# ishine/minimax-speech

Hardware: AMD Instinct MI355X
Metric: 24 kHz audio-seconds generated per wall-second per node (CosyVoice2-0.5B-shaped LM + flow + DAC-VAE, end to end) (higher is better)
Workload: dtype bf16

## Files before the change

### include/mmx_hip.h

```cpp
#ifndef MMX_HIP_H
#define MMX_HIP_H
#include <stdint.h>
#ifdef __cplusplus
extern "C" {
#endif

#ifndef __HIP__
typedef struct ihipStream_t* hipStream_t;
#endif

#define MMX_F32 0
#define MMX_BF16 1
#define MMX_X2 2
#define MMX_X3 3
#define MMX_X2W 0x12
#define MMX_X3W 0x13
#define MMX_H2 4
#define MMX_H2W 0x14

#define MMX_ACT_NONE 0
#define MMX_ACT_LRELU 1
#define MMX_ACT_GELU 2
#define MMX_ACT_SILU 3
#define MMX_ACT_MISH 4
#define MMX_ACT_TANH 5

int mmx_abi_version(void);

typedef struct MmxGemmParams {
    const void* A;
    const void* W;
    const float* bias;
    const float* residual;
    const float* rowmask;
    const float* alpha;
    float* out_f32;
    void* out_act;
    int64_t lda, ldw, ldr, ldo_f, ldo_a;
    int64_t a_bstride, w_bstride, r_bstride, rm_bstride, of_bstride, oa_bstride;
    int64_t row_off, row_lo, row_hi;
    int64_t out_off, out_len;
    int32_t M, N, batch;
    int32_t ntaps, cin, dil;
    int32_t bias_mod, alpha_mod, bias_per_row;
    int32_t act, act2;
    float slope;
    int32_t row_stride;
} MmxGemmParams;
int mmx_gemm_win(const MmxGemmParams* p, int dtype, hipStream_t stream);
#define MMX_TILE_128x128 1
#define MMX_TILE_128x64 2
#define MMX_TILE_64x64 3
#define MMX_TILE_32x64 4
int mmx_gemm_win_tile(const MmxGemmParams* p, int dtype, int tile, hipStream_t stream);

int mmx_rownorm(const float* x, int64_t ldx, int64_t x_bstride, int rows, int C, int batch,
                const float* gamma, const float* beta, float eps, int rms, int act,
                const float* rowmask, int64_t rm_bstride, const float* addvec, int64_t av_bstride,
                float* out_f32, int64_t ldo_f, int64_t of_bstride,
                void* out_act, int64_t ldo_a, int64_t oa_bstride, int dtype, hipStream_t stream);

int mmx_groupnorm(const float* x, int B, int T, int C, int groups, const float* gamma, const float* beta, float eps,
                  int act, const float* rowmask, void* out, int dtype, hipStream_t stream);

int mmx_act_rows(const float* x, int64_t rows, int C, int act, const float* rowmask, float* out_f32, void* out_act, int dtype,
                 hipStream_t stream);

int mmx_gather_rows(const int64_t* ids, int n, const float* table, int C, float scale, const float* rowmask,
                    float* out_f32, int64_t ldo_f, void* out_act, int64_t ldo_a, int dtype, hipStream_t stream);

int mmx_copy2d(const void* in, int in_dtype, int64_t ibs, int64_t irs, int64_t ics, int rep,
               void* out, int out_dtype, int64_t obs, int64_t ors, int64_t ocs,
               int rows, int cols, int batch, hipStream_t stream);

int mmx_est_pack(const float* x, int64_t x_bs, int x_mod, const float* mu, const float* spks, const float* cond, int B, int T, int C,
                 void* h, int64_t ldh, int dtype, hipStream_t stream);
int mmx_sinusoidal_emb(const float* t, int B, int dim, float scale, void* out, int dtype, hipStream_t stream);

int mmx_cfg_euler(float* x, const float* d_cond, const float* d_uncond, float cfg, float dt, int64_t n,
                  hipStream_t stream);

int mmx_attn_dense(const void* q, int64_t ldq, int64_t q_bs, const void* k, int64_t ldk, int64_t k_bs,
                   const void* v, int64_t ldv, int64_t v_bs, void* out, int64_t ldo, int64_t o_bs,
                   int B, int H, int D, int Tq, int Tk, float scale, const float* keymask, int64_t km_bs, int chunk,
                   const void* pos, int64_t ldp, const float* pos_u, const float* pos_v,
                   int head_stride, int q_begin, int dtype, hipStream_t stream);
int mmx_attn_flash_bf16(const void* q, int64_t ldq, int64_t q_bs, const void* k, int64_t ldk, int64_t k_bs,
                        const void* vt, int64_t ldvt, int64_t vt_bs, void* out, int64_t ldo, int64_t o_bs,
                        int B, int H, int T, float scale, const float* keymask, int64_t km_bs, int chunk, int q_begin,
                        const int32_t* klen, hipStream_t stream);
int mmx_attn_relpos_x(const float* q, int64_t ldq, int64_t q_bs, const float* k, int64_t ldk, int64_t k_bs, const float* v,
                      int64_t ldv, int64_t v_bs, const float* pos, int64_t ldp, const float* pos_u, const float* pos_v,
                      float* out, int64_t ldo, int64_t o_bs, int B, int H, int T, float scale, int chunk, const int32_t* klen,
                      hipStream_t stream);
int mmx_attn_flash_x(const float* q, int64_t ldq, int64_t q_bs, const float* k, int64_t ldk, int64_t k_bs,
                     const float* v, int64_t ldv, int64_t v_bs, float* out, int64_t ldo, int64_t o_bs,
                     int B, int H, int T, float scale, const float* keymask, int64_t km_bs, int chunk,
                     int q_begin, const int32_t* klen, hipStream_t stream);
int mmx_attn_flash_xs(const void* qk, int64_t ldqk, int64_t qk_bs, const void* vt, int64_t ldvt, int64_t vt_bs,
                      float* out, int64_t ldo, int64_t o_bs, int B, int H, int T, float scale, const float* keymask,
                      int64_t km_bs, int chunk, int q_begin, const int32_t* klen, int form, hipStream_t stream);
int mmx_attn_relpos_bf16(const void* q, int64_t ldq, int64_t q_bs, const void* k, int64_t ldk, int64_t k_bs,
                         const void* vt, int64_t ldvt, int64_t vt_bs, const void* pos, int64_t ldp,
                         const float* pos_u, const float* pos_v, void* out, int64_t ldo, int64_t o_bs,
                         int B, int H, int T, float scale, int chunk, const int32_t* klen, hipStream_t stream);

int mmx_attn_flash_fp8(const void* q, int64_t ldq, int64_t q_bs, const void* k, int64_t ldk, int64_t k_bs,
                       const void* vt, int64_t ldvt, int64_t vt_bs, void* out, int64_t ldo, int64_t o_bs,
                       int B, int H, int T, float scale, const float* keymask, int64_t km_bs, int chunk, int q_begin,
                       const int32_t* klen, hipStream_t stream);

int mmx_conv_cin1(const float* x, int64_t x_bs, int T, int C, int k, const float* w, const float* bias, float slope,
                  const float* alpha, float* out_f32, void* out_act, int batch, int dtype, hipStream_t stream);
int mmx_vae_sample(const float* ml, const float* noise, int64_t rows, int D, float* z, float* m, float* logs,
                   hipStream_t stream);
int mmx_mask_rows(void* x, int64_t rows, int C, const float* rowmask, int dtype, hipStream_t stream);
int mmx_pool_rows(const float* x, int64_t x_bs, int rows, int C, int batch, const float* mask, int64_t m_bs, void* out,
                  int64_t ldo, int dtype, hipStream_t stream);
int mmx_prefetch4(const void* p0, int64_t n0, const void* p1, int64_t n1, const void* p2, int64_t n2, const void* p3, int64_t n3,
                  void* sink, int workgroups, hipStream_t stream);
int mmx_resample_linear(const float* x, int64_t rows, int T, int T2, float* out, hipStream_t stream);

int mmx_conv_cout1_tanh(const void* act, int64_t a_bs, int T, int C, int k, const float* w, const float* bias,
                        float slope, int use_tanh, float* out, int64_t o_bs, int batch, int dtype, hipStream_t stream);

#define MMX_X_PACKED 1
#define MMX_OUT_PACKED 2
int mmx_pack_skinny(const void* w, int64_t ldw, int N, int K, const float* kscale, int interleave_half,
                    void* wp, int dtype, hipStream_t stream);
int mmx_skinny_gemm(const void* x, int x_dtype, int64_t ldx, int B, int K, int N, const void* wp,
                    const float* bias, int rs, float eps, int epi, float* out_f32, int64_t ldo_f,
                    void* out_act, int64_t ldo_a, int dtype, int flags, const float* kgamma, hipStream_t stream);

int mmx_decode_prep(const float* x, int64_t ldx, int B, int K, const float* gamma, float* h, int64_t ldh, void* xs,
                    float* ssq, int dtype, hipStream_t stream);
int mmx_skinny2(const void* xs, int B, int K, int N, const void* wp, const float* bias, const float* ssq_in, float eps,
                int epi, float* out, int64_t ldo, void* xs_out, const float* gamma_next, float* ssq_out,
                int tiles_per_wg, int ksplit, float* part, int64_t part_floats, int32_t* tickets, int dtype,
                hipStream_t stream);

int mmx_rope_kv_store(const float* qkv, int64_t ldqkv, int64_t qkv_bs, int B, int rows, int Hq, int Hkv, int D,
                      const float* inv_freq, const int32_t* pos, void* q_out, int64_t ldq, int64_t q_bs,
                      void* kc, void* vc, const int32_t* block_table, int max_pages, int page,
                      int dtype, hipStream_t stream);
int mmx_paged_attn(const void* q, int64_t ldq, int64_t q_bs, int B, int rows, int Hq, int Hkv, int D, float scale,
                   const int32_t* pos, const void* kc, const void* vc, const int32_t* block_table, int max_pages,
                   int page, void* out, int64_t ldo, int64_t o_bs, int dtype, hipStream_t stream);
#define MMX_DA_PACKED 1
#define MMX_DA_PER_HEAD 2
#define MMX_DA_SPLIT 4
#define MMX_DA_H2 8
#define MMX_DA_ONE_HEAD 16
int mmx_decode_attn(const float* qkv, int64_t ldqkv, int B, int Hq, int Hkv, int D, const float* inv_freq,
                    const float* rope_tab, const int32_t* pos, void* kc, void* vc, const int32_t* block_table, int max_pages, int page,
                    float scale, void* out, int64_t ldo, int dtype, int out_packed, hipStream_t stream);
int mmx_decode_attn_fin(const float* qkv, int64_t ldqkv, int B, int Hq, int Hkv, int D, const float* inv_freq,
                        const float* rope_tab, const int32_t* pos, const int32_t* finished, void* kc, void* vc,
                        const int32_t* block_table, int max_pages, int page, float scale, void* out, int64_t ldo, int dtype,
                        int out_packed, hipStream_t stream);
int mmx_swiglu(const float* gu, int64_t ldgu, int rows, int I, void* out, int64_t ldo, int dtype, hipStream_t stream);

int mmx_sample_step(const float* logits, int64_t ldl, int V, int B, int eos_id, int top_k, float top_p,
                    int win_size, float tau_r, uint64_t seed, int32_t* state, int32_t* out_tokens, int max_out,
                    int32_t* sampled, const int32_t* forced, const float* speech_emb, int E, float* next_x,
                    int64_t ldx, float* logp_out, hipStream_t stream);
int mmx_sample_step_tab(const float* logits, int64_t ldl, int V, int B, int eos_id, const int32_t* samp, int32_t* state,
                        int32_t* out_tokens, int max_out, int32_t* sampled, const int32_t* forced, const float* speech_emb,
                        int E, float* next_x, int64_t ldx, float* logp_out, hipStream_t stream);

typedef struct MmxEstNext {
    const void* wqkv;
    const float* n1g;
    const float* n1b;
    void* q_out;
    void* vt_out;
    int64_t q_bs, vt_bs;
    int32_t ldq, ldvt;
} MmxEstNext;
typedef struct MmxEstTailParams {
    const void* ao;
    float* x;
    const void* wo;
    const void* w1;
    const void* w2;
    const float* bo;
    const float* b1;
    const float* b2;
    const float* n3g;
    const float* n3b;
    const float* rowmask;
    void* act_out;
    int64_t ao_bs, x_bs, rm_bs, act_bs;
    int32_t ldao, act_ld, B, T;
    int32_t t_begin;
    float eps;
    MmxEstNext next;
} MmxEstTailParams;
typedef struct MmxEstResnetParams {
    const void* a_in;
    float* x;
    const void* w1;
    const void* w2;
    const void* wr;
    const float* b1;
    const float* g1;
    const float* be1;
    const float* b2;
    const float* g2;
    const float* be2;
    const float* br;
    const float* tv;
    const float* rowmask;
    int64_t a_bs, x_bs, tv_bs, rm_bs;
    int32_t lda, cin, B, T;
    int32_t t_begin;
    float eps;
    MmxEstNext next;
} MmxEstResnetParams;
int mmx_est_tail(const MmxEstTailParams* p, int dtype, int bm, int cfg, hipStream_t stream);
int mmx_est_resnet(const MmxEstResnetParams* p, int dtype, int bm, int cfg, hipStream_t stream);
typedef struct {
    const float* x;
    float* x_out;
    void* act_out;
    const void* w7;
    const void* w1;
    const float* b7;
    const float* b1;
    const float* a0;
    const float* a2;
    const float* alpha_next;
    const int32_t* lens;
    int64_t x_bs;
    int32_t B, T, C, dil;
    float slope;
} MmxDacRuParams;
int mmx_dac_ru(const MmxDacRuParams* p, int dtype, int bm, hipStream_t stream);

int mmx_logmel(const float* wave, int64_t w_bs, int L, int B, const float* gain, const int32_t* lens, const int32_t* h_lens,
               const void* basis, const void* filt, int n_fft, int hop, int bin0, int n_bins, int n_mels, float* out_cm,
               int64_t ldo, void* out_tm, int T, int dtype, hipStream_t stream);

int mmx_logmel_w(const float* wave, int64_t w_bs, int L, int B, const int32_t* lens, const int32_t* h_lens, const void* basis,
                 const void* filt, int n_fft, int hop, int bin0, int n_bins, int n_mels, float* out_cm, int64_t ldo,
                 void* out_tm, int T, int dtype, hipStream_t stream);

int mmx_s3_rope_fsmn(float* qkv, int64_t ldqkv, int64_t qkv_bs, int B, int T, int C, const float* x, int64_t x_bs, float* r,
                     int64_t r_bs, const float* wt, const float* rope_cos, const float* rope_sin, int rope_rows,
                     const int32_t* lens, hipStream_t stream);

int mmx_fsq_encode(const float* x, int64_t ldx, int64_t x_bs, int B, int T, int C, const float* W, const float* bias,
                   const int32_t* lens, int32_t* ids, int64_t ld_ids, float* pre, hipStream_t stream);

#define MMX_RESAMPLE_NOUT 1024
int mmx_resample_sinc(const float* wave, int64_t w_bs, int L, int B, const int32_t* lens, const int32_t* h_lens, int orig, int neu,
                      int width, const float* taps, const int32_t* first, const int32_t* count, int cmax, float* out,
                      int64_t o_bs, int out_cols, hipStream_t stream);

#define MMX_LOUD_PAD 0
#define MMX_LOUD_DROP 1
#define MMX_LOUD_MAX_CH 5
int mmx_kweight_blocks(const float* wave, int64_t w_bs, int L, int B, const int32_t* lens, int rate, int partial, const double* tab,
                       int seg, double* work, int cap, double* energy, int64_t e_bs, float* peak, hipStream_t stream);
int mmx_loudness_gate(const double* energy, int64_t e_bs, int cap, const float* peak, const int32_t* lens, int L, int nclips, int nch,
                      const double* G, int rate, int partial, float* lufs, int want_gain, float target_db, float max_peak, float* gain,
                      uint8_t* mask, int64_t mask_bs, hipStream_t stream);
int mmx_scale_rows(const float* x, int64_t x_bs, int L, int B, const int32_t* lens, const float* gain, int nch, float* out,
                   int64_t o_bs, hipStream_t stream);

int mmx_spec_dist(const float* x, int64_t x_bs, const float* y, int64_t y_bs, int L, int B, const int32_t* lens, const int32_t* h_lens,
                  const void* basis, const void* filt, int n_fft, int n_mels, double eps, double pow, double* work, int cap,
                  double* out, hipStream_t stream);
int mmx_wave_sums(const float* x, int64_t x_bs, const float* y, int64_t y_bs, int L, int B, const int32_t* lens, float clip, double* work,
                  int cap, double* out, hipStream_t stream);

#ifdef __cplusplus
}
#endif
#endif
```

### minimax-speech_amd/csrc/fused.hip

```cpp
#include "common.h"
#include "../../include/mmx_hip.h"
#include <type_traits>

namespace {

typedef __attribute__((ext_vector_type(4))) unsigned int u32x4_t;

__device__ unsigned long long* g_tail_stamps = nullptr;
#define TSTAMP(i) do { if constexpr (LAB) { if (st && lane == 0) st[(i)] = __builtin_amdgcn_s_memtime(); } } while (0)

template <typename T> struct FT;
template <> struct FT<bf16_t> { static constexpr int E = 8, KB = 32; typedef short8_t frag_t; };
template <> struct FT<float> { static constexpr int E = 4, KB = 16; typedef float4_t frag_t; };

template <typename T>
__device__ __forceinline__ float4_t mma(typename FT<T>::frag_t a, typename FT<T>::frag_t b, float4_t c) {
    if constexpr (sizeof(T) == 2) {
        return __builtin_amdgcn_mfma_f32_16x16x32_bf16(a, b, c, 0, 0, 0);
    } else {
#pragma unroll
        for (int s = 0; s < 4; ++s) c = __builtin_amdgcn_mfma_f32_16x16x4f32(a[s], b[s], c, 0, 0, 0);
        return c;
    }
}

__host__ __device__ constexpr int tile_pitch(int K, int esz) { return ((K * esz + 255) & ~255) + 32; }

template <typename T, int NF, int PF_>
struct WRing {
    static constexpr int E = FT<T>::E, PF = PF_;
    u32x4_t w[PF][NF];
    __device__ __forceinline__ void prime(const T* wb, long ns, int nk, int nf) {
#pragma unroll
        for (int p = 0; p < PF; ++p)
#pragma unroll
            for (int j = 0; j < NF; ++j)
                w[p][j] = *reinterpret_cast<const u32x4_t*>(wb + (j < nf ? j : 0) * ns + (long)(p < nk ? p : nk - 1) * 64 * E);
    }
};

template <typename T, int MF, int NF, int PF, int NS = 1, int RW = 4>
__device__ __forceinline__ void stage_run(WRing<T, RW, PF>& ring, const char* a_lane, int pitch, int cin_steps,
                                          const T* wb, long ns, int nk, const T* wbn, long nsn, int nkn, int nfn,
                                          float4_t (&acc)[MF][NF], int plane = 0, int tap_pitch = 0) {
    constexpr int E = FT<T>::E, KB = FT<T>::KB;
    typedef typename FT<T>::frag_t frag_t;
    if (tap_pitch == 0) tap_pitch = pitch;
    constexpr int AD = (PF % 2) ? PF : ((MF == 1 && PF >= 4) ? 4 : 2);
    static_assert(PF % AD == 0, "ring depths");
    if constexpr (NS == 2 && MF == 4) {
        frag_t a2[2][MF];
        int rt = 0, rc = 0, rs = 0, rp = 0;
        auto read_u = [&](frag_t (&dst)[MF]) {
            const char* ap = a_lane + rt * tap_pitch + rc * (KB * (int)sizeof(T)) + rp * plane;
#pragma unroll
            for (int i = 0; i < MF; ++i) dst[i] = *reinterpret_cast<const frag_t*>(ap + i * 16 * pitch);
            if (rp == 0) rp = 1;
            else {
                rp = 0;
                if (rs + 1 < nk) {
                    ++rs;
                    if (++rc == cin_steps) { rc = 0; ++rt; }
                }
            }
        };
        auto group2 = [&](int ks, auto last_c) {
            constexpr bool LAST = decltype(last_c)::value;
#pragma unroll
            for (int p = 0; p < PF; ++p) {
                frag_t b[NF];
#pragma unroll
                for (int jj = 0; jj < NF; ++jj) b[jj] = __builtin_bit_cast(frag_t, ring.w[p][jj]);
                if constexpr (LAST) {
                    if (wbn) {
                        const T* src = wbn + (long)(p < nkn ? p : nkn - 1) * 64 * E;
#pragma unroll
                        for (int jj = 0; jj < RW; ++jj) ring.w[p][jj] = *reinterpret_cast<const u32x4_t*>(src + (jj < nfn ? jj : 0) * nsn);
                    }
                } else {
                    const T* src = wb + (long)(ks + p + PF) * 64 * E;
#pragma unroll
                    for (int jj = 0; jj < NF; ++jj) ring.w[p][jj] = *reinterpret_cast<const u32x4_t*>(src + jj * ns);
                }
#pragma unroll
                for (int s2 = 0; s2 < 2; ++s2) {
                    read_u(a2[(s2 + 1) & 1]);
                    __builtin_amdgcn_sched_barrier(0);
#pragma unroll
                    for (int i = 0; i < MF; ++i)
#pragma unroll
                        for (int jj = 0; jj < NF; ++jj) acc[i][jj] = mma<T>(a2[s2][i], b[jj], acc[i][jj]);
                    __builtin_amdgcn_sched_barrier(0);
                }
            }
        };
        read_u(a2[0]);
        for (int ks = 0; ks + PF < nk; ks += PF) group2(ks, std::false_type{});
        group2(nk - PF, std::true_type{});
        return;
    }
    frag_t a[AD][NS][MF];
    int rt = 0, rc = 0, rs = 0;
    auto read_a = [&](frag_t (&dst)[NS][MF]) {
        const char* ap = a_lane + rt * tap_pitch + rc * (KB * (int)sizeof(T));
#pragma unroll
        for (int s2 = 0; s2 < NS; ++s2)
#pragma unroll
            for (int i = 0; i < MF; ++i) dst[s2][i] = *reinterpret_cast<const frag_t*>(ap + s2 * plane + i * 16 * pitch);
        if (rs + 1 < nk) {
            ++rs;
            if (++rc == cin_steps) { rc = 0; ++rt; }
        }
    };
    auto group = [&](int ks, auto last_c) {
        constexpr bool LAST = decltype(last_c)::value;
#pragma unroll
        for (int p = 0; p < PF; ++p) {
            read_a(a[(p + AD - 1) % AD]);
            frag_t b[NF];
#pragma unroll
            for (int jj = 0; jj < NF; ++jj) b[jj] = __builtin_bit_cast(frag_t, ring.w[p][jj]);
            if constexpr (LAST) {
                if (wbn) {
                    const T* src = wbn + (long)(p < nkn ? p : nkn - 1) * 64 * E;
#pragma unroll
                    for (int jj = 0; jj < RW; ++jj) ring.w[p][jj] = *reinterpret_cast<const u32x4_t*>(src + (jj < nfn ? jj : 0) * nsn);
                }
            } else {
                const T* src = wb + (long)(ks + p + PF) * 64 * E;
#pragma unroll
                for (int jj = 0; jj < NF; ++jj) ring.w[p][jj] = *reinterpret_cast<const u32x4_t*>(src + jj * ns);
            }
            __builtin_amdgcn_sched_barrier(0);
#pragma unroll
            for (int s2 = 0; s2 < NS; ++s2)
#pragma unroll
                for (int i = 0; i < MF; ++i)
#pragma unroll
                    for (int jj = 0; jj < NF; ++jj) acc[i][jj] = mma<T>(a[p % AD][s2][i], b[jj], acc[i][jj]);
            __builtin_amdgcn_sched_barrier(0);
        }
    };
#pragma unroll
    for (int s_ = 0; s_ < AD - 1; ++s_) read_a(a[s_]);
    for (int ks = 0; ks + PF < nk; ks += PF) group(ks, std::false_type{});
    group(nk - PF, std::true_type{});
}

template <typename T, int MF, int NF, int PF, int NS, int RW, bool WP>
__device__ __forceinline__ void stage_run_w(WRing<T, RW, PF>& ring, const char* a_lane, int pitch, int cin_steps,
                                            const T* wb, long ns, int nk, long wlo, const T* wbn, long nsn, int nkn, int nfn,
                                            float4_t (&acc)[MF][NF], int plane = 0, int tap_pitch = 0) {
    if constexpr (!WP) {
        stage_run<T, MF, NF, PF, NS, RW>(ring, a_lane, pitch, cin_steps, wb, ns, nk, wbn, nsn, nkn, nfn, acc, plane, tap_pitch);
    } else {
        stage_run<T, MF, NF, PF, NS, RW>(ring, a_lane, pitch, cin_steps, wb, ns, nk, wb + wlo, ns, nk, NF, acc, plane, tap_pitch);
        stage_run<T, MF, NF, PF, 1, RW>(ring, a_lane, pitch, cin_steps, wb + wlo, ns, nk, wbn, nsn, nkn, nfn, acc, 0, tap_pitch);
    }
}

template <int MF, int NF>
__device__ __forceinline__ void zero_acc(float4_t (&acc)[MF][NF]) {
#pragma unroll
    for (int i = 0; i < MF; ++i)
#pragma unroll
        for (int j = 0; j < NF; ++j) acc[i][j] = float4_t{0.f, 0.f, 0.f, 0.f};
}

constexpr int PATCH_FLOATS = 16 * 68;
constexpr int TAIL_PRM_FLOATS = 6 * 256 + 1024;
template <int NF>
__device__ __forceinline__ void to_rows(const float4_t (&acc)[NF], float* patch, int lane, float (&v)[NF * 4]) {
    constexpr int LDC = NF * 16 + 4;
    const int g = lane >> 4, l16 = lane & 15;
#pragma unroll
    for (int j = 0; j < NF; ++j)
#pragma unroll
        for (int r = 0; r < 4; ++r) patch[(4 * g + r) * LDC + j * 16 + l16] = acc[j][r];
    __builtin_amdgcn_fence(__ATOMIC_RELEASE, "wavefront");
    __builtin_amdgcn_wave_barrier();
    const float* src = patch + (lane >> 2) * LDC + (lane & 3) * (NF * 4);
#pragma unroll
    for (int c = 0; c < NF * 4; c += 4) {
        const float4_t t = *reinterpret_cast<const float4_t*>(src + c);
        v[c] = t[0]; v[c + 1] = t[1]; v[c + 2] = t[2]; v[c + 3] = t[3];
    }
    __builtin_amdgcn_wave_barrier();
}

constexpr int SPATCH_FLOATS = 16 * 20;
__device__ __forceinline__ void to_rows_sp(const float4_t (&acc)[2], float* patch, int lane, float (&v)[8]) {
    constexpr int LDC = 20;
    const int g = lane >> 4, l16 = lane & 15;
    const float* src = patch + (lane >> 2) * LDC + (lane & 1) * 8;
#pragma unroll
    for (int j = 0; j < 2; ++j) {
#pragma unroll
        for (int r = 0; r < 4; ++r) patch[(4 * g + r) * LDC + l16] = acc[j][r];
        __builtin_amdgcn_fence(__ATOMIC_RELEASE, "wavefront");
        __builtin_amdgcn_wave_barrier();
        if (((lane >> 1) & 1) == j) {
            const float4_t t0 = *reinterpret_cast<const float4_t*>(src), t1 = *reinterpret_cast<const float4_t*>(src + 4);
            v[0] = t0[0]; v[1] = t0[1]; v[2] = t0[2]; v[3] = t0[3];
            v[4] = t1[0]; v[5] = t1[1]; v[6] = t1[2]; v[7] = t1[3];
        }
        __builtin_amdgcn_wave_barrier();
    }
}
template <int NF, bool SP>
__device__ __forceinline__ void rows_of(const float4_t (&acc)[NF], float* patch, int lane, float (&v)[NF * 4]) {
    if constexpr (SP) { static_assert(NF == 2, "one-fragment patch: 32-column slices"); to_rows_sp(acc, patch, lane, v); }
    else to_rows<NF>(acc, patch, lane, v);
}

template <int N>
__device__ __forceinline__ void loadn(const float* p, float (&v)[N]) {
#pragma unroll
    for (int c = 0; c < N; c += 4) {
        const float4_t t = *reinterpret_cast<const float4_t*>(p + c);
        v[c] = t[0]; v[c + 1] = t[1]; v[c + 2] = t[2]; v[c + 3] = t[3];
    }
}
template <int N>
__device__ __forceinline__ void storen(float* p, const float (&v)[N]) {
#pragma unroll
    for (int c = 0; c < N; c += 4) *reinterpret_cast<float4_t*>(p + c) = float4_t{v[c], v[c + 1], v[c + 2], v[c + 3]};
}
template <typename T, int N>
__device__ __forceinline__ void storen_T(T* p, const float (&v)[N]) {
    if constexpr (sizeof(T) == 2) {
#pragma unroll
        for (int c = 0; c < N; c += 8) {
            uint4 pk;
            pk.x = pack_bf16x2(v[c], v[c + 1]);
            pk.y = pack_bf16x2(v[c + 2], v[c + 3]);
            pk.z = pack_bf16x2(v[c + 4], v[c + 5]);
            pk.w = pack_bf16x2(v[c + 6], v[c + 7]);
            *reinterpret_cast<uint4*>(p + c) = pk;
        }
    } else {
        storen<N>(p, v);
    }
}

template <typename T, int NS, int N>
__device__ __forceinline__ void store_tile(char* p, int plane, const float (&v)[N]) {
    if constexpr (NS == 1) {
        storen_T<T, N>(reinterpret_cast<T*>(p), v);
    } else {
        float lo[N];
#pragma unroll
        for (int c = 0; c < N; c += 8) {
            uint4 pk;
            pk.x = pack_bf16x2(v[c], v[c + 1]);
            pk.y = pack_bf16x2(v[c + 2], v[c + 3]);
            pk.z = pack_bf16x2(v[c + 4], v[c + 5]);
            pk.w = pack_bf16x2(v[c + 6], v[c + 7]);
            *reinterpret_cast<uint4*>(p + c * 2) = pk;
            const unsigned w[4] = {pk.x, pk.y, pk.z, pk.w};
#pragma unroll
            for (int e = 0; e < 4; ++e) {
                lo[c + 2 * e] = v[c + 2 * e] - __uint_as_float(w[e] << 16);
                lo[c + 2 * e + 1] = v[c + 2 * e + 1] - __uint_as_float(w[e] & 0xffff0000u);
            }
        }
        storen_T<bf16_t, N>(reinterpret_cast<bf16_t*>(p + plane), lo);
    }
}

template <int MFR, int CW, int NW>
__device__ __forceinline__ void layernorm_rows(float (&v)[MFR][CW], float* stats, const float (&g)[CW], const float (&be)[CW],
                                               float eps, int wave, int lane) {
    const int rl = lane >> 2;
    float mean[MFR];
    auto total = [&](int row) {
        float t = 0.f;
#pragma unroll
        for (int w = 0; w < NW; w += 4) {
            const float4_t q = *reinterpret_cast<const float4_t*>(stats + row * NW + w);
            t += (q[0] + q[1]) + (q[2] + q[3]);
        }
        return t;
    };
#pragma unroll
    for (int i = 0; i < MFR; ++i) {
        float s = 0.f;
#pragma unroll
        for (int c = 0; c < CW; ++c) s += v[i][c];
        s += dpp_f32<0xB1>(s);
        s += dpp_f32<0x4E>(s);
        if ((lane & 3) == 0) stats[(i * 16 + rl) * NW + wave] = s;
    }
    __syncthreads();
#pragma unroll
    for (int i = 0; i < MFR; ++i) mean[i] = total(i * 16 + rl) * (1.0f / 256.0f);
    __syncthreads();
#pragma unroll
    for (int i = 0; i < MFR; ++i) {
        float q = 0.f;
#pragma unroll
        for (int c = 0; c < CW; ++c) { const float d = v[i][c] - mean[i]; q += d * d; }
        q += dpp_f32<0xB1>(q);
        q += dpp_f32<0x4E>(q);
        if ((lane & 3) == 0) stats[(i * 16 + rl) * NW + wave] = q;
    }
    __syncthreads();
#pragma unroll
    for (int i = 0; i < MFR; ++i) {
        const float rstd = rsqrtf(total(i * 16 + rl) * (1.0f / 256.0f) + eps);
#pragma unroll
        for (int c = 0; c < CW; ++c) v[i][c] = (v[i][c] - mean[i]) * rstd * g[c] + be[c];
    }
}

template <typename T>
__device__ __forceinline__ void load_tile(const T* __restrict__ src, long ld, int r0, int nvalid, int rows, int K,
                                          char* tile, int pitch, int tid, int nthreads) {
    constexpr int E = FT<T>::E, U = 8;
    const int cpr = K / E;
    const int total = rows * cpr;
    for (int base = tid; base < total; base += U * nthreads) {
        uint4 v[U];
        int off[U];
#pragma unroll
        for (int u = 0; u < U; ++u) {
            const int id = base + u * nthreads;
            const int idc = id < total ? id : total - 1;
            const int r = idc / cpr, ch = idc - r * cpr;
            const int gr = r0 + r;
            const bool ok = gr >= 0 && gr < nvalid;
            const int grc = gr < 0 ? 0 : (gr < nvalid ? gr : nvalid - 1);
            v[u] = *reinterpret_cast<const uint4*>(src + (long)grc * ld + ch * E);
            if (!ok) v[u] = make_uint4(0, 0, 0, 0);
            off[u] = id < total ? r * pitch + ch * 16 : -1;
        }
#pragma unroll
        for (int u = 0; u < U; ++u)
            if (off[u] >= 0) *reinterpret_cast<uint4*>(tile + off[u]) = v[u];
    }
}
__device__ __forceinline__ void load_tile_split(const float* __restrict__ src, long ld, int r0, int nvalid, int rows, int K,
                                                char* tile, int pitch, int plane, int tid, int nthreads) {
    constexpr int U = 8;
    const int cpr = K / 4;
    const int total = rows * cpr;
    for (int base = tid; base < total; base += U * nthreads) {
        float4 v[U];
        int off[U];
#pragma unroll
        for (int u = 0; u < U; ++u) {
            const int id = base + u * nthreads;
            const int idc = id < total ? id : total - 1;
            const int r = idc / cpr, ch = idc - r * cpr;
            const int gr = r0 + r;
            const bool ok = gr >= 0 && gr < nvalid;
            const int grc = gr < 0 ? 0 : (gr < nvalid ? gr : nvalid - 1);
            v[u] = *reinterpret_cast<const float4*>(src + (long)grc * ld + ch * 4);
            if (!ok) v[u] = make_float4(0.f, 0.f, 0.f, 0.f);
            off[u] = id < total ? r * pitch + ch * 8 : -1;
        }
#pragma unroll
        for (int u = 0; u < U; ++u) {
            if (off[u] < 0) continue;
            uint2 hi, lo;
            hi.x = pack_bf16x2(v[u].x, v[u].y);
            hi.y = pack_bf16x2(v[u].z, v[u].w);
            lo.x = pack_bf16x2(v[u].x - __uint_as_float(hi.x << 16), v[u].y - __uint_as_float(hi.x & 0xffff0000u));
            lo.y = pack_bf16x2(v[u].z - __uint_as_float(hi.y << 16), v[u].w - __uint_as_float(hi.y & 0xffff0000u));
            *reinterpret_cast<uint2*>(tile + off[u]) = hi;
            *reinterpret_cast<uint2*>(tile + plane + off[u]) = lo;
        }
    }
}

__device__ __forceinline__ void load_tile_split_halves(const float* __restrict__ src, long ld, int r0, int nvalid, int rows,
                                                       char* tile0, char* tile1, int pitch, int plane, int tid, int nthreads) {
    constexpr int U = 16;
    constexpr int cpr = 512 / 4;
    const int total = rows * cpr;
    for (int base = tid; base < total; base += U * nthreads) {
        float4 v[U];
        int off[U];
#pragma unroll
        for (int u = 0; u < U; ++u) {
            const int id = base + u * nthreads;
            const int idc = id < total ? id : total - 1;
            const int r = idc / cpr, ch = idc - r * cpr;
            const int gr = r0 + r;
            const bool ok = gr >= 0 && gr < nvalid;
            const int grc = gr < 0 ? 0 : (gr < nvalid ? gr : nvalid - 1);
            v[u] = *reinterpret_cast<const float4*>(src + (long)grc * ld + ch * 4);
            if (!ok) v[u] = make_float4(0.f, 0.f, 0.f, 0.f);
            off[u] = id < total ? r * pitch + (ch & 63) * 8 + ((ch >> 6) ? (int)(tile1 - tile0) : 0) : -1;
        }
#pragma unroll
        for (int u = 0; u < U; ++u) {
            if (off[u] < 0) continue;
            uint2 hi, lo;
            hi.x = pack_bf16x2(v[u].x, v[u].y);
            hi.y = pack_bf16x2(v[u].z, v[u].w);
            lo.x = pack_bf16x2(v[u].x - __uint_as_float(hi.x << 16), v[u].y - __uint_as_float(hi.x & 0xffff0000u));
            lo.y = pack_bf16x2(v[u].z - __uint_as_float(hi.y << 16), v[u].w - __uint_as_float(hi.y & 0xffff0000u));
            *reinterpret_cast<uint2*>(tile0 + off[u]) = hi;
            *reinterpret_cast<uint2*>(tile0 + plane + off[u]) = lo;
        }
    }
}

template <typename T, int NW, int PW = 4>
__device__ __forceinline__ const T* qkv_pass(const void* wqkv, int wave, int lane, int p) {
    constexpr int E = FT<T>::E, KB = FT<T>::KB, PC = 16 * PW, PPK = 512 / (PC * NW);
    return reinterpret_cast<const T*>(wqkv) + (long)lane * E +
           (long)(((p / PPK) * 512 + (wave * PPK + p % PPK) * PC) / 16) * ((long)(256 / KB) * 64 * E);
}

template <typename T, int MF, int PF, int NW, int NS = 1, int PW = 4, bool WP = false>
__device__ __forceinline__ void ln_qkv(float (&xv)[MF][64 / NW], const float (&n1g)[64 / NW], const float (&n1b)[64 / NW],
                                       const MmxEstNext& nx, float eps, char* a1, float* patch, float* stats,
                                       WRing<T, PW, PF>& ring, int b, int t0, int Tn, int wave, int lane, int plane = 0,
                                       unsigned long long* st = nullptr) {
    typedef std::conditional_t<NS == 1, T, float> TI;
    constexpr int E = FT<T>::E, KB = FT<T>::KB, C = 256, CW = 64 / NW, PC = 16 * PW, PPK = 512 / (PC * NW), NP = 3 * PPK;
    constexpr int P1 = tile_pitch(C, sizeof(T));
    constexpr int NK = C / KB;
    const int g = lane >> 4, l16 = lane & 15, rl = lane >> 2;
    const int col0 = wave * (256 / NW) + (lane & 3) * CW;
    const long ns = (long)NK * 64 * E;
    layernorm_rows<MF, CW, NW>(xv, stats, n1g, n1b, eps, wave, lane);
#pragma unroll
    for (int i = 0; i < MF; ++i) store_tile<T, NS, CW>(a1 + (i * 16 + rl) * P1 + col0 * (int)sizeof(T), plane, xv[i]);
    __syncthreads();
    TSTAMP(32);
    const char* a_lane = a1 + l16 * P1 + g * 16;
    constexpr bool VTC = sizeof(T) == 2;
    const bool planes = NS > 1 && nx.vt_out != nullptr;
    const bool vt_path = VTC && (NS == 1 || planes);
    constexpr int PV = 16 * 2 + 16;
    for (int p = 0; p < NP; ++p) {
        float4_t acc[MF][PW];
        zero_acc(acc);
        const T* wn = p + 1 < NP ? qkv_pass<T, NW, PW>(nx.wqkv, wave, lane, p + 1) : nullptr;
        stage_run_w<T, MF, PW, PF, NS, PW, WP>(ring, a_lane, P1, NK, qkv_pass<T, NW, PW>(nx.wqkv, wave, lane, p), ns, NK, 1536L * C, wn, ns, NK, PW, acc, plane);
        TSTAMP(33 + 2 * p);
        const int kind = p / PPK, cw = (wave * PPK + p % PPK) * PC;
        if (vt_path && kind == 2) {
            char* vw = reinterpret_cast<char*>(patch);
#pragma unroll
            for (int s2 = 0; s2 < NS; ++s2) {
                bf16_t* dst = reinterpret_cast<bf16_t*>(nx.vt_out) + (long)b * nx.vt_bs + (long)s2 * 512 * nx.ldvt + (long)cw * nx.ldvt + t0;
#pragma unroll
                for (int i = 0; i < MF; ++i) {
#pragma unroll
                    for (int j = 0; j < PW; ++j) {
                        uint2 pk;
                        pk.x = pack_bf16x2(acc[i][j][0], acc[i][j][1]);
                        pk.y = pack_bf16x2(acc[i][j][2], acc[i][j][3]);
                        *reinterpret_cast<uint2*>(vw + (j * 16 + l16) * PV + (4 * g) * 2) = pk;
                        if (s2 + 1 < NS) {
                            acc[i][j][0] -= __uint_as_float(pk.x << 16); acc[i][j][1] -= __uint_as_float(pk.x & 0xffff0000u);
                            acc[i][j][2] -= __uint_as_float(pk.y << 16); acc[i][j][3] -= __uint_as_float(pk.y & 0xffff0000u);
                        }
                    }
                    __builtin_amdgcn_fence(__ATOMIC_RELEASE, "wavefront");
                    __builtin_amdgcn_wave_barrier();
#pragma unroll
                    for (int k2 = 0; k2 < PW / 2; ++k2) {
                        const int chunk = lane + 64 * k2, colv = chunk >> 1, c8 = chunk & 1;
                        uint4 v = *reinterpret_cast<const uint4*>(vw + colv * PV + c8 * 16);
                        const int t = t0 + i * 16 + c8 * 8;
                        if (t >= Tn) continue;
                        if (t + 8 > Tn) {
                            unsigned short* h = reinterpret_cast<unsigned short*>(&v);
#pragma unroll
                            for (int e = 0; e < 8; ++e)
                                if (t + e >= Tn) h[e] = 0;
                        }
                        *reinterpret_cast<uint4*>(dst + (long)colv * nx.ldvt + i * 16 + c8 * 8) = v;
                    }
                    __builtin_amdgcn_wave_barrier();
                }
            }
        } else if (planes) {
            bf16_t* out = reinterpret_cast<bf16_t*>(nx.q_out) + (long)b * nx.q_bs;
            const int col = kind * 512 + cw + (lane & 3) * (4 * PW);
#pragma unroll
            for (int i = 0; i < MF; ++i) {
                float v[4 * PW], lo[4 * PW];
                to_rows<PW>(acc[i], patch, lane, v);
                const int t = t0 + i * 16 + rl;
                if (t < Tn) {
#pragma unroll
                    for (int c = 0; c < 4 * PW; ++c) lo[c] = v[c] - bf2f(f2bf(v[c]));
                    storen_T<bf16_t, 4 * PW>(out + (long)t * nx.ldq + col, v);
                    storen_T<bf16_t, 4 * PW>(out + (long)t * nx.ldq + 1024 + col, lo);
                }
            }
        } else {
            TI* out = reinterpret_cast<TI*>(nx.q_out) + (long)b * nx.q_bs;
            const int col = kind * 512 + cw + (lane & 3) * (4 * PW);
#pragma unroll
            for (int i = 0; i < MF; ++i) {
                float v[4 * PW];
                to_rows<PW>(acc[i], patch, lane, v);
                const int t = t0 + i * 16 + rl;
                if (t < Tn) storen_T<TI, 4 * PW>(out + (long)t * nx.ldq + col, v);
            }
        }
        TSTAMP(34 + 2 * p);
    }
}

template <typename T, int BM, int PF, int NW, int NS, int PW, bool WP = false>
__device__ __forceinline__ void est_tail_tile(const MmxEstTailParams& p, const int tile) {
    constexpr bool HK = NS == 2 && BM == 64 && sizeof(T) == 2;
    static_assert(!HK || (NW == 8 && PW == 2), "64-row split tile: 8 waves, 32-column passes");
    constexpr int MF = BM / 16, E = FT<T>::E, KB = FT<T>::KB, C = 256, CI = 512, CF = 1024, CH = HK ? 256 : 512, NCH = CF / CH;
    constexpr int WC = C / NW, CW = WC / 4, NFN = WC / 16, PC = 16 * PW, PPC = CH / (PC * NW);
    static_assert(NFN <= PW, "the ring is PW fragments wide");
    constexpr int P0 = tile_pitch(HK ? C : CI, sizeof(T)), P1 = tile_pitch(C, sizeof(T));
    constexpr int PL0 = BM * P0, PL1 = BM * P1;
    constexpr bool PRECISE = sizeof(T) == 4;
    typedef std::conditional_t<NS == 1, T, float> TI;
    extern __shared__ __attribute__((aligned(16))) char smem[];
    char* buf0 = smem;
    char* a1 = buf0 + NS * PL0;
    float* patch_all = reinterpret_cast<float*>(a1 + NS * PL1);
    constexpr int PATCHF = HK ? SPATCH_FLOATS : PATCH_FLOATS;
    float* stats = patch_all + NW * PATCHF;
    float* prm = stats + BM * NW;
    constexpr int PRM_BO = 0, PRM_N3G = 256, PRM_N3B = 512, PRM_B2 = 768, PRM_N1G = 1024, PRM_N1B = 1280, PRM_B1 = 1536;
    const int tid = threadIdx.x, lane = tid & 63, wave = tid >> 6;
    const int g = lane >> 4, l16 = lane & 15, rl = lane >> 2;
    float* patch = patch_all + wave * PATCHF;
    const int b = blockIdx.y, t0 = p.t_begin + tile * BM, Tn = p.T;
    const int col0 = wave * WC + (lane & 3) * CW;
    unsigned long long* st = nullptr;
    if constexpr (LAB) {
        st = g_tail_stamps;
        if (st) st += ((long)(blockIdx.y * gridDim.x + blockIdx.x) * NW + wave) * 64;
    }
    TSTAMP(0);

    const T* wo = reinterpret_cast<const T*>(p.wo) + (long)lane * E;
    const T* w1 = reinterpret_cast<const T*>(p.w1) + (long)lane * E;
    const T* w2 = reinterpret_cast<const T*>(p.w2) + (long)lane * E;
    constexpr int NK0 = CI / KB, NK1 = C / KB, NK2 = CH / KB, NK2T = CF / KB, NKH = NK0 / 2;
    const long ns0 = (long)NK0 * 64 * E, ns1 = (long)NK1 * 64 * E, ns2 = (long)NK2T * 64 * E;
    WRing<T, PW, PF> ring;
    const T* wo_w = wo + (long)(wave * NFN) * ns0;

    auto w1_pass = [&](int q) { return w1 + (long)(((q / PPC) * CH + (wave * PPC + q % PPC) * PC) / 16) * ns1; };
    float x1[MF][CW];
    float rm[MF];
    {
        const float* rmk = p.rowmask ? p.rowmask + (long)b * p.rm_bs : nullptr;
#pragma unroll
        for (int i = 0; i < MF; ++i) {
            const int t = t0 + i * 16 + rl;
            rm[i] = (rmk && t < Tn) ? rmk[t] : 1.f;
        }
    }
    {
        constexpr int PRM_PER = (TAIL_PRM_FLOATS / 4 + 64 * NW - 1) / (64 * NW);
        float4_t pr[PRM_PER];
#pragma unroll
        for (int k = 0; k < PRM_PER; ++k) {
            const int id0 = tid + k * 64 * NW, id = id0 < TAIL_PRM_FLOATS / 4 ? id0 : TAIL_PRM_FLOATS / 4 - 1;
            const int seg = id >> 6, o4 = (id & 63) * 4;
            const float* src = seg == 0 ? p.bo : seg == 1 ? p.n3g : seg == 2 ? p.n3b : seg == 3 ? p.b2
                             : seg == 4 ? (p.next.wqkv ? p.next.n1g : p.b2) : seg == 5 ? (p.next.wqkv ? p.next.n1b : p.b2) : p.b1 + (seg - 6) * 256;
            pr[k] = *reinterpret_cast<const float4_t*>(src + o4);
        }
        const float* xr = p.x + (long)b * p.x_bs;
#pragma unroll
        for (int i = 0; i < MF; ++i) {
            const int t = t0 + i * 16 + rl;
            loadn<CW>(xr + (long)(t < Tn ? t : Tn - 1) * C + col0, x1[i]);
            if (t >= Tn) {
#pragma unroll
                for (int c = 0; c < CW; ++c) x1[i][c] = 0.f;
            }
        }
        ring.prime(wo_w, ns0, NK0, NFN);
        if constexpr (HK) {
            static_assert(P0 == P1 && PL0 == PL1, "both halves of the attention tile have the shape of a1");
            load_tile_split_halves(reinterpret_cast<const float*>(p.ao) + (long)b * p.ao_bs, p.ldao, t0, Tn, BM, buf0, a1, P0, PL0, tid, 64 * NW);
        } else if constexpr (NS == 1) load_tile<T>(reinterpret_cast<const T*>(p.ao) + (long)b * p.ao_bs, p.ldao, t0, Tn, BM, CI, buf0, P0, tid, 64 * NW);
        else load_tile_split(reinterpret_cast<const float*>(p.ao) + (long)b * p.ao_bs, p.ldao, t0, Tn, BM, CI, buf0, P0, PL0, tid, 64 * NW);
#pragma unroll
        for (int k = 0; k < PRM_PER; ++k) {
            const int id = tid + k * 64 * NW;
            if (id < TAIL_PRM_FLOATS / 4) *reinterpret_cast<float4_t*>(prm + id * 4) = pr[k];
        }
        TSTAMP(1);
        __syncthreads();
        TSTAMP(2);
        float4_t acc[MF][NFN];
        zero_acc(acc);
        if constexpr (HK) {
            const T* wo_h = wo_w + (long)NKH * 64 * E;
            if constexpr (WP) {
                const long wlo = (long)C * CI;
                stage_run<T, MF, NFN, PF, NS, PW>(ring, buf0 + l16 * P0 + g * 16, P0, NKH, wo_w, ns0, NKH, wo_h, ns0, NKH, NFN, acc, PL0);
                stage_run<T, MF, NFN, PF, NS, PW>(ring, a1 + l16 * P1 + g * 16, P1, NKH, wo_h, ns0, NKH, wo_w + wlo, ns0, NKH, NFN, acc, PL1);
                stage_run<T, MF, NFN, PF, 1, PW>(ring, buf0 + l16 * P0 + g * 16, P0, NKH, wo_w + wlo, ns0, NKH, wo_h + wlo, ns0, NKH, NFN, acc, 0);
                stage_run<T, MF, NFN, PF, 1, PW>(ring, a1 + l16 * P1 + g * 16, P1, NKH, wo_h + wlo, ns0, NKH, w1_pass(0), ns1, NK1, PW, acc, 0);
            } else {
                stage_run<T, MF, NFN, PF, NS, PW>(ring, buf0 + l16 * P0 + g * 16, P0, NKH, wo_w, ns0, NKH, wo_h, ns0, NKH, NFN, acc, PL0);
                stage_run<T, MF, NFN, PF, NS, PW>(ring, a1 + l16 * P1 + g * 16, P1, NKH, wo_h, ns0, NKH, w1_pass(0), ns1, NK1, PW, acc, PL1);
            }
        } else
        stage_run_w<T, MF, NFN, PF, NS, PW, WP>(ring, buf0 + l16 * P0 + g * 16, P0, NK0, wo_w, ns0, NK0, (long)C * CI, w1_pass(0), ns1, NK1, PW, acc, PL0);
        TSTAMP(3);
        float bo[CW];
        loadn<CW>(prm + PRM_BO + col0, bo);
#pragma unroll
        for (int i = 0; i < MF; ++i) {
            float v[CW];
            rows_of<NFN, HK>(acc[i], patch, lane, v);
#pragma unroll
            for (int c = 0; c < CW; ++c) x1[i][c] += v[c] + bo[c];
        }
        TSTAMP(4);
    }
    float n3g[CW], n3b[CW];
    loadn<CW>(prm + PRM_N3G + col0, n3g);
    loadn<CW>(prm + PRM_N3B + col0, n3b);
    {
        float hn[MF][CW];
#pragma unroll
        for (int i = 0; i < MF; ++i)
#pragma unroll
            for (int c = 0; c < CW; ++c) hn[i][c] = x1[i][c];
        layernorm_rows<MF, CW, NW>(hn, stats, n3g, n3b, p.eps, wave, lane);
#pragma unroll
        for (int i = 0; i < MF; ++i) store_tile<T, NS, CW>(a1 + (i * 16 + rl) * P1 + col0 * (int)sizeof(T), PL1, hn[i]);
    }
    __syncthreads();
    TSTAMP(5);
    float4_t acc2[MF][NFN];
    zero_acc(acc2);
    const T* w2_w = w2 + (long)(wave * NFN) * ns2;
    for (int ch = 0; ch < NCH; ++ch) {
        const int sb = HK ? 6 + ch * 5 : 0;
        for (int h = 0; h < PPC; ++h) {
            const int q = ch * PPC + h;
            const int hc = (wave * PPC + h) * PC + (lane & 3) * (4 * PW);
            float4_t acc[MF][PW];
            zero_acc(acc);
            const bool more = h + 1 < PPC;
            const T* wn = more ? w1_pass(q + 1) : w2_w + (long)(ch * NK2) * 64 * E;
            stage_run_w<T, MF, PW, PF, NS, PW, WP>(ring, a1 + l16 * P1 + g * 16, P1, NK1, w1_pass(q), ns1, NK1, (long)CF * C, wn, more ? ns1 : ns2,
                                                   more ? NK1 : NK2, more ? PW : NFN, acc, PL1);
            TSTAMP(HK ? sb : 6 + ch * 12 + h * 2);
            if constexpr (HK) {
                const bool odd = lane & 1;
                const int cb = (wave * PPC + h) * PC;
                float bj[PW];
#pragma unroll
                for (int j = 0; j < PW; ++j) bj[j] = prm[PRM_B1 + ch * CH + cb + j * 16 + l16];
                char* dst = buf0 + (4 * g + (odd ? 2 : 0)) * P0 + (cb + (l16 & ~1)) * (int)sizeof(T);
#pragma unroll
                for (int r = 0; r < MF; ++r)
#pragma unroll
                    for (int j = 0; j < PW; ++j) {
                        float v[4];
#pragma unroll
                        for (int e = 0; e < 4; e += 2) {
                            const f32x2_t gl = gelu_fast2(f32x2_t{acc[r][j][e] + bj[j], acc[r][j][e + 1] + bj[j]});
                            v[e] = gl.x; v[e + 1] = gl.y;
                        }
                        const float y0 = dpp_f32<0xB1>(odd ? v[0] : v[2]), y1 = dpp_f32<0xB1>(odd ? v[1] : v[3]);
                        const float a0 = odd ? y0 : v[0], c0 = odd ? v[2] : y0, a1v = odd ? y1 : v[1], c1 = odd ? v[3] : y1;
                        const unsigned h0 = pack_bf16x2(a0, c0), h1 = pack_bf16x2(a1v, c1);
                        const unsigned l0 = pack_bf16x2(a0 - __uint_as_float(h0 << 16), c0 - __uint_as_float(h0 & 0xffff0000u));
                        const unsigned l1 = pack_bf16x2(a1v - __uint_as_float(h1 << 16), c1 - __uint_as_float(h1 & 0xffff0000u));
                        char* q2 = dst + r * 16 * P0 + j * 16 * (int)sizeof(T);
                        *reinterpret_cast<unsigned*>(q2) = h0;
                        *reinterpret_cast<unsigned*>(q2 + P0) = h1;
                        *reinterpret_cast<unsigned*>(q2 + PL0) = l0;
                        *reinterpret_cast<unsigned*>(q2 + PL0 + P0) = l1;
                    }
                TSTAMP(sb + 1);
                continue;
            }
            float b1[4 * PW];
            loadn<4 * PW>(prm + PRM_B1 + ch * CH + hc, b1);
#pragma unroll
            for (int i = 0; i < MF; ++i) {
                float v[4 * PW];
                rows_of<PW, HK>(acc[i], patch, lane, v);
                if constexpr (NS > 1 && !PRECISE) {
#pragma unroll
                    for (int c = 0; c < 4 * PW; c += 2) {
                        const f32x2_t gl = gelu_fast2(f32x2_t{v[c] + b1[c], v[c + 1] + b1[c + 1]});
                        v[c] = gl.x; v[c + 1] = gl.y;
                    }
                } else {
#pragma unroll
                    for (int c = 0; c < 4 * PW; ++c) v[c] = act_c<((PRECISE || NS > 1) ? ACT_GELU : ACT_GELU_POLY), PRECISE>(v[c] + b1[c], 0.f);
                }
                store_tile<T, NS, 4 * PW>(buf0 + (i * 16 + rl) * P0 + hc * (int)sizeof(T), PL0, v);
            }
            TSTAMP(HK ? sb + 1 : 7 + ch * 12 + h * 2);
        }
        __syncthreads();
        TSTAMP(HK ? sb + 2 : 14 + ch * 12);
        const T* wn = ch + 1 < NCH ? w1_pass((ch + 1) * PPC) : (p.next.wqkv ? qkv_pass<T, NW, PW>(p.next.wqkv, wave, lane, 0) : nullptr);
        if constexpr (WP && !HK) {
            constexpr int NKQ = NK2 / 2;
            const T* wh = w2_w + (long)(ch * NK2) * 64 * E;
            stage_run_w<T, MF, NFN, PF, NS, PW, WP>(ring, buf0 + l16 * P0 + g * 16, P0, NKQ, wh, ns2, NKQ, (long)C * CF, wh + (long)NKQ * 64 * E, ns2, NKQ, NFN, acc2, PL0);
            stage_run_w<T, MF, NFN, PF, NS, PW, WP>(ring, buf0 + NKQ * KB * (int)sizeof(T) + l16 * P0 + g * 16, P0, NKQ, wh + (long)NKQ * 64 * E, ns2, NKQ, (long)C * CF, wn, ns1, NK1, PW, acc2, PL0);
        } else
        stage_run_w<T, MF, NFN, PF, NS, PW, WP>(ring, buf0 + l16 * P0 + g * 16, P0, NK2, w2_w + (long)(ch * NK2) * 64 * E, ns2, NK2, (long)C * CF, wn, ns1, NK1, PW, acc2, PL0);
        TSTAMP(HK ? sb + 3 : 15 + ch * 12);
        __syncthreads();
        TSTAMP(HK ? sb + 4 : 16 + ch * 12);
    }
    float* wpatch = HK ? reinterpret_cast<float*>(buf0) + wave * PATCH_FLOATS : patch;
    {
        float* xw = p.x + (long)b * p.x_bs;
        float b2[CW];
        loadn<CW>(prm + PRM_B2 + col0, b2);
#pragma unroll
        for (int i = 0; i < MF; ++i) {
            float v[CW];
            to_rows<NFN>(acc2[i], wpatch, lane, v);
            const int t = t0 + i * 16 + rl;
#pragma unroll
            for (int c = 0; c < CW; ++c) x1[i][c] = (x1[i][c] + v[c] + b2[c]) * rm[i];
            if (t < Tn) {
                storen<CW>(xw + (long)t * C + col0, x1[i]);
                if (p.act_out)
                    storen_T<TI, CW>(reinterpret_cast<TI*>(p.act_out) + (long)b * p.act_bs + (long)t * p.act_ld + col0, x1[i]);
            }
        }
    }
    TSTAMP(31);
    if (p.next.wqkv) {
        float n1g[CW], n1b[CW];
        loadn<CW>(prm + PRM_N1G + col0, n1g);
        loadn<CW>(prm + PRM_N1B + col0, n1b);
        ln_qkv<T, MF, PF, NW, NS, PW, WP>(x1, n1g, n1b, p.next, p.eps, a1, wpatch, stats, ring, b, t0, Tn, wave, lane, PL1, st);
    }
    TSTAMP(63);
}

template <typename T, int BM, int PF, int NW, int NS = 1, int OCC = 1, int PW = 4, bool WP = false>
__global__ __launch_bounds__(64 * NW, OCC) void est_tail_kernel(MmxEstTailParams p) {
    est_tail_tile<T, BM, PF, NW, NS, PW, WP>(p, blockIdx.x);
}

template <typename T, int BM, int PF, int NW, int NS = 1, bool WP = false>
__global__ __launch_bounds__(64 * NW) void est_resnet_kernel(MmxEstResnetParams p) {
    constexpr int MF = BM / 16, MH = MF + 1, E = FT<T>::E, KB = FT<T>::KB, C = 256;
    constexpr int WC = C / NW, CW = WC / 4, NFN = WC / 16;
    constexpr int P1 = tile_pitch(C, sizeof(T));
    constexpr int PLH = (BM + 16) * P1;
    constexpr bool PRECISE = sizeof(T) == 4;
    extern __shared__ __attribute__((aligned(16))) char smem[];
    const int cin = p.cin;
    const int PA = tile_pitch(cin, sizeof(T));
    const int PLA = (BM + 18) * PA;
    char* ain = smem;
    char* h1 = ain + NS * PLA;
    float* patch_all = reinterpret_cast<float*>(h1 + NS * PLH);
    float* stats = patch_all + NW * PATCH_FLOATS;
    const int tid = threadIdx.x, lane = tid & 63, wave = tid >> 6;
    const int g = lane >> 4, l16 = lane & 15, rl = lane >> 2;
    float* patch = patch_all + wave * PATCH_FLOATS;
    const int b = blockIdx.y, t0 = p.t_begin + blockIdx.x * BM, Tn = p.T;
    const int col0 = wave * WC + (lane & 3) * CW;
    const int cs = cin / KB;
    const T* w1 = reinterpret_cast<const T*>(p.w1) + (long)lane * E;
    const T* w2 = reinterpret_cast<const T*>(p.w2) + (long)lane * E;
    const T* wr = reinterpret_cast<const T*>(p.wr) + (long)lane * E;
    const int nk1 = 3 * cs, nk2 = 3 * (C / KB), nkr = cs;
    const long ns1 = (long)nk1 * 64 * E, ns2 = (long)nk2 * 64 * E, nsr = (long)nkr * 64 * E;
    const T* w1_w = w1 + (long)(wave * NFN) * ns1;
    const T* w2_w = w2 + (long)(wave * NFN) * ns2;
    const T* wr_w = wr + (long)(wave * NFN) * nsr;
    WRing<T, 4, PF> ring;
    ring.prime(w1_w, ns1, nk1, NFN);
    const float* rmk = p.rowmask ? p.rowmask + (long)b * p.rm_bs : nullptr;
    float bb[CW], tv[CW], gg[CW], be[CW], rm1[MH];
    loadn<CW>(p.b1 + col0, bb);
    loadn<CW>(p.tv + (long)b * p.tv_bs + col0, tv);
    loadn<CW>(p.g1 + col0, gg);
    loadn<CW>(p.be1 + col0, be);
#pragma unroll
    for (int i = 0; i < MH; ++i) {
        const int t = t0 - 16 + i * 16 + rl;
        rm1[i] = (t >= 0 && t < Tn) ? (rmk ? rmk[t] : 1.f) : 0.f;
    }
    if constexpr (NS == 1) load_tile<T>(reinterpret_cast<const T*>(p.a_in) + (long)b * p.a_bs, p.lda, t0 - 18, Tn, BM + 18, cin, ain, PA, tid, 64 * NW);
    else load_tile_split(reinterpret_cast<const float*>(p.a_in) + (long)b * p.a_bs, p.lda, t0 - 18, Tn, BM + 18, cin, ain, PA, PLA, tid, 64 * NW);
    __syncthreads();

    {
        float4_t acc[MH][NFN];
        zero_acc(acc);
        stage_run_w<T, MH, NFN, PF, NS, 4, WP>(ring, ain + l16 * PA + g * 16, PA, cs, w1_w, ns1, nk1, (long)C * 3 * cin, w2_w, ns2, nk2, NFN, acc, PLA);
        float hv[MH][CW];
#pragma unroll
        for (int i = 0; i < MH; ++i) {
            to_rows<NFN>(acc[i], patch, lane, hv[i]);
#pragma unroll
            for (int c = 0; c < CW; ++c) hv[i][c] += bb[c];
        }
        layernorm_rows<MH, CW, NW>(hv, stats, gg, be, p.eps, wave, lane);
#pragma unroll
        for (int i = 0; i < MH; ++i) {
            const int t = t0 - 16 + i * 16 + rl;
            float o[CW];
#pragma unroll
            for (int c = 0; c < CW; ++c) {
                const float y = act_c<ACT_MISH, PRECISE>(hv[i][c], 0.f) * rm1[i];
                o[c] = t >= 0 ? (y + tv[c]) * rm1[i] : 0.f;
            }
            store_tile<T, NS, CW>(h1 + (i * 16 + rl) * P1 + col0 * (int)sizeof(T), PLH, o);
        }
    }
    float br[CW];
    loadn<CW>(p.b2 + col0, bb);
    loadn<CW>(p.g2 + col0, gg);
    loadn<CW>(p.be2 + col0, be);
    loadn<CW>(p.br + col0, br);
    __syncthreads();
    float h2[MF][CW];
    {
        float4_t acc[MF][NFN];
        zero_acc(acc);
        stage_run_w<T, MF, NFN, PF, NS, 4, WP>(ring, h1 + (14 + l16) * P1 + g * 16, P1, C / KB, w2_w, ns2, nk2, (long)C * 3 * C, wr_w, nsr, nkr, NFN, acc, PLH);
#pragma unroll
        for (int i = 0; i < MF; ++i) {
            to_rows<NFN>(acc[i], patch, lane, h2[i]);
#pragma unroll
            for (int c = 0; c < CW; ++c) h2[i][c] += bb[c];
        }
        layernorm_rows<MF, CW, NW>(h2, stats, gg, be, p.eps, wave, lane);
#pragma unroll
        for (int i = 0; i < MF; ++i)
#pragma unroll
            for (int c = 0; c < CW; ++c) h2[i][c] = act_c<ACT_MISH, PRECISE>(h2[i][c], 0.f) * rm1[i + 1];
    }
    {
        if (p.next.wqkv) { loadn<CW>(p.next.n1g + col0, gg); loadn<CW>(p.next.n1b + col0, be); }
        float4_t acc[MF][NFN];
        zero_acc(acc);
        const T* wq0 = p.next.wqkv ? qkv_pass<T, NW>(p.next.wqkv, wave, lane, 0) : nullptr;
        stage_run_w<T, MF, NFN, PF, NS, 4, WP>(ring, ain + (18 + l16) * PA + g * 16, PA, cs, wr_w, nsr, nkr, (long)C * cin, wq0, (long)(C / KB) * 64 * E, C / KB, 4, acc, PLA);
        float* xw = p.x + (long)b * p.x_bs;
#pragma unroll
        for (int i = 0; i < MF; ++i) {
            float v[CW];
            to_rows<NFN>(acc[i], patch, lane, v);
            const int t = t0 + i * 16 + rl;
#pragma unroll
            for (int c = 0; c < CW; ++c) h2[i][c] += v[c] + br[c];
            if (t < Tn) storen<CW>(xw + (long)t * C + col0, h2[i]);
        }
    }
    __syncthreads();
    if (p.next.wqkv) ln_qkv<T, MF, PF, NW, NS, 4, WP>(h2, gg, be, p.next, p.eps, h1, patch, stats, ring, b, t0, Tn, wave, lane, PLH);
}


__host__ __device__ constexpr int dac_pitch(int cp) { return (((cp * 2 + 31) / 32) | 1) * 32; }
__host__ __device__ constexpr int dac_patch_floats(int C) { return 16 * ((C % 48 == 0 ? 48 : 64) + 4); }

template <int C, int BM, int WR, int WC, int NS, int PF, bool WP = false, int NF = C / (16 * WC)>
__global__ __launch_bounds__(256) void dac_ru_kernel(MmxDacRuParams p) {
    typedef bf16_t T;
    constexpr int E = 8, KB = 32, CP = (C + 31) / 32 * 32, PA = dac_pitch(CP);
    constexpr int NC = 4 * NF, WCOLS = 16 * NF, DAC_PATCH_FLOATS = dac_patch_floats(C);
    static_assert(NF >= 2 && NF <= 4 && 16 * (WCOLS + 4) <= DAC_PATCH_FLOATS, "n-fragments per wave / patch");
    constexpr int BMW = BM / WR, MF = BMW / 16;
    constexpr int NK7 = 7 * CP / KB, NK1 = CP / KB;
    constexpr bool PRECISE = NS > 1;
    static_assert(WR * WC == 4 && WC * NF * 16 == C && NK7 % PF == 0 && NK1 % PF == 0, "wave grid / ring depth");
    typedef std::conditional_t<NS == 1, bf16_t, float> TA;
    extern __shared__ __attribute__((aligned(16))) char smem[];
    const int d = p.dil, halo = 3 * d, rows_in = BM + 2 * halo;
    const int PLA = rows_in * PA, PLM = BM * PA;
    char* ain = smem;
    char* mid = ain + NS * PLA;
    float* patch_all = reinterpret_cast<float*>(mid + NS * PLM);
    float* prm = patch_all + 4 * DAC_PATCH_FLOATS;
    auto snk = [](float x, float alpha, float inv) {
        const float sn = PRECISE ? sin_cw(alpha * x) : __sinf(alpha * x);
        return x + inv * (sn * sn);
    };
    const int tid = threadIdx.x, lane = tid & 63, wave = tid >> 6;
    const int g = lane >> 4, l16 = lane & 15, rl = lane >> 2;
    const int wr = wave / WC, wc = wave % WC;
    float* patch = patch_all + wave * DAC_PATCH_FLOATS;
    const int b = blockIdx.y, t0 = blockIdx.x * BM;
    const int len = p.lens ? p.lens[b] : p.T;
    const int lc = len > 0 ? len : 1;
    const float* xb = p.x + (long)b * p.x_bs;

    const T* w7 = reinterpret_cast<const T*>(p.w7) + (long)lane * E;
    const T* w1 = reinterpret_cast<const T*>(p.w1) + (long)lane * E;
    const long ns7 = (long)NK7 * 64 * E, ns1 = (long)NK1 * 64 * E;
    const T* w7_w = w7 + (long)(wc * NF) * ns7;
    const T* w1_w = w1 + (long)(wc * NF) * ns1;
    WRing<T, NF, PF> ring;
    ring.prime(w7_w, ns7, NK7, NF);

    for (int id = tid; id < 8 * CP; id += 256) {
        const int v = id / CP, c = id - v * CP;
        const float* src = v == 0 ? p.a0 : v == 1 ? p.a2 : v == 2 ? p.b7 : v == 3 ? p.b1 : v == 4 ? p.alpha_next : v == 5 ? p.a0 : v == 6 ? p.a2 : p.alpha_next;
        const float val = (c < C && src) ? src[c] : 0.f;
        prm[id] = v < 5 ? val : 1.0f / (val + 1e-9f);
    }
    __syncthreads();
    {
        constexpr int CPR = CP / 4, U = 16;
        const int total = rows_in * CPR;
        for (int base = tid; base < total; base += U * 256) {
            float4 v[U];
            int off[U], cch[U];
#pragma unroll
            for (int u = 0; u < U; ++u) {
                const int id = base + u * 256;
                const int idc = id < total ? id : total - 1;
                const int r = idc / CPR, ch = idc - r * CPR;
                const int t = t0 - halo + r;
                const bool ok = t >= 0 && t < len && ch * 4 < C;
                const int tc = t < 0 ? 0 : (t < lc ? t : lc - 1);
                const int cc = ch * 4 < C ? ch * 4 : 0;
                v[u] = *reinterpret_cast<const float4*>(xb + (long)tc * C + cc);
                if (!ok) v[u] = make_float4(0.f, 0.f, 0.f, 0.f);
                off[u] = id < total ? r * PA + ch * 8 : -1;
                cch[u] = ch * 4;
            }
#pragma unroll
            for (int u = 0; u < U; ++u) {
                if (off[u] < 0) continue;
                const float4_t al = *reinterpret_cast<const float4_t*>(prm + cch[u]);
                const float4_t iv = *reinterpret_cast<const float4_t*>(prm + 5 * CP + cch[u]);
                float o[4] = {snk(v[u].x, al[0], iv[0]), snk(v[u].y, al[1], iv[1]), snk(v[u].z, al[2], iv[2]), snk(v[u].w, al[3], iv[3])};
                uint2 hi;
                hi.x = pack_bf16x2(o[0], o[1]);
                hi.y = pack_bf16x2(o[2], o[3]);
                *reinterpret_cast<uint2*>(ain + off[u]) = hi;
                if constexpr (NS > 1) {
                    uint2 lo;
                    lo.x = pack_bf16x2(o[0] - __uint_as_float(hi.x << 16), o[1] - __uint_as_float(hi.x & 0xffff0000u));
                    lo.y = pack_bf16x2(o[2] - __uint_as_float(hi.y << 16), o[3] - __uint_as_float(hi.y & 0xffff0000u));
                    *reinterpret_cast<uint2*>(ain + PLA + off[u]) = lo;
                }
            }
        }
        if constexpr (CP > C) {
            for (int id = tid; id < BM * (CP - C) / 4; id += 256) {
                const int r = id / ((CP - C) / 4), ch = id % ((CP - C) / 4);
#pragma unroll
                for (int s2 = 0; s2 < NS; ++s2) *reinterpret_cast<uint2*>(mid + s2 * PLM + r * PA + (C + ch * 4) * 2) = make_uint2(0, 0);
            }
        }
    }
    __syncthreads();
    {
        float4_t acc[MF][NF];
        zero_acc(acc);
        stage_run_w<T, MF, NF, PF, NS, NF, WP>(ring, ain + (wr * BMW + l16) * PA + g * 16, PA, CP / KB, w7_w, ns7, NK7, (long)C * 7 * CP, w1_w, ns1, NK1, NF, acc, PLA, d * PA);
        const int col = wc * WCOLS + (lane & 3) * NC;
        float b7[NC], a2[NC], i2[NC];
        loadn<NC>(prm + 2 * CP + col, b7);
        loadn<NC>(prm + 1 * CP + col, a2);
        loadn<NC>(prm + 6 * CP + col, i2);
#pragma unroll
        for (int i = 0; i < MF; ++i) {
            float v[NC];
            to_rows<NF>(acc[i], patch, lane, v);
#pragma unroll
            for (int c = 0; c < NC; ++c) {
                float y = v[c] + b7[c];
                y = y > 0.f ? y : y * p.slope;
                v[c] = snk(y, a2[c], i2[c]);
            }
            char* dst = mid + (wr * BMW + i * 16 + rl) * PA + col * 2;
            unsigned w[NC / 2];
#pragma unroll
            for (int e = 0; e < NC / 2; ++e) w[e] = pack_bf16x2(v[2 * e], v[2 * e + 1]);
#pragma unroll
            for (int e = 0; e < NC / 4; ++e) *reinterpret_cast<uint2*>(dst + 8 * e) = make_uint2(w[2 * e], w[2 * e + 1]);
            if constexpr (NS > 1) {
                unsigned l[NC / 2];
#pragma unroll
                for (int e = 0; e < NC / 2; ++e)
                    l[e] = pack_bf16x2(v[2 * e] - __uint_as_float(w[e] << 16), v[2 * e + 1] - __uint_as_float(w[e] & 0xffff0000u));
#pragma unroll
                for (int e = 0; e < NC / 4; ++e) *reinterpret_cast<uint2*>(dst + PLM + 8 * e) = make_uint2(l[2 * e], l[2 * e + 1]);
            }
        }
    }
    const int col = wc * WCOLS + (lane & 3) * NC;
    float xr[MF][NC];
#pragma unroll
    for (int i = 0; i < MF; ++i) {
        const int t = t0 + wr * BMW + i * 16 + rl;
        loadn<NC>(xb + (long)(t < lc ? t : lc - 1) * C + col, xr[i]);
    }
    __syncthreads();
    {
        float4_t acc[MF][NF];
        zero_acc(acc);
        stage_run_w<T, MF, NF, PF, NS, NF, WP>(ring, mid + (wr * BMW + l16) * PA + g * 16, PA, NK1, w1_w, ns1, NK1, (long)C * CP, (const T*)nullptr, 0, 0, NF, acc, PLM);
        float b1[NC], an[NC], in[NC];
        loadn<NC>(prm + 3 * CP + col, b1);
        loadn<NC>(prm + 4 * CP + col, an);
        loadn<NC>(prm + 7 * CP + col, in);
        float* xo = p.x_out ? p.x_out + (long)b * p.x_bs : nullptr;
#pragma unroll
        for (int i = 0; i < MF; ++i) {
            float v[NC];
            to_rows<NF>(acc[i], patch, lane, v);
            const int t = t0 + wr * BMW + i * 16 + rl;
            const bool live = t < len;
#pragma unroll
            for (int c = 0; c < NC; ++c) {
                float y = v[c] + b1[c];
                y = y > 0.f ? y : y * p.slope;
                v[c] = live ? y + xr[i][c] : 0.f;
            }
            if (t < p.T) {
                if (xo) storen<NC>(xo + (long)t * C + col, v);
                if (p.act_out) {
#pragma unroll
                    for (int c = 0; c < NC; ++c) v[c] = snk(v[c], an[c], in[c]);
                    TA* ao = reinterpret_cast<TA*>(p.act_out) + (long)b * p.x_bs + (long)t * C + col;
                    if constexpr (NS == 1) {
#pragma unroll
                        for (int e = 0; e < NC / 4; ++e)
                            *reinterpret_cast<uint2*>(ao + 4 * e) = make_uint2(pack_bf16x2(v[4 * e], v[4 * e + 1]), pack_bf16x2(v[4 * e + 2], v[4 * e + 3]));
                    } else {
                        storen<NC>(reinterpret_cast<float*>(ao), v);
                    }
                }
            }
        }
    }
}

constexpr size_t LDS_MAX = 160 * 1024;
constexpr size_t dac_ru_lds(int C, int bm, int ns, int dil) {
    const int CP = (C + 31) / 32 * 32, PA = dac_pitch(CP);
    return (size_t)ns * ((size_t)(bm + 6 * dil) * PA + (size_t)bm * PA) + 4 * dac_patch_floats(C) * 4 + 8 * CP * 4;
}
constexpr size_t tail_lds(int esz, int bm, int nw, int ns) {
    if (ns == 2 && bm == 64 && esz == 2)
        return (size_t)ns * 2 * bm * tile_pitch(256, esz) + (size_t)nw * SPATCH_FLOATS * 4 + (size_t)bm * nw * 4 + (size_t)TAIL_PRM_FLOATS * 4;
    return ns * ((size_t)bm * tile_pitch(512, esz) + (size_t)bm * tile_pitch(256, esz)) + (size_t)nw * PATCH_FLOATS * 4 + (size_t)bm * nw * 4 +
           (size_t)TAIL_PRM_FLOATS * 4;
}
constexpr size_t resnet_lds(int esz, int bm, int nw, int ns, int cin) {
    return ns * ((size_t)(bm + 18) * tile_pitch(cin, esz) + (size_t)(bm + 16) * tile_pitch(256, esz)) + (size_t)nw * PATCH_FLOATS * 4 +
           (size_t)(bm + 16) * nw * 4;
}

template <typename P>
struct Form {
    int dtype;
    bool wp;
    int bm, nw, pf;
    int pw, C;
    int (*launch)(const P&, hipStream_t);
};
template <typename T, int NS>
constexpr int form_dtype = sizeof(T) == 4 ? MMX_F32 : NS == 2 ? MMX_X2 : MMX_BF16;
template <typename P, size_t N>
constexpr const Form<P>* find_form(const Form<P> (&forms)[N], int dtype, bool wp, int bm, int nw, int pf, int pw, int C) {
    for (const Form<P>& f : forms)
        if (f.dtype == dtype && f.wp == wp && f.bm == bm && f.nw == nw && f.pf == pf && f.pw == pw && f.C == C) return &f;
    return nullptr;
}
constexpr bool cfg_fields_ok(int cfg, int known) {
    const int pf = cfg & 15, nw = (cfg >> 4) & 15;
    return cfg >= 0 && !(cfg & ~known) && (pf == 0 || pf == 2 || pf == 4 || pf == 8) && (nw == 0 || nw == 4 || nw == 8);
}

int check_next(const MmxEstNext& nx, int dtype, int T_) {
    if (!nx.wqkv) return MMX_OK;
    MMX_CHECK_ARG(nx.n1g && nx.n1b && nx.q_out);
    MMX_CHECK_ARG(((uintptr_t)nx.q_out % 16) == 0 && nx.q_bs % 8 == 0);
    if (dtype == MMX_X2) {
        if (nx.vt_out) {
            MMX_CHECK_ARG(nx.ldq % 8 == 0 && nx.ldq >= 2048 && nx.q_bs % 8 == 0 && nx.ldvt % 8 == 0 && nx.ldvt >= ((T_ + 7) / 8) * 8);
            MMX_CHECK_ARG(((uintptr_t)nx.vt_out % 16) == 0 && nx.vt_bs % 8 == 0 && nx.vt_bs >= 2 * 512 * (int64_t)nx.ldvt);
        } else {
            MMX_CHECK_ARG(nx.ldq % 4 == 0 && nx.ldq >= 1536 && nx.q_bs % 4 == 0);
        }
    } else if (dtype == MMX_BF16) {
        MMX_CHECK_ARG(nx.vt_out && nx.ldq % 8 == 0 && nx.ldq >= 1024 && nx.ldvt % 8 == 0 && nx.ldvt >= ((T_ + 7) / 8) * 8);
        MMX_CHECK_ARG(((uintptr_t)nx.vt_out % 16) == 0 && nx.vt_bs % 8 == 0);
    } else {
        MMX_CHECK_ARG(nx.ldq % 4 == 0 && nx.ldq >= 1536);
    }
    return MMX_OK;
}

template <typename T, int BM, int PF, int NW, int NS, int PW, bool WP>
int launch_tail(const MmxEstTailParams& p, hipStream_t stream) {
    constexpr size_t lds = tail_lds(sizeof(T), BM, NW, NS);
    MMX_CHECK_ARG(lds <= LDS_MAX);
    MMX_LDS_OPT_IN((est_tail_kernel<T, BM, PF, NW, NS, 1, PW, WP>), lds);
    hipLaunchKernelGGL((est_tail_kernel<T, BM, PF, NW, NS, 1, PW, WP>), dim3((p.T - p.t_begin + BM - 1) / BM, p.B), dim3(64 * NW), lds, stream, p);
    MMX_LAUNCH_CHECK();
    return MMX_OK;
}
using TailForm = Form<MmxEstTailParams>;
template <typename T, int BM, int PF, int NW, int NS = 1, int PW = 4, bool WP = false>
constexpr TailForm tail_form() { return {form_dtype<T, NS>, WP, BM, NW, PF, PW, 0, launch_tail<T, BM, PF, NW, NS, PW, WP>}; }
constexpr TailForm TAIL_FORMS[] = {
    tail_form<bf16_t, 64, 2, 8, 1, 2>(), tail_form<bf16_t, 32, 8, 8, 1, 2>(), tail_form<bf16_t, 32, 4, 8, 1, 2>(),
    tail_form<bf16_t, 64, 4, 4>(), tail_form<bf16_t, 64, 2, 4>(), tail_form<bf16_t, 32, 4, 8>(), tail_form<bf16_t, 32, 2, 8>(),
    tail_form<bf16_t, 32, 2, 4>(), tail_form<bf16_t, 32, 4, 4>(), tail_form<bf16_t, 16, 4, 8>(), tail_form<bf16_t, 16, 8, 4>(),
    tail_form<bf16_t, 64, 2, 8, 2, 2>(), tail_form<bf16_t, 64, 4, 8, 2, 2>(), tail_form<bf16_t, 32, 2, 8, 2, 2>(), tail_form<bf16_t, 32, 4, 8, 2, 2>(),
    tail_form<bf16_t, 32, 2, 8, 2>(), tail_form<bf16_t, 32, 4, 4, 2>(), tail_form<bf16_t, 16, 4, 8, 2>(), tail_form<bf16_t, 16, 8, 4, 2>(),
    tail_form<bf16_t, 64, 2, 8, 2, 2, true>(), tail_form<bf16_t, 32, 2, 8, 2, 4, true>(), tail_form<bf16_t, 16, 4, 8, 2, 4, true>(),
    tail_form<float, 32, 4, 4>(), tail_form<float, 16, 8, 4>(),
};
constexpr const TailForm* tail_select(int dtype, bool wp, int bm, int cfg) {
    if (!cfg_fields_ok(cfg, 0x7ff) || (bm != 16 && bm != 32 && bm != 64)) return nullptr;
    if (wp) cfg = 0;
    if (cfg & (256 | 1024)) return nullptr;
    int pf = cfg & 15, nw = (cfg >> 4) & 15;
    bool narrow = (cfg >> 9) & 1;
    if (cfg == 0 && dtype == MMX_BF16 && bm >= 32) { narrow = true; pf = bm == 64 ? 2 : 8; }
    if (dtype == MMX_X2 && bm == 64) narrow = true;
    if (narrow) nw = 8;
    else if (nw == 0) nw = dtype == MMX_X2 || (dtype == MMX_BF16 && bm == 32) ? 8 : 4;
    const int pw = narrow ? 2 : 4, pf_tile = narrow ? 128 / bm : 512 / (bm * nw);
    const TailForm* f = find_form(TAIL_FORMS, dtype, wp, bm, nw, pf, pw, 0);
    return f ? f : find_form(TAIL_FORMS, dtype, wp, bm, nw, pf_tile, pw, 0);
}
static_assert(tail_select(MMX_BF16, false, 64, 0)->launch == launch_tail<bf16_t, 64, 2, 8, 1, 2, false> && tail_select(MMX_BF16, false, 32, 0)->launch == launch_tail<bf16_t, 32, 8, 8, 1, 2, false>);
static_assert(tail_select(MMX_BF16, false, 16, 0)->launch == launch_tail<bf16_t, 16, 8, 4, 1, 4, false> && tail_select(MMX_X2, false, 64, 0)->launch == launch_tail<bf16_t, 64, 2, 8, 2, 2, false>);
static_assert(tail_select(MMX_X2, false, 32, 0)->launch == launch_tail<bf16_t, 32, 2, 8, 2, 4, false> && tail_select(MMX_X2, false, 16, 0)->launch == launch_tail<bf16_t, 16, 4, 8, 2, 4, false>);
static_assert(tail_select(MMX_X2, true, 64, 0)->launch == launch_tail<bf16_t, 64, 2, 8, 2, 2, true> && tail_select(MMX_X2, true, 32, 0)->launch == launch_tail<bf16_t, 32, 2, 8, 2, 4, true>);
static_assert(tail_select(MMX_X2, true, 16, 0)->launch == launch_tail<bf16_t, 16, 4, 8, 2, 4, true>);
static_assert(tail_select(MMX_F32, false, 32, 0)->launch == launch_tail<float, 32, 4, 4, 1, 4, false> && tail_select(MMX_F32, false, 16, 0)->launch == launch_tail<float, 16, 8, 4, 1, 4, false>);

template <typename T, int BM, int PF, int NW, int NS, bool WP>
int launch_resnet(const MmxEstResnetParams& p, hipStream_t stream) {
    const size_t lds = resnet_lds(sizeof(T), BM, NW, NS, p.cin);
    MMX_CHECK_ARG(lds <= LDS_MAX);
    MMX_LDS_OPT_IN((est_resnet_kernel<T, BM, PF, NW, NS, WP>), lds);
    hipLaunchKernelGGL((est_resnet_kernel<T, BM, PF, NW, NS, WP>), dim3((p.T - p.t_begin + BM - 1) / BM, p.B), dim3(64 * NW), lds, stream, p);
    MMX_LAUNCH_CHECK();
    return MMX_OK;
}
using ResnetForm = Form<MmxEstResnetParams>;
template <typename T, int BM, int PF, int NW, int NS = 1, bool WP = false>
constexpr ResnetForm resnet_form() { return {form_dtype<T, NS>, WP, BM, NW, PF, 0, 0, launch_resnet<T, BM, PF, NW, NS, WP>}; }
constexpr ResnetForm RESNET_FORMS[] = {
    resnet_form<bf16_t, 64, 2, 8>(), resnet_form<bf16_t, 32, 4, 8>(), resnet_form<bf16_t, 32, 2, 8>(), resnet_form<bf16_t, 16, 4, 8>(), resnet_form<bf16_t, 16, 2, 8>(),
    resnet_form<bf16_t, 64, 4, 4>(), resnet_form<bf16_t, 64, 2, 4>(), resnet_form<bf16_t, 32, 4, 4>(), resnet_form<bf16_t, 32, 2, 4>(),
    resnet_form<bf16_t, 16, 8, 4>(), resnet_form<bf16_t, 16, 4, 4>(), resnet_form<bf16_t, 16, 2, 4>(),
    resnet_form<float, 16, 8, 4>(), resnet_form<float, 16, 4, 4>(), resnet_form<float, 16, 2, 4>(),
    resnet_form<bf16_t, 32, 4, 8, 2>(), resnet_form<bf16_t, 32, 2, 8, 2>(), resnet_form<bf16_t, 32, 4, 4, 2>(), resnet_form<bf16_t, 32, 2, 4, 2>(),
    resnet_form<bf16_t, 16, 4, 8, 2>(), resnet_form<bf16_t, 16, 2, 8, 2>(), resnet_form<bf16_t, 16, 4, 4, 2>(), resnet_form<bf16_t, 16, 2, 4, 2>(),
    resnet_form<bf16_t, 32, 4, 8, 2, true>(), resnet_form<bf16_t, 32, 2, 8, 2, true>(), resnet_form<bf16_t, 32, 4, 4, 2, true>(), resnet_form<bf16_t, 32, 2, 4, 2, true>(),
    resnet_form<bf16_t, 16, 4, 8, 2, true>(), resnet_form<bf16_t, 16, 2, 8, 2, true>(), resnet_form<bf16_t, 16, 4, 4, 2, true>(), resnet_form<bf16_t, 16, 2, 4, 2, true>(),
};
constexpr int ring_depth(int want, int cin, int kb) {
    int pf = want;
    while (pf > 2 && ((3 * cin / kb) % pf || (cin / kb) % pf || (256 / kb) % pf)) pf /= 2;
    return (cin / kb) % 2 == 0 ? pf : 0;
}
constexpr const ResnetForm* resnet_select(int dtype, bool wp, int bm, int cfg, int cin) {
    if (!cfg_fields_ok(cfg, 0xff)) return nullptr;
    int nw = cfg >> 4;
    if (dtype == MMX_X2) nw = nw != 4 && resnet_lds(2, 32, 8, 2, cin) <= LDS_MAX ? 8 : 4;
    else if (nw == 0) nw = dtype == MMX_BF16 && resnet_lds(2, bm, 8, 1, cin) <= LDS_MAX ? 8 : 4;
    for (int pf = ring_depth(cfg & 15 ? cfg & 15 : 8, cin, dtype == MMX_F32 ? 16 : 32); pf >= 2; pf /= 2)
        if (const ResnetForm* f = find_form(RESNET_FORMS, dtype, wp, bm, nw, pf, 0, 0)) return f;
    return nullptr;
}
static_assert(resnet_select(MMX_BF16, false, 64, 0, 256)->launch == launch_resnet<bf16_t, 64, 2, 8, 1, false> && resnet_select(MMX_BF16, false, 32, 0, 256)->launch == launch_resnet<bf16_t, 32, 4, 8, 1, false>);
static_assert(resnet_select(MMX_X2, false, 32, 0, 320)->launch == launch_resnet<bf16_t, 32, 2, 4, 2, false> && resnet_select(MMX_X2, false, 32, 0, 256)->launch == launch_resnet<bf16_t, 32, 4, 8, 2, false>);
static_assert(resnet_select(MMX_X2, false, 32, 16 * 4, 256)->launch == launch_resnet<bf16_t, 32, 4, 4, 2, false> && resnet_select(MMX_X2, false, 16, 0, 512)->launch == launch_resnet<bf16_t, 16, 4, 4, 2, false>);
static_assert(resnet_select(MMX_X2, true, 32, 0, 320)->launch == launch_resnet<bf16_t, 32, 2, 4, 2, true> && resnet_select(MMX_X2, true, 32, 0, 256)->launch == launch_resnet<bf16_t, 32, 4, 8, 2, true>);
static_assert(resnet_select(MMX_X2, true, 32, 16 * 4, 256)->launch == launch_resnet<bf16_t, 32, 4, 4, 2, true> && resnet_select(MMX_F32, false, 16, 0, 256)->launch == launch_resnet<float, 16, 8, 4, 1, false>);

template <int C, int BM, int WR, int WC, int NS, int PF, bool WP>
int launch_dac_ru(const MmxDacRuParams& p, hipStream_t stream) {
    const size_t lds = dac_ru_lds(C, BM, NS, p.dil);
    MMX_CHECK_ARG(lds <= LDS_MAX);
    MMX_LDS_OPT_IN((dac_ru_kernel<C, BM, WR, WC, NS, PF, WP>), lds);
    hipLaunchKernelGGL((dac_ru_kernel<C, BM, WR, WC, NS, PF, WP>), dim3((p.T + BM - 1) / BM, p.B), dim3(256), lds, stream, p);
    MMX_LAUNCH_CHECK();
    return MMX_OK;
}
using DacRuForm = Form<MmxDacRuParams>;
template <int C, int BM, int WR, int WC, int NS, int PF, bool WP = false>
constexpr DacRuForm dac_ru_form() { return {NS == 2 ? MMX_X2 : MMX_BF16, WP, BM, 0, 0, 0, C, launch_dac_ru<C, BM, WR, WC, NS, PF, WP>}; }
constexpr DacRuForm DAC_RU_FORMS[] = {
    dac_ru_form<48, 256, 4, 1, 1, 2>(), dac_ru_form<48, 128, 4, 1, 1, 2>(), dac_ru_form<48, 64, 4, 1, 1, 2>(),
    dac_ru_form<96, 256, 2, 2, 1, 3>(), dac_ru_form<96, 128, 2, 2, 1, 3>(), dac_ru_form<96, 64, 2, 2, 1, 3>(),
    dac_ru_form<192, 128, 1, 4, 1, 2>(), dac_ru_form<192, 64, 1, 4, 1, 2>(), dac_ru_form<192, 32, 1, 4, 1, 2>(),
    dac_ru_form<48, 128, 4, 1, 2, 2>(), dac_ru_form<48, 64, 4, 1, 2, 2>(),
    dac_ru_form<96, 128, 2, 2, 2, 3>(), dac_ru_form<96, 64, 2, 2, 2, 3>(), dac_ru_form<96, 32, 2, 2, 2, 3>(),
    dac_ru_form<192, 32, 1, 4, 2, 2>(), dac_ru_form<192, 16, 1, 4, 2, 2>(),
    dac_ru_form<48, 64, 4, 1, 2, 2, true>(), dac_ru_form<96, 128, 2, 2, 2, 3, true>(), dac_ru_form<96, 64, 2, 2, 2, 3, true>(),
    dac_ru_form<192, 32, 1, 4, 2, 2, true>(),
    dac_ru_form<64, 256, 4, 1, 1, 2>(), dac_ru_form<64, 128, 4, 1, 1, 2>(), dac_ru_form<64, 64, 4, 1, 1, 2>(),
    dac_ru_form<128, 128, 2, 2, 1, 2>(), dac_ru_form<128, 64, 2, 2, 1, 2>(),
    dac_ru_form<64, 128, 4, 1, 2, 2>(), dac_ru_form<64, 64, 4, 1, 2, 2>(),
    dac_ru_form<128, 64, 2, 2, 2, 2>(), dac_ru_form<128, 32, 2, 2, 2, 2>(),
};
static_assert(dac_ru_lds(64, 256, 1, 9) <= LDS_MAX && dac_ru_lds(128, 128, 1, 9) <= LDS_MAX && dac_ru_lds(64, 128, 2, 9) <= LDS_MAX);
static_assert(dac_ru_lds(128, 64, 2, 9) <= LDS_MAX && dac_ru_lds(128, 128, 2, 9) > LDS_MAX);
constexpr const DacRuForm* dac_ru_select(int dtype, bool wp, int bm, int C, int dil) {
    const int dflt = dtype == MMX_BF16 ? (C == 48 || C == 64 || C == 128 ? 128 : C == 96 ? 256 : dil > 3 ? 32 : 64)
                   : dtype == MMX_X2   ? (C == 48 || C == 64 || C == 128 ? 64 : C == 96 ? (dil > 3 ? 128 : 64) : 32) : 0;
    if (wp && bm != 0 && bm != dflt) return nullptr;
    return find_form(DAC_RU_FORMS, dtype, wp, bm ? bm : dflt, 0, 0, 0, C);
}
static_assert(dac_ru_select(MMX_BF16, false, 0, 48, 9)->launch == launch_dac_ru<48, 128, 4, 1, 1, 2, false> && dac_ru_select(MMX_BF16, false, 0, 96, 9)->launch == launch_dac_ru<96, 256, 2, 2, 1, 3, false>);
static_assert(dac_ru_select(MMX_BF16, false, 0, 192, 3)->launch == launch_dac_ru<192, 64, 1, 4, 1, 2, false> && dac_ru_select(MMX_BF16, false, 0, 192, 9)->launch == launch_dac_ru<192, 32, 1, 4, 1, 2, false>);
static_assert(dac_ru_select(MMX_X2, false, 0, 48, 9)->launch == launch_dac_ru<48, 64, 4, 1, 2, 2, false> && dac_ru_select(MMX_X2, false, 0, 192, 9)->launch == launch_dac_ru<192, 32, 1, 4, 2, 2, false>);
static_assert(dac_ru_select(MMX_X2, false, 0, 96, 3)->launch == launch_dac_ru<96, 64, 2, 2, 2, 3, false> && dac_ru_select(MMX_X2, false, 0, 96, 9)->launch == launch_dac_ru<96, 128, 2, 2, 2, 3, false>);
static_assert(dac_ru_select(MMX_X2, true, 0, 48, 9)->launch == launch_dac_ru<48, 64, 4, 1, 2, 2, true> && dac_ru_select(MMX_X2, true, 0, 192, 9)->launch == launch_dac_ru<192, 32, 1, 4, 2, 2, true>);
static_assert(dac_ru_select(MMX_X2, true, 0, 96, 3)->launch == launch_dac_ru<96, 64, 2, 2, 2, 3, true> && dac_ru_select(MMX_X2, true, 0, 96, 9)->launch == launch_dac_ru<96, 128, 2, 2, 2, 3, true>);
static_assert(dac_ru_select(MMX_BF16, false, 0, 64, 1)->launch == launch_dac_ru<64, 128, 4, 1, 1, 2, false> && dac_ru_select(MMX_BF16, false, 0, 128, 9)->launch == launch_dac_ru<128, 128, 2, 2, 1, 2, false>);
static_assert(dac_ru_select(MMX_X2, false, 0, 64, 9)->launch == launch_dac_ru<64, 64, 4, 1, 2, 2, false> && dac_ru_select(MMX_X2, false, 0, 128, 9)->launch == launch_dac_ru<128, 64, 2, 2, 2, 2, false>);
static_assert(dac_ru_select(MMX_X2, true, 0, 64, 1) == nullptr && dac_ru_select(MMX_X2, true, 0, 128, 1) == nullptr);

}

#if MMX_LAB
extern "C" int mmx_lab_tail_stamps(void* buf) {
    unsigned long long* p = reinterpret_cast<unsigned long long*>(buf);
    const hipError_t e = hipMemcpyToSymbol(HIP_SYMBOL(g_tail_stamps), &p, sizeof(p));
    return e == hipSuccess ? MMX_OK : -(int)e - 1000;
}
#endif

extern "C" int mmx_est_tail(const MmxEstTailParams* pp, int dtype, int bm, int cfg, hipStream_t stream) {
    MMX_CHECK_ARG(pp != nullptr);
    const MmxEstTailParams& p = *pp;
    const bool wplanes = dtype == MMX_X2W;
    if (wplanes) dtype = MMX_X2;
    MMX_CHECK_ARG(p.ao && p.x && p.wo && p.w1 && p.w2 && p.bo && p.b1 && p.b2 && p.n3g && p.n3b && p.B > 0 && p.T > 0);
    MMX_CHECK_ARG(p.t_begin >= 0 && p.t_begin < p.T && p.t_begin % 16 == 0);
    MMX_CHECK_ARG(p.ldao >= 512 && p.ldao % (dtype == MMX_X2 ? 4 : 8) == 0 && p.ao_bs % (dtype == MMX_X2 ? 4 : 8) == 0 && p.x_bs % 4 == 0);
    MMX_CHECK_ARG(((uintptr_t)p.ao % 16) == 0 && ((uintptr_t)p.x % 16) == 0);
    MMX_CHECK_ARG(!p.act_out || (p.act_ld % (dtype == MMX_X2 ? 4 : 8) == 0 && p.act_bs % (dtype == MMX_X2 ? 4 : 8) == 0 && ((uintptr_t)p.act_out % 16) == 0));
    if (int rc = check_next(p.next, dtype, p.T)) return rc;
    const TailForm* form = tail_select(dtype, wplanes, bm, cfg);
    return form ? form->launch(p, stream) : MMX_EARG;
}

extern "C" int mmx_est_resnet(const MmxEstResnetParams* pp, int dtype, int bm, int cfg, hipStream_t stream) {
    MMX_CHECK_ARG(pp != nullptr);
    const MmxEstResnetParams& p = *pp;
    const bool wplanes = dtype == MMX_X2W;
    if (wplanes) dtype = MMX_X2;
    MMX_CHECK_ARG(p.a_in && p.x && p.w1 && p.w2 && p.wr && p.b1 && p.b2 && p.br && p.g1 && p.be1 && p.g2 && p.be2 && p.tv);
    MMX_CHECK_ARG(p.t_begin >= 0 && p.t_begin < p.T && p.t_begin % 16 == 0);
    MMX_CHECK_ARG(p.B > 0 && p.T > 0 && p.cin >= 64 && p.cin % 32 == 0 && p.cin <= 512 && p.lda >= p.cin);
    MMX_CHECK_ARG(p.lda % (dtype == MMX_X2 ? 4 : 8) == 0 && p.a_bs % (dtype == MMX_X2 ? 4 : 8) == 0);
    MMX_CHECK_ARG(((uintptr_t)p.a_in % 16) == 0 && ((uintptr_t)p.x % 16) == 0 && p.x_bs % 4 == 0 && p.tv_bs % 4 == 0 && ((uintptr_t)p.tv % 16) == 0);
    if (int rc = check_next(p.next, dtype, p.T)) return rc;
    const ResnetForm* form = resnet_select(dtype, wplanes, bm, cfg, p.cin);
    return form ? form->launch(p, stream) : MMX_EARG;
}

extern "C" int mmx_dac_ru(const MmxDacRuParams* pp, int dtype, int bm, hipStream_t stream) {
    MMX_CHECK_ARG(pp != nullptr);
    const MmxDacRuParams& p = *pp;
    MMX_CHECK_ARG(p.x && (p.x_out || p.act_out) && p.x != p.x_out && p.w7 && p.w1 && p.b7 && p.b1 && p.a0 && p.a2 && p.B > 0 && p.T > 0);
    MMX_CHECK_ARG(p.dil >= 1 && p.dil <= 9 && (p.C == 48 || p.C == 64 || p.C == 96 || p.C == 128 || p.C == 192) && p.x_bs % 4 == 0 && p.x_bs >= (int64_t)p.T * p.C);
    MMX_CHECK_ARG(((uintptr_t)p.x % 16) == 0 && ((uintptr_t)p.x_out % 16) == 0 && ((uintptr_t)p.act_out % 16) == 0 && ((uintptr_t)p.a0 % 16) == 0);
    MMX_CHECK_ARG(!p.act_out || p.alpha_next);
    const bool wplanes = dtype == MMX_X2W;
    const DacRuForm* form = dac_ru_select(wplanes ? MMX_X2 : dtype, wplanes, bm, p.C, p.dil);
    return form ? form->launch(p, stream) : MMX_EARG;
}
```

### minimax-speech_amd/mmx/_lib.py

```python
import ctypes as C
import os

import torch

F32, BF16 = 0, 1
X2, X3 = 2, 3
X2W, X3W = 0x12, 0x13
H2, H2W = 4, 0x14
DA_PACKED, DA_PER_HEAD, DA_SPLIT, DA_H2, DA_ONE_HEAD = 1, 2, 4, 8, 16
ACT = {"none": 0, "lrelu": 1, "gelu": 2, "silu": 3, "mish": 4, "tanh": 5}
TORCH_DT = {F32: torch.float32, BF16: torch.bfloat16, X2: torch.float32, X3: torch.float32, X2W: torch.float32, X3W: torch.float32}
WEIGHT_DT = {F32: torch.float32, BF16: torch.bfloat16, X2: torch.bfloat16, X3: torch.bfloat16, X2W: torch.bfloat16, X3W: torch.bfloat16}
ESIZE = {F32: 4, BF16: 2, X2: 4, X3: 4}
WPLANES = {X2W: 2, X3W: 3}
DTYPE_NAMES = {"f32": F32, "bf16": BF16, "x": X2, "x2": X2, "x3": X3}


def is_split(dtype):
    return dtype in (X2, X3, X2W, X3W)

_HERE = os.path.dirname(os.path.abspath(__file__))
LIB_PATH = os.environ.get("MMX_LIB") or os.path.join(os.path.dirname(_HERE), "lib", "libmmx_hip.so")

SYMBOLS = [
    "mmx_abi_version", "mmx_gemm_win", "mmx_gemm_win_tile", "mmx_rownorm", "mmx_groupnorm", "mmx_act_rows", "mmx_gather_rows", "mmx_copy2d", "mmx_est_pack",
    "mmx_sinusoidal_emb", "mmx_cfg_euler", "mmx_attn_dense", "mmx_attn_flash_bf16", "mmx_attn_flash_fp8", "mmx_attn_relpos_bf16", "mmx_attn_relpos_x", "mmx_attn_flash_x", "mmx_attn_flash_xs", "mmx_conv_cout1_tanh", "mmx_conv_cin1", "mmx_vae_sample", "mmx_resample_linear", "mmx_prefetch4", "mmx_mask_rows",
    "mmx_est_tail", "mmx_est_resnet", "mmx_dac_ru", "mmx_pack_skinny", "mmx_skinny_gemm", "mmx_skinny2", "mmx_decode_prep", "mmx_rope_kv_store", "mmx_paged_attn", "mmx_decode_attn", "mmx_decode_attn_fin", "mmx_swiglu", "mmx_sample_step",
    "mmx_sample_step_tab", "mmx_logmel", "mmx_pool_rows", "mmx_logmel_w", "mmx_s3_rope_fsmn", "mmx_fsq_encode", "mmx_resample_sinc", "mmx_kweight_blocks", "mmx_loudness_gate", "mmx_scale_rows",
    "mmx_spec_dist", "mmx_wave_sums",
]


class GemmParams(C.Structure):
    _fields_ = [
        ("A", C.c_void_p), ("W", C.c_void_p), ("bias", C.c_void_p), ("residual", C.c_void_p),
        ("rowmask", C.c_void_p), ("alpha", C.c_void_p), ("out_f32", C.c_void_p), ("out_act", C.c_void_p),
        ("lda", C.c_int64), ("ldw", C.c_int64), ("ldr", C.c_int64), ("ldo_f", C.c_int64), ("ldo_a", C.c_int64),
        ("a_bstride", C.c_int64), ("w_bstride", C.c_int64), ("r_bstride", C.c_int64), ("rm_bstride", C.c_int64),
        ("of_bstride", C.c_int64), ("oa_bstride", C.c_int64),
        ("row_off", C.c_int64), ("row_lo", C.c_int64), ("row_hi", C.c_int64),
        ("out_off", C.c_int64), ("out_len", C.c_int64),
        ("M", C.c_int32), ("N", C.c_int32), ("batch", C.c_int32),
        ("ntaps", C.c_int32), ("cin", C.c_int32), ("dil", C.c_int32),
        ("bias_mod", C.c_int32), ("alpha_mod", C.c_int32), ("bias_per_row", C.c_int32),
        ("act", C.c_int32), ("act2", C.c_int32), ("slope", C.c_float), ("row_stride", C.c_int32),
    ]


class EstNext(C.Structure):
    _fields_ = [("wqkv", C.c_void_p), ("n1g", C.c_void_p), ("n1b", C.c_void_p), ("q_out", C.c_void_p), ("vt_out", C.c_void_p),
                ("q_bs", C.c_int64), ("vt_bs", C.c_int64), ("ldq", C.c_int32), ("ldvt", C.c_int32)]


class EstTailParams(C.Structure):
    _fields_ = [(k, C.c_void_p) for k in ("ao", "x", "wo", "w1", "w2", "bo", "b1", "b2", "n3g", "n3b", "rowmask", "act_out")] + \
               [(k, C.c_int64) for k in ("ao_bs", "x_bs", "rm_bs", "act_bs")] + \
               [(k, C.c_int32) for k in ("ldao", "act_ld", "B", "T", "t_begin")] + [("eps", C.c_float), ("next", EstNext)]


class EstResnetParams(C.Structure):
    _fields_ = [(k, C.c_void_p) for k in ("a_in", "x", "w1", "w2", "wr", "b1", "g1", "be1", "b2", "g2", "be2", "br", "tv", "rowmask")] + \
               [(k, C.c_int64) for k in ("a_bs", "x_bs", "tv_bs", "rm_bs")] + \
               [(k, C.c_int32) for k in ("lda", "cin", "B", "T", "t_begin")] + [("eps", C.c_float), ("next", EstNext)]


class DacRuParams(C.Structure):
    _fields_ = [(k, C.c_void_p) for k in ("x", "x_out", "act_out", "w7", "w1", "b7", "b1", "a0", "a2", "alpha_next", "lens")] + \
               [("x_bs", C.c_int64)] + [(k, C.c_int32) for k in ("B", "T", "C", "dil")] + [("slope", C.c_float)]


def fill_struct(st, **kw):
    for k, v in kw.items():
        if v is not None and hasattr(v, "data_ptr"):
            assert v.is_cuda
            v = v.data_ptr()
        setattr(st, k, v)
    return st


ABI_VERSION = 10
_lib = None


class MmxError(RuntimeError):
    pass


def load():
    global _lib
    if _lib is None:
        if not os.path.exists(LIB_PATH):
            raise MmxError(f"{LIB_PATH} not found: build it with `make -C minimax-speech_amd/csrc` "
                           "(or __graft_entry__.build()); the hot path has no CPU fallback")
        lib = C.CDLL(LIB_PATH)
        for s in SYMBOLS:
            getattr(lib, s).restype = C.c_int
        if lib.mmx_abi_version() != ABI_VERSION:
            raise MmxError(f"{LIB_PATH} has ABI version {lib.mmx_abi_version()}, this package binds version {ABI_VERSION}: "
                           "rebuild it (`make -C minimax-speech_amd/csrc`)")
        _lib = lib
    return _lib


def _p(t):
    if t is None:
        return None
    if isinstance(t, int):
        return C.c_void_p(t)
    assert t.is_cuda, "libmmx_hip works on device memory only (no CPU fallback)"
    return C.c_void_p(t.data_ptr())


def stream():
    return C.c_void_p(torch.cuda.current_stream().cuda_stream)


def check(rc, what):
    if rc != 0:
        raise MmxError(f"{what} failed with code {rc}" + (" (argument/shape error)" if rc == -1 else ""))


def dt_of(t):
    return BF16 if t.dtype == torch.bfloat16 else F32


def i64(x):
    return C.c_int64(int(x))


def gemm_params(**kw):
    p = GemmParams()
    p.bias_mod = 1
    p.alpha_mod = 1
    p.ntaps = 1
    p.dil = 1
    p.batch = 1
    p.row_lo = 0
    p.out_len = 1 << 62
    p.slope = 0.1
    p.row_stride = 1
    for k, v in kw.items():
        if k in ("A", "W", "bias", "residual", "rowmask", "alpha", "out_f32", "out_act"):
            v = None if v is None else (v if isinstance(v, int) else v.data_ptr())
        setattr(p, k, v)
    return p


TILES = {"auto": 0, "128x128": 1, "128x64": 2, "64x64": 3, "32x64": 4}


def gemm_win(p, dtype, tile=0):
    if tile:
        check(load().mmx_gemm_win_tile(C.byref(p), C.c_int(dtype), C.c_int(tile), stream()), "mmx_gemm_win_tile")
    else:
        check(load().mmx_gemm_win(C.byref(p), C.c_int(dtype), stream()), "mmx_gemm_win")
```

### minimax-speech_amd/mmx/flow.py

```python
import gc
import itertools
import math
from collections import OrderedDict
from typing import Dict, Optional

import torch

from . import ops
from ._lib import BF16, F32, TORCH_DT, WEIGHT_DT, X2, X2W, is_split


def espnet_rel_pe(T: int, d: int) -> torch.Tensor:
    pos = torch.arange(T - 1, -T, -1, dtype=torch.float32)[:, None]
    div = torch.exp(torch.arange(0, d, 2, dtype=torch.float32) * -(math.log(10000.0) / d))
    pe = torch.zeros(2 * T - 1, d)
    pe[:, 0::2] = torch.sin(pos * div)
    pe[:, 1::2] = torch.cos(pos * div)
    return pe


import threading

CAPTURE_LOCK = threading.RLock()


_capture_primed = {}


def _prime_capture_state(dev):
    key = torch.device(dev).index if torch.device(dev).index is not None else torch.cuda.current_device()
    if key in _capture_primed:
        return
    with torch.inference_mode(False):
        t = torch.zeros(1, device=f"cuda:{key}")
        g = torch.cuda.CUDAGraph()
        gc_was_on = gc.isenabled()
        gc.collect()
        gc.disable()
        try:
            with torch.cuda.graph(g, capture_error_mode="thread_local"):
                t.add_(1.0)
        finally:
            if gc_was_on:
                gc.enable()
    _capture_primed[key] = (g, t)


class Graphed:

    cold_calls = 0

    def __init__(self, fn, enabled=True):
        self.fn, self.enabled, self.graph, self.calls = fn, enabled, None, 0

    def release(self):
        g, self.graph, self.fn = self.graph, None, None
        if g is not None:
            with CAPTURE_LOCK:
                g.reset()
            del g

    def __call__(self):
        if not self.enabled:
            return self.fn()
        if self.graph is None:
            self.calls += 1
            Graphed.cold_calls += 1
            if self.calls == 1:
                return self.fn()
            with CAPTURE_LOCK:
                torch.cuda.current_stream().synchronize()
                _prime_capture_state(torch.cuda.current_device())
                g = torch.cuda.CUDAGraph()
                gc_was_on = gc.isenabled()
                gc.collect()
                gc.disable()
                try:
                    with torch.cuda.graph(g, capture_error_mode="thread_local"):
                        self.fn()
                finally:
                    if gc_was_on:
                        gc.enable()
                self.graph = g
        self.graph.replay()


class FlowEngine:
    def __init__(self, sd: Dict[str, torch.Tensor], dtype=BF16, device="cuda", n_timesteps=10, cfg_rate=0.7,
                 enc_chunk=25, est_chunk=50, pre_lookahead_len=3, use_graphs=True, parts=("encoder", "estimator"),
                 fused=None, attn="bf16", wplanes=False):
        self.dtype, self.tdt, self.dev = dtype, TORCH_DT[dtype], torch.device(device)
        self.wplanes = dtype == X2 and ops.resolve_wplanes(wplanes, (v for k, v in sd.items() if v.dim() >= 2 and v.is_floating_point()
                                                                     and k != "input_embedding.weight" and not k.endswith("rand_noise")))
        self.pdt = X2W if self.wplanes else dtype
        self.n_timesteps, self.cfg, self.L = n_timesteps, cfg_rate, pre_lookahead_len
        self.enc_chunk, self.est_chunk = enc_chunk, est_chunk
        self.use_graphs = use_graphs
        self.fused = fused
        self.split = is_split(dtype)
        assert attn in ("bf16", "fp8")
        self.attn_fp8 = attn == "fp8" and dtype == BF16
        dt = self.pdt
        f = lambda k: sd[k].detach().to(self.dev, torch.float32).contiguous()
        lin = lambda k: ops.pack_linear(f(k), dt)
        cv = lambda k: ops.pack_conv1d(f(k), dt)
        self._pe, self._plans, self._vt = OrderedDict(), OrderedDict(), {}
        self.plan_budget_bytes = 16 << 30
        self.shape_log = None
        self.polite = False
        self.polite_flash_form = getattr(FlowEngine, "polite_flash_form_default", 1)
        self.plan_bytes = 0
        self.rand_noise = torch.randn([1, 80, 50 * 300], generator=torch.Generator().manual_seed(0))
        self.spk_enc = None
        if "speaker_encoder.init.weight" in sd:
            from .spk import SpeakerEncoderEngine
            self.spk_enc = SpeakerEncoderEngine(sd, dtype=dtype, device=device, pack_dtype=self.pdt)
        if "encoder" in parts:
            self._init_encoder(sd, f, lin, cv)
        if "estimator" in parts:
            self._init_estimator(sd, f, lin, cv)

    def clone_shared(self):
        import copy
        c = copy.copy(self)
        c._plans, c._pe, c._vt, c.plan_bytes = OrderedDict(), OrderedDict(), {}, 0
        c._stream_pool = OrderedDict()
        return c

    def set_noise(self, noise: torch.Tensor):
        if noise is not self.rand_noise and not torch.equal(noise.cpu(), self.rand_noise):
            self.rand_noise = noise.detach().cpu().float()
            self.close()

    def _init_encoder(self, sd, f, lin, cv):
        flow_level = "input_embedding.weight" in sd
        if flow_level:
            self.emb_table = f("input_embedding.weight")
            self.spk_w, self.spk_b = lin("spk_embed_affine_layer.weight"), f("spk_embed_affine_layer.bias")
            self.spk_dim = sd["spk_embed_affine_layer.weight"].shape[1]
            self.spk_gamma = torch.full((self.spk_dim,), 1.0 / math.sqrt(self.spk_dim), device=self.dev)
        e = "encoder"
        xs = math.sqrt(512.0)

        def embed(p):
            return dict(w=lin(p + ".out.0.weight"), b=f(p + ".out.0.bias"), g=f(p + ".out.1.weight") * xs,
                        beta=f(p + ".out.1.bias") * xs)

        def conf_layer(p):
            a = p + ".self_attn"
            return dict(
                n1g=f(p + ".norm_mha.weight"), n1b=f(p + ".norm_mha.bias"),
                wqkv=ops.pack_linear(torch.cat([f(a + ".linear_q.weight"), f(a + ".linear_k.weight"), f(a + ".linear_v.weight")], 0), self.pdt),
                bqkv=torch.cat([f(a + ".linear_q.bias"), f(a + ".linear_k.bias"), f(a + ".linear_v.bias")], 0).contiguous(),
                wpos=lin(a + ".linear_pos.weight"), pu=f(a + ".pos_bias_u"), pv=f(a + ".pos_bias_v"),
                wo=lin(a + ".linear_out.weight"), bo=f(a + ".linear_out.bias"),
                n2g=f(p + ".norm_ff.weight"), n2b=f(p + ".norm_ff.bias"),
                w1=lin(p + ".feed_forward.w_1.weight"), b1=f(p + ".feed_forward.w_1.bias"),
                w2=lin(p + ".feed_forward.w_2.weight"), b2=f(p + ".feed_forward.w_2.bias"))

        self.enc = dict(embed=embed(e + ".embed"), up_embed=embed(e + ".up_embed"),
                        pl_w1=cv(e + ".pre_lookahead_layer.conv1.weight"), pl_b1=f(e + ".pre_lookahead_layer.conv1.bias"),
                        pl_w2=cv(e + ".pre_lookahead_layer.conv2.weight"), pl_b2=f(e + ".pre_lookahead_layer.conv2.bias"),
                        layers=[conf_layer(f"{e}.encoders.{i}") for i in range(6)],
                        up_w=cv(e + ".up_layer.conv.weight"), up_b=f(e + ".up_layer.conv.bias"),
                        up_layers=[conf_layer(f"{e}.up_encoders.{i}") for i in range(4)],
                        ang=f(e + ".after_norm.weight"), anb=f(e + ".after_norm.bias"))
        if flow_level:
            self.enc.update(wproj=lin("encoder_proj.weight"), bproj=f("encoder_proj.bias"))

    def _init_estimator(self, sd, f, lin, cv):
        dt = self.dtype
        q = "decoder.estimator"
        self.tdim = sd[q + ".time_mlp.linear_1.weight"].shape[1]
        self.t_w1, self.t_b1 = lin(q + ".time_mlp.linear_1.weight"), f(q + ".time_mlp.linear_1.bias")
        self.t_w2, self.t_b2 = lin(q + ".time_mlp.linear_2.weight"), f(q + ".time_mlp.linear_2.bias")

        def tblock(p):
            a = p + ".attn1"
            d = dict(n1g=f(p + ".norm1.weight"), n1b=f(p + ".norm1.bias"),
                     wo=lin(a + ".to_out.0.weight"), bo=f(a + ".to_out.0.bias"),
                     n3g=f(p + ".norm3.weight"), n3b=f(p + ".norm3.bias"),
                     w1=lin(p + ".ff.net.0.proj.weight"), b1=f(p + ".ff.net.0.proj.bias"),
                     w2=lin(p + ".ff.net.2.weight"), b2=f(p + ".ff.net.2.bias"))
            wq, wk, wv = f(a + ".to_q.weight"), f(a + ".to_k.weight"), f(a + ".to_v.weight")
            if self.fused is not False:
                pk = (lambda w: ops.pack_skinny(w.float().contiguous(), dtype=X2W)) if self.wplanes else \
                     (lambda w: ops.pack_skinny(w.to(WEIGHT_DT[dt]).contiguous(), dtype=dt))
                d.update(wo_p=pk(f(a + ".to_out.0.weight")), w1_p=pk(f(p + ".ff.net.0.proj.weight")),
                         w2_p=pk(f(p + ".ff.net.2.weight")), wqkv_p=pk(torch.cat([wq, wk, wv], 0)))
            if dt == BF16:
                d["wqk"] = ops.pack_linear(torch.cat([wq, wk], 0), dt)
                d["wv"] = ops.pack_linear(wv, dt)
            else:
                d["wqkv"] = ops.pack_linear(torch.cat([wq, wk, wv], 0), self.pdt)
            return d

        self.resnets, mlp_w, mlp_b = [], [], []

        def resnet(p):
            idx = len(self.resnets)
            r = dict(idx=idx, cin=sd[p + ".block1.block.0.weight"].shape[1],
                     w1=cv(p + ".block1.block.0.weight"), b1=f(p + ".block1.block.0.bias"),
                     g1=f(p + ".block1.block.2.weight"), be1=f(p + ".block1.block.2.bias"),
                     w2=cv(p + ".block2.block.0.weight"), b2=f(p + ".block2.block.0.bias"),
                     g2=f(p + ".block2.block.2.weight"), be2=f(p + ".block2.block.2.bias"),
                     wr=cv(p + ".res_conv.weight"), br=f(p + ".res_conv.bias"))
            if self.fused is not False:
                pc = (lambda k: ops.pack_skinny(ops.conv1d_matrix(f(k)).contiguous(), dtype=X2W)) if self.wplanes else \
                     (lambda k: ops.pack_skinny(ops.pack_conv1d(f(k), dt), dtype=dt))
                r.update(w1_p=pc(p + ".block1.block.0.weight"), w2_p=pc(p + ".block2.block.0.weight"), wr_p=pc(p + ".res_conv.weight"))
            mlp_w.append(f(p + ".mlp.1.weight"))
            mlp_b.append(f(p + ".mlp.1.bias"))
            self.resnets.append(r)
            return r

        def stage(p):
            return dict(res=resnet(p + ".0"), blocks=[tblock(f"{p}.1.{j}") for j in range(4)])

        self.n_mid = len({k.split(".")[3] for k in sd if k.startswith(q + ".mid_blocks.")})
        self.down = stage(q + ".down_blocks.0")
        self.down_w, self.down_b = cv(q + ".down_blocks.0.2.weight"), f(q + ".down_blocks.0.2.bias")
        self.mid = [stage(f"{q}.mid_blocks.{i}") for i in range(self.n_mid)]
        self.up = stage(q + ".up_blocks.0")
        self.up_w, self.up_b = cv(q + ".up_blocks.0.2.weight"), f(q + ".up_blocks.0.2.bias")
        self.fin_w, self.fin_b = cv(q + ".final_block.block.0.weight"), f(q + ".final_block.block.0.bias")
        self.fin_g, self.fin_be = f(q + ".final_block.block.2.weight"), f(q + ".final_block.block.2.bias")
        self.proj_w, self.proj_b = cv(q + ".final_proj.weight"), f(q + ".final_proj.bias")
        self.mlp_w = ops.pack_linear(torch.cat(mlp_w, 0), self.pdt)
        self.mlp_b = torch.cat(mlp_b, 0).contiguous()
        self.C = sd[q + ".final_proj.weight"].shape[1]

    def _new(self, *shape, f32=False):
        return torch.empty(*shape, dtype=torch.float32 if f32 else self.tdt, device=self.dev)

    def _pos(self, T):
        if T in self._pe:
            self._pe.move_to_end(T)
        else:
            self._pe[T] = espnet_rel_pe(T, 512).to(self.dev, self.tdt)
            while len(self._pe) > 64:
                self._pe.popitem(last=False)
        return self._pe[T]

    def _conformer(self, lw, x, T, chunk, pe=None, B=1, klen=None, keymask=None, qkv=None, pos=None, t0=0):
        dt, R = self.dtype, B * (T - t0)
        hn = self._new(R, 512)
        ops.rownorm(x, lw["n1g"], lw["n1b"], 1e-12, rows=R, C_=512, out_act=hn, dtype=dt)
        dense = qkv is not None or not (dt == BF16 or self.split)
        if pos is None:
            pos = self._new(2 * T - 1, 512)
            ops.linear(pe, lw["wpos"], 512, dtype=dt, out_act=pos)
        ao = self._new(B * T, 512)
        if dt == BF16 and not dense:
            qk = self._new(R, 1024)
            ops.linear(hn, lw["wqkv"][:1024], 512, dtype=dt, bias=lw["bqkv"][:1024], out_act=qk)
            Tp = ops.round_up(T, 8)
            vt = self._new(B, 512, Tp)
            if Tp > T:
                vt[:, :, T:].zero_()
            ops.gemm(lw["wqkv"][1024:], hn, 512, T, dtype=dt, lda=lw["wqkv"].shape[1], cin=512, batch=B, a_bstride=0,
                     w_bstride=T * 512, bias=lw["bqkv"][1024:], bias_per_row=True, out_act=vt, ldo_a=Tp, oa_bstride=512 * Tp)
            ops.attn_relpos_bf16(qk, qk[:, 512:], vt, pos, lw["pu"], lw["pv"], ao, B=B, H=8, T=T, ldq=1024, ldk=1024, ldvt=Tp,
                                 ldp=512, ldo=512, q_bs=T * 1024, k_bs=T * 1024, vt_bs=512 * Tp, o_bs=T * 512, scale=0.125,
                                 chunk=chunk, klen=klen)
        else:
            if qkv is None:
                qkv = self._new(R, 1536)
            ops.linear(hn, lw["wqkv"], 512, dtype=dt, bias=lw["bqkv"], out_act=qkv[t0:])
            if not dense:
                ops.attn_relpos_x(qkv, qkv[:, 512:], qkv[:, 1024:], pos, lw["pu"], lw["pv"], ao, B=B, H=8, T=T, ldq=1536, ldk=1536,
                                  ldv=1536, ldp=512, ldo=512, q_bs=T * 1536, k_bs=T * 1536, v_bs=T * 1536, o_bs=T * 512, scale=0.125,
                                  chunk=chunk, klen=klen)
            else:
                ops.attn_dense(qkv, qkv[:, 512:], qkv[:, 1024:], ao, B=B, H=8, Tq=T, Tk=T, ldq=1536, ldk=1536, ldv=1536, ldo=512,
                               q_bs=T * 1536, k_bs=T * 1536, v_bs=T * 1536, o_bs=T * 512, scale=0.125, dtype=dt, chunk=chunk, pos=pos,
                               ldp=512, pos_u=lw["pu"], pos_v=lw["pv"], keymask=keymask, q_begin=t0)
        x2 = self._new(R, 512, f32=True)
        ops.linear(ao[t0:], lw["wo"], 512, dtype=dt, bias=lw["bo"], residual=x, out_f32=x2)
        ops.rownorm(x2, lw["n2g"], lw["n2b"], 1e-12, rows=R, C_=512, out_act=hn, dtype=dt)
        ff = self._new(R, 2048)
        ops.linear(hn, lw["w1"], 512, dtype=dt, bias=lw["b1"], act="silu", out_act=ff)
        x3 = self._new(R, 512, f32=True)
        ops.linear(ff, lw["w2"], 2048, dtype=dt, bias=lw["b2"], residual=x2, out_f32=x3)
        return x3

    def _embed(self, ew, a, T, rowmask=None):
        dt = self.dtype
        tmp = self._new(T, 512, f32=True)
        ops.linear(a, ew["w"], 512, dtype=dt, bias=ew["b"], out_f32=tmp)
        x = self._new(T, 512, f32=True)
        xa = self._new(T, 512)
        ops.rownorm(tmp, ew["g"], ew["beta"], 1e-5, rows=T, C_=512, out_f32=x, out_act=xa, dtype=dt, rowmask=rowmask)
        return x, xa

    def encode(self, ids: torch.Tensor, finalize: bool, streaming: bool) -> torch.Tensor:
        Lt = ids.numel()
        a0 = self._new(Lt, 512)
        ops.gather_rows(ids, self.emb_table, out_act=a0, dtype=self.dtype)
        return self.encode_embedded(a0, finalize, streaming)

    def encode_embedded(self, a0: torch.Tensor, finalize: bool, streaming: bool, hidden=False) -> torch.Tensor:
        Lt = a0.shape[0]
        return self._encode(a0, 1, Lt if finalize else Lt - self.L, self.enc_chunk if streaming else 0, hidden=hidden)[0]

    def encode_batch(self, ids_list) -> list:
        B = len(ids_list)
        lens = [int(i.numel()) for i in ids_list]
        if B == 1:
            return [self.encode(ids_list[0].reshape(-1), True, False)]
        T = max(lens)
        ids = torch.zeros(B, T, dtype=torch.int64, device=self.dev)
        for b, i in enumerate(ids_list):
            ids[b, :lens[b]] = i.reshape(-1)
        a0 = self._new(B * T, 512)
        ops.gather_rows(ids.reshape(-1), self.emb_table, out_act=a0, dtype=self.dtype)
        mu = self._encode(a0, B, T, lens=torch.tensor(lens, dtype=torch.int32, device=self.dev))
        return [mu[b, :2 * lens[b]] for b in range(B)]

    def _encode(self, a0, B, T, chunk=0, lens=None, hidden=False):
        dt, E = self.dtype, self.enc
        Lt, T2 = a0.shape[0] // B, 2 * T
        mask = mask2 = klen2 = None
        if lens is not None:
            ar = torch.arange(T2, device=self.dev)
            mask = (ar[None, :T] < lens[:, None]).float().contiguous()
            mask2 = (ar[None, :] < 2 * lens[:, None]).float().contiguous()
            klen2 = (2 * lens).contiguous()
        x_all, xa_all = self._embed(E["embed"], a0, B * Lt, rowmask=(None if mask is None else mask.reshape(-1)))
        h1 = self._new(B * T, 512)
        ops.gemm(xa_all, E["pl_w1"], T, 512, dtype=dt, lda=512, cin=512, ntaps=4, row_off=0, row_lo=0, row_hi=Lt, batch=B,
                 a_bstride=Lt * 512, bias=E["pl_b1"], act="lrelu", slope=0.01, out_act=h1, ldo_a=512, oa_bstride=T * 512)
        x = self._new(B * T, 512, f32=True)
        ops.conv1d(h1, E["pl_w2"], T=T, Cin=512, k=3, pad_left=2, dtype=dt, batch=B, bias=E["pl_b2"], residual=x_all, out_f32=x)
        pe = self._pos(T)
        for lw in E["layers"]:
            x = self._conformer(lw, x, T, chunk, pe, B=B, klen=lens, keymask=mask)
        up = self._new(B * T2, 512)
        ops.copy2d(x, F32, T * 512, 512, 1, up, dt, T2 * 512, 512, 1, rows=T2, cols=512, batch=B, rep=2)
        c5 = self._new(B * T2, 512)
        ops.conv1d(up, E["up_w"], T=T2, Cin=512, k=5, pad_left=4, dtype=dt, batch=B, bias=E["up_b"], out_act=c5)
        x, _ = self._embed(E["up_embed"], c5, B * T2)
        pe = self._pos(T2)
        for lw in E["up_layers"]:
            x = self._conformer(lw, x, T2, 2 * chunk, pe, B=B, klen=klen2, keymask=mask2)
        hn = self._new(B * T2, 512)
        hf = self._new(B, T2, 512, f32=True) if hidden else None
        ops.rownorm(x, E["ang"], E["anb"], 1e-5, rows=B * T2, C_=512, out_f32=hf, out_act=hn, dtype=dt)
        if hidden:
            return hf
        mu = self._new(B, T2, 80, f32=True)
        ops.linear(hn, E["wproj"], 512, dtype=dt, bias=E["bproj"], out_f32=mu)
        return mu

    def _enc_stream_state(self, st):
        if st.enc is None:
            E, dt = self.enc, self.dtype
            Tt, Tf = st.Tcap // 2 + self.L, st.Tcap
            z = lambda *sh, f32=False: torch.zeros(*sh, dtype=torch.float32 if f32 else self.tdt, device=self.dev)

            def pos_tables(layers, T):
                pe = espnet_rel_pe(T, 512).to(self.dev, self.tdt)
                out = []
                for lw in layers:
                    p = z(2 * T - 1, 512)
                    ops.linear(pe, lw["wpos"], 512, dtype=dt, out_act=p)
                    out.append(p)
                return out

            st.enc = dict(T=0, xa=z(Tt, 512), x=z(Tt, 512, f32=True), h1=z(Tt, 512), up=z(Tf, 512), mu=z(Tf, 80, f32=True),
                          qkv=[z(Tt, 1536) for _ in E["layers"]], qkv2=[z(Tf, 1536) for _ in E["up_layers"]],
                          pos=pos_tables(E["layers"], Tt), pos2=pos_tables(E["up_layers"], Tf), Tt=Tt, Tf=Tf)
        return st.enc

    def _encode_stream_rows(self, st, ids: torch.Tensor, tb: int, Lt: int):
        dt, E, S = self.dtype, self.enc, self._enc_stream_state(st)
        T = Lt - self.L
        assert tb < T and Lt <= S["Tt"]
        a0 = self._new(Lt - tb, 512)
        ops.gather_rows(ids[tb:], self.emb_table, out_act=a0, dtype=dt)
        tmp = self._new(Lt - tb, 512, f32=True)
        ops.linear(a0, E["embed"]["w"], 512, dtype=dt, bias=E["embed"]["b"], out_f32=tmp)
        ops.rownorm(tmp, E["embed"]["g"], E["embed"]["beta"], 1e-5, rows=Lt - tb, C_=512, out_f32=S["x"][tb:Lt], out_act=S["xa"][tb:Lt], dtype=dt)
        n = T - tb
        ops.gemm(S["xa"], E["pl_w1"], n, 512, dtype=dt, lda=512, cin=512, ntaps=4, row_off=tb, row_lo=0, row_hi=Lt,
                 bias=E["pl_b1"], act="lrelu", slope=0.01, out_act=S["h1"][tb:T], ldo_a=512)
        x = self._new(n, 512, f32=True)
        ops.gemm(S["h1"], E["pl_w2"], n, 512, dtype=dt, lda=512, cin=512, ntaps=3, row_off=tb - 2, row_lo=0, row_hi=T,
                 bias=E["pl_b2"], residual=S["x"][tb:T], ldr=512, out_f32=x, ldo_f=512)
        for lw, qkv, pos in zip(E["layers"], S["qkv"], S["pos"]):
            x = self._conformer(lw, x, T, self.enc_chunk, qkv=qkv, pos=pos[S["Tt"] - T:], t0=tb)
        f0, F = 2 * tb, 2 * T
        ops.copy2d(x, F32, 0, 512, 1, S["up"][f0:F], dt, 0, 512, 1, rows=F - f0, cols=512, rep=2)
        c5 = self._new(F - f0, 512)
        ops.gemm(S["up"], E["up_w"], F - f0, 512, dtype=dt, lda=512, cin=512, ntaps=5, row_off=f0 - 4, row_lo=0, row_hi=F,
                 bias=E["up_b"], out_act=c5, ldo_a=512)
        x, _ = self._embed(E["up_embed"], c5, F - f0)
        for lw, qkv, pos in zip(E["up_layers"], S["qkv2"], S["pos2"]):
            x = self._conformer(lw, x, F, 2 * self.enc_chunk, qkv=qkv, pos=pos[S["Tf"] - F:], t0=f0)
        hn = self._new(F - f0, 512)
        ops.rownorm(x, E["ang"], E["anb"], 1e-5, rows=F - f0, C_=512, out_act=hn, dtype=dt)
        ops.linear(hn, E["wproj"], 512, dtype=dt, bias=E["bproj"], out_f32=S["mu"][f0:F])

    def _resnet(self, r, a_in, lda, B, T, tv, mask, out_x):
        dt, C = self.dtype, self.C
        cin = r["cin"]
        c1 = self._new(B, T, C, f32=True)
        kw = dict(dtype=dt, lda=lda, cin=cin, ntaps=3, row_off=-2, row_lo=0, row_hi=T, batch=B, a_bstride=T * lda)
        ops.gemm(a_in, r["w1"], T, C, bias=r["b1"], out_f32=c1, ldo_f=C, of_bstride=T * C, **kw)
        h1 = self._new(B, T, C)
        ops.rownorm(c1, r["g1"], r["be1"], 1e-5, rows=T, C_=C, batch=B, act="mish", rowmask=mask,
                    addvec=tv[:, r["idx"] * C:], av_bstride=tv.shape[1], out_act=h1, dtype=dt)
        ops.conv1d(h1, r["w2"], T=T, Cin=C, k=3, pad_left=2, dtype=dt, batch=B, bias=r["b2"], out_f32=c1)
        h2 = self._new(B, T, C, f32=True)
        ops.rownorm(c1, r["g2"], r["be2"], 1e-5, rows=T, C_=C, batch=B, act="mish", rowmask=mask, out_f32=h2, dtype=dt)
        ops.gemm(a_in, r["wr"], T, C, dtype=dt, lda=lda, cin=cin, ntaps=1, row_lo=0, row_hi=T, batch=B, a_bstride=T * lda,
                 bias=r["br"], residual=h2, ldr=C, r_bstride=T * C, out_f32=out_x, ldo_f=C, of_bstride=T * C)

    def _tblock(self, w, x, B, T, mask, chunk, act_out=None, act_ld=0, klen=None):
        dt, C = self.dtype, self.C
        hn = self._new(B, T, C)
        ops.rownorm(x, w["n1g"], w["n1b"], 1e-5, rows=T, C_=C, batch=B, out_act=hn, dtype=dt)
        ao = self._new(B, T, 512)
        qk, vt = self._attn_bufs(B, T, presplit=False)
        ld = qk.shape[-1]
        ops.gemm(hn, w["wqkv"] if vt is None else w["wqk"], T, ld, dtype=dt, lda=C, cin=C, batch=B, a_bstride=T * C, out_act=qk,
                 ldo_a=ld, oa_bstride=T * ld)
        if vt is not None:
            ops.gemm(w["wv"], hn, 512, T, dtype=dt, lda=w["wv"].shape[1], cin=C, batch=B, a_bstride=0, w_bstride=T * C,
                     out_act=vt, ldo_a=vt.shape[-1], oa_bstride=512 * vt.shape[-1])
        self._attention(qk, vt, ao, B=B, T=T, chunk=chunk, mask=mask, klen=(None if dt == BF16 else klen))
        ops.gemm(ao, w["wo"], T, C, dtype=dt, lda=512, cin=512, batch=B, a_bstride=T * 512, bias=w["bo"], residual=x,
                 ldr=C, r_bstride=T * C, out_f32=x, ldo_f=C, of_bstride=T * C)
        ops.rownorm(x, w["n3g"], w["n3b"], 1e-5, rows=T, C_=C, batch=B, out_act=hn, dtype=dt)
        ff = self._new(B, T, 1024)
        ops.gemm(hn, w["w1"], T, 1024, dtype=dt, lda=C, cin=C, batch=B, a_bstride=T * C, bias=w["b1"], act="gelu",
                 out_act=ff, ldo_a=1024, oa_bstride=T * 1024)
        ops.gemm(ff, w["w2"], T, C, dtype=dt, lda=1024, cin=1024, batch=B, a_bstride=T * 1024, bias=w["b2"], residual=x,
                 ldr=C, r_bstride=T * C, out_f32=x, ldo_f=C, of_bstride=T * C,
                 rowmask=(mask if act_out is not None else None), rm_bstride=T,
                 out_act=act_out, ldo_a=act_ld, oa_bstride=T * act_ld)

    def _attn_layout(self, presplit):
        if self.dtype == BF16:
            return 1024, self.tdt, 1
        if self.split and presplit:
            return 2048, torch.bfloat16, 2
        return 1536, self.tdt, 0

    def _attn_bufs(self, B, T, presplit):
        ld, qdt, planes = self._attn_layout(presplit)
        qk = torch.empty(B, T, ld, dtype=qdt, device=self.dev)
        if not planes:
            return qk, None
        key = (B, ops.round_up(T, 8), planes)
        if key not in self._vt:
            self._vt[key] = torch.zeros(B, planes * 512, key[1], dtype=torch.bfloat16, device=self.dev)
        return qk, self._vt[key]

    def _attention(self, qk, vt, ao, *, B, T, chunk, mask=None, klen=None, q_begin=0, fp8=False, form=0):
        ld, Tc = qk.shape[-1], qk.shape[1]
        km = None if klen is not None else mask
        kw = dict(B=B, H=8, ldo=512, o_bs=Tc * 512, scale=0.125, chunk=chunk, q_begin=q_begin)
        if vt is None and not self.split:
            ops.attn_dense(qk, qk[:, :, 512:], qk[:, :, 1024:], ao, Tq=T, Tk=T, ldq=ld, ldk=ld, ldv=ld, q_bs=Tc * ld, k_bs=Tc * ld,
                           v_bs=Tc * ld, dtype=self.dtype, keymask=mask, **kw)
        elif vt is None:
            ops.attn_flash_x(qk, qk[:, :, 512:], qk[:, :, 1024:], ao, T=T, ldq=ld, ldk=ld, ldv=ld, q_bs=Tc * ld, k_bs=Tc * ld,
                             v_bs=Tc * ld, keymask=km, klen=klen, **kw)
        elif self.split:
            ops.attn_flash_xs(qk, vt, ao, T=T, ldqk=ld, ldvt=vt.shape[-1], qk_bs=Tc * ld, vt_bs=vt[0].numel(), keymask=km,
                              klen=klen, form=form, **kw)
        else:
            ops.attn_flash_bf16(qk, qk[:, :, 512:], vt, ao, T=T, ldq=ld, ldk=ld, ldvt=vt.shape[-1], q_bs=Tc * ld, k_bs=Tc * ld,
                                vt_bs=vt[0].numel(), keymask=km, fp8=fp8, klen=klen, **kw)

    def _time_mlp(self, t, B):
        dt = self.dtype
        te = self._new(B, self.tdim)
        ops.sinusoidal_emb(t, te, dim=self.tdim, dtype=dt)
        t1 = self._new(B, 1024)
        ops.linear(te, self.t_w1, self.tdim, dtype=dt, bias=self.t_b1, act="silu", out_act=t1)
        t2 = self._new(B, 1024)
        ops.linear(t1, self.t_w2, 1024, dtype=dt, bias=self.t_b2, act2="mish", out_act=t2)
        tv = self._new(B, self.mlp_w.shape[0], f32=True)
        ops.linear(t2, self.mlp_w, 1024, dtype=dt, bias=self.mlp_b, out_f32=tv)
        return tv

    def estimator(self, x, x_bstride, mu, spks, cond, t, B, T, mask=None, streaming=False, out=None, x_mod=None, klen=None):
        C, chunk = self.C, (self.est_chunk if streaming else 0)
        tv = self._time_mlp(t, B)
        a = self._new(B, T, C)
        S = dict(h0=self._new(B, T, 320), cat=self._new(B, T, 2 * C), amid=[a] * len(self.mid), aup=a, a2=self._new(B, T, C),
                 c1=self._new(B, T, C, f32=True), afin=a, d=(self._new(B, T, 80, f32=True) if out is None else out),
                 xs=self._new(B, T, C, f32=True))
        ops.est_pack(x, mu, spks, cond, S["h0"], B=B, T=T, dtype=self.dtype, x_bstride=x_bstride, x_mod=(x_mod or B))
        if self.fused or (self.fused is None and (self.dtype == BF16 or self.split or B * ((T + 15) // 16) >= 256)):
            S["ao"] = self._new(B, T, 512)
            self._estimator_rows(S, tv, B, T, chunk, itertools.repeat(self._attn_bufs(B, T, presplit=True)), mask=mask,
                                 klen=klen, fp8=self.attn_fp8, form=(self.polite_flash_form if self.polite else 0))
            return S["d"]

        def stage(sw, a_in, lda, act_out, act_ld):
            self._resnet(sw["res"], a_in, lda, B, T, tv, mask, S["xs"])
            for j, w in enumerate(sw["blocks"]):
                last = j == len(sw["blocks"]) - 1
                self._tblock(w, S["xs"], B, T, mask, chunk, act_out=(act_out if last else None), act_ld=act_ld, klen=klen)

        self._walk(stage, S, B, T, mask)
        return S["d"]

    def _walk(self, stage, S, B, T, mask=None, r0=0, Tc=None):
        dt, C, Tc = self.dtype, self.C, Tc or T
        assert mask is None or r0 == 0

        def conv3(src, ld, w, b, rowmask, out_act=None, out_f32=None):
            N = w.shape[0]
            ops.gemm(src, w, T - r0, N, dtype=dt, lda=ld, cin=C, ntaps=3, row_off=r0 - 2, row_lo=0, row_hi=T, batch=B,
                     a_bstride=Tc * ld, bias=b, rowmask=rowmask, rm_bstride=Tc, out_act=(None if out_act is None else out_act[:, r0:]),
                     ldo_a=N, oa_bstride=Tc * N, out_f32=(None if out_f32 is None else out_f32[:, r0:]), ldo_f=N, of_bstride=Tc * N)

        stage(self.down, S["h0"], 320, S["cat"][:, :, C:], 2 * C)
        conv3(S["cat"][:, :, C:], 2 * C, self.down_w, self.down_b, mask, out_act=S["amid"][0])
        for i, sw in enumerate(self.mid):
            last = i == len(self.mid) - 1
            stage(sw, S["amid"][i], C, S["cat"] if last else S["amid"][i + 1], 2 * C if last else C)
        stage(self.up, S["cat"], 2 * C, S["aup"], C)
        conv3(S["aup"], C, self.up_w, self.up_b, mask, out_act=S["a2"])
        conv3(S["a2"], C, self.fin_w, self.fin_b, None, out_f32=S["c1"])
        ops.rownorm(S["c1"][:, r0:], self.fin_g, self.fin_be, 1e-5, rows=T - r0, C_=C, batch=B, x_bstride=Tc * C, act="mish",
                    rowmask=mask, out_act=S["afin"][:, r0:], o_bstride=Tc * C, dtype=dt)
        ops.gemm(S["afin"][:, r0:], self.proj_w, T - r0, 80, dtype=dt, lda=C, cin=C, row_hi=T - r0, batch=B, a_bstride=Tc * C,
                 bias=self.proj_b, rowmask=mask, rm_bstride=Tc, out_f32=S["d"][:, r0:], ldo_f=80, of_bstride=Tc * 80)

    _WG_US = {16: 27.1, 32: 29.9, 64: 44.1}
    _WG_US_X = {16: 29.1, 32: 35.8, 64: 60.3}
    _WG_US_XW = {16: 46.9, 32: 52.6, 64: 81.2}

    @classmethod
    def _launch_us(cls, bm, tiles, split=False):
        wg = (cls._WG_US_XW if split == "w" else cls._WG_US_X if split else cls._WG_US)[bm]
        t = lambda n: wg * (1.0 + 0.45 * (n / 256.0) ** 2)
        full, rem = divmod(tiles, 256)
        return full * t(256) + (t(rem) if rem else 0.0)

    def _tile_rows(self, B, T):
        tiles = lambda bm: B * ((T + bm - 1) // bm)
        if self.dtype == BF16:
            cap = getattr(self, "max_tile_rows", 64)
            bm = min((b for b in (64, 32, 16) if b <= cap), key=lambda b: (self._launch_us(b, tiles(b)), -b))
            bm = max(bm, getattr(self, "min_tile_rows", 16), 64 if self.polite else 16)
            return bm, bm
        if self.split:
            cap = getattr(self, "max_tile_rows", 64)
            bm = min((b for b in (64, 32, 16) if b <= cap), key=lambda b: (self._launch_us(b, tiles(b), "w" if self.wplanes else True), -b))
            if self.polite:
                bm = max(bm, min(cap, 64))
            br = 32 if (tiles(32) >= 128 or self.polite) else 16
            return bm, br
        return (32 if tiles(32) >= 128 else 16), 16

    def _estimator_rows(self, S, tv, B, T, chunk, attn_bufs, mask=None, klen=None, r0=0, Tc=None, fp8=False, form=0):
        dt, C, Tc = self.dtype, self.C, Tc or T
        bm_t, bm_r = self._tile_rows(B, T - r0)
        ntv = tv.shape[1]

        def nxt(w, qk, vt):
            return ops.est_next(wqkv=w["wqkv_p"], n1g=w["n1g"], n1b=w["n1b"], q_out=qk, ldq=qk.shape[-1], q_bs=Tc * qk.shape[-1],
                                vt_out=vt, ldvt=(0 if vt is None else vt.shape[-1]), vt_bs=(0 if vt is None else vt[0].numel()))

        def stage(sw, a_in, lda, act_out, act_ld):
            r, blocks = sw["res"], sw["blocks"]
            bufs = [next(attn_bufs) for _ in blocks]
            ops.est_resnet(a_in, lda, lda, S["xs"], r, tv[:, r["idx"] * C:], ntv, B=B, T=T, dtype=dt,
                           bm=(16 if (self.split and lda > 320) else bm_r), rowmask=mask, nxt=nxt(blocks[0], *bufs[0]),
                           t_begin=r0, Tcap=Tc)
            for j, w in enumerate(blocks):
                last = j == len(blocks) - 1
                self._attention(*bufs[j], S["ao"], B=B, T=T, chunk=chunk, mask=mask, klen=klen, q_begin=r0, fp8=fp8, form=form)
                ops.est_tail(S["ao"], S["xs"], w, B=B, T=T, dtype=dt, bm=bm_t, rowmask=(mask if last else None),
                             act_out=(act_out if last else None), act_ld=act_ld,
                             nxt=(None if last else nxt(blocks[j + 1], *bufs[j + 1])), t_begin=r0, Tcap=Tc)

        self._walk(stage, S, B, T, mask, r0, Tc)

    class StreamState:

        def __init__(self, eng, Tcap):
            self.eng, self.Tcap, self.T = eng, ops.round_up(Tcap, 64), 0
            self.steps = [None] * eng.n_timesteps
            self.lat = torch.zeros(self.Tcap, 80, device=eng.dev)
            Tc, new = self.Tcap, eng._new
            self.xs, self.c1 = new(2, Tc, eng.C, f32=True), new(2, Tc, eng.C, f32=True)
            self.ao, self.afin, self.d = new(2, Tc, 512), new(2, Tc, eng.C), new(2, Tc, 80, f32=True)
            tt, dd = eng.t_schedule()
            self.t_all = torch.tensor([[v, v] for v in tt], dtype=torch.float32, device=eng.dev)
            self.dt = dd
            self.enc = None
            self.tok_done = 0
            self.z = eng.rand_noise[0, :, :self.Tcap].t().contiguous().to(eng.dev)
            self.cond = torch.zeros(self.Tcap, 80, device=eng.dev)
            self.spks2 = torch.zeros(2, 80, device=eng.dev)
            self.ids = torch.zeros(self.Tcap // 2 + eng.L + 8, dtype=torch.int64, device=eng.dev)
            self.graphs, self._win = {}, {}
            self.busy = False

        def release(self):
            for g in self.graphs.values():
                g.release()
            self.graphs, self._win, self.steps, self.enc = {}, {}, [None] * self.eng.n_timesteps, None

        def window(self, n):
            if n not in self._win:
                d = self.eng.dev
                self._win[n] = dict(x=torch.zeros(1, n, 80, device=d), mu2=torch.zeros(2, n, 80, device=d),
                                    cond2=torch.zeros(2, n, 80, device=d))
            return self._win[n]

        def reset(self):
            self.T = self.tok_done = 0

        def step_buffers(self, s):
            if self.steps[s] is None:
                e, Tc = self.eng, self.Tcap
                z = lambda *sh, dtype=e.tdt: torch.zeros(*sh, dtype=dtype, device=e.dev)
                nblk = 4 * (2 + len(e.mid))
                ldq, qdt, planes = e._attn_layout(presplit=False)
                self.steps[s] = dict(h0=z(2, Tc, 320), amid=[z(2, Tc, e.C) for _ in e.mid], cat=z(2, Tc, 2 * e.C), aup=z(2, Tc, e.C),
                                     a2=z(2, Tc, e.C), qk=[z(2, Tc, ldq, dtype=qdt) for _ in range(nblk)],
                                     vt=[z(2, planes * 512, Tc, dtype=torch.bfloat16) if planes else None for _ in range(nblk)],
                                     xs=self.xs, ao=self.ao, c1=self.c1, afin=self.afin, d=self.d)
            return self.steps[s]

    stream_cap_frames = 4096
    stream_budget_bytes = 24 << 30

    def _stream_state_bytes(self, cap):
        per_frame = 0.36e6 * (1 if self.dtype == BF16 else 2)
        return int(cap * per_frame)

    def stream_open(self, max_frames: int) -> "FlowEngine.StreamState":
        cap = min(ops.round_up(max(max_frames, 1), 512), ops.round_up(self.stream_cap_frames, 64))
        if not hasattr(self, "_stream_pool") or not isinstance(self._stream_pool, OrderedDict):
            self._stream_pool = OrderedDict()
        for key, st in self._stream_pool.items():
            if st.Tcap == cap and not st.busy:
                self._stream_pool.move_to_end(key)
                break
        else:
            self._stream_evict(self._stream_state_bytes(cap))
            st = FlowEngine.StreamState(self, cap)
            self._stream_pool[id(st)] = st
        st.busy = True
        st.reset()
        return st

    def stream_close(self, st):
        st.busy = False
        self._stream_evict(0)

    def _stream_evict(self, incoming):
        pool = getattr(self, "_stream_pool", None)
        if not pool:
            return
        total = sum(self._stream_state_bytes(s_.Tcap) for s_ in pool.values()) + incoming
        for key in list(pool):
            if total <= self.stream_budget_bytes:
                break
            if not pool[key].busy:
                total -= self._stream_state_bytes(pool[key].Tcap)
                pool.pop(key).release()

    def _cfm_stream_rows(self, st, tb: int, T: int):
        assert tb < T <= st.Tcap and tb % self.est_chunk == 0 and T % self.est_chunk == 0, (tb, T, st.Tcap)
        n = T - tb
        W = st.window(n)
        W["x"].copy_(st.z[tb:T].reshape(1, n, 80))
        W["mu2"][0].copy_(st.enc["mu"][tb:T])
        W["cond2"][0].copy_(st.cond[tb:T])
        for s in range(self.n_timesteps):
            S = st.step_buffers(s)
            tv = self._time_mlp(st.t_all[s], 2)
            h0w = self._new(2, n, 320)
            ops.est_pack(W["x"], W["mu2"], st.spks2, W["cond2"], h0w, B=2, T=n, dtype=self.dtype, x_bstride=n * 80, x_mod=1)
            S["h0"][:, tb:T].copy_(h0w)
            self._estimator_rows(S, tv, 2, T, self.est_chunk, zip(S["qk"], S["vt"]), r0=tb // 16 * 16, Tc=st.Tcap)
            ops.cfg_euler(W["x"], S["d"][0, tb:T], S["d"][1, tb:T], self.cfg, st.dt[s], n * 80)
        st.lat[tb:T].copy_(W["x"][0])

    @torch.no_grad()
    def stream_hop(self, st, ids: torch.Tensor, embedding: torch.Tensor, prompt_feat: Optional[torch.Tensor] = None) -> torch.Tensor:
        Lt = ids.numel()
        T, tb = Lt - self.L, st.tok_done
        if tb == 0:
            st.cond.zero_()
            if prompt_feat is not None and prompt_feat.shape[0]:
                st.cond[:prompt_feat.shape[0]].copy_(prompt_feat.to(self.dev, torch.float32))
            st.spks2.zero_()
            en = self._new(1, self.spk_dim)
            ops.rownorm(embedding.to(self.dev, torch.float32).contiguous(), self.spk_gamma, None, 1e-30, rows=1, C_=self.spk_dim,
                        rms=True, out_act=en, dtype=self.dtype)
            ops.linear(en, self.spk_w, self.spk_dim, dtype=self.dtype, bias=self.spk_b, out_f32=st.spks2[0:1])
        self._enc_stream_state(st)
        st.ids[:Lt].copy_(ids.reshape(-1))
        key = (tb, Lt)
        if key not in st.graphs:
            def hop(tb=tb, Lt=Lt, T=T):
                self._encode_stream_rows(st, st.ids[:Lt], tb, Lt)
                self._cfm_stream_rows(st, 2 * tb, 2 * T)
            st.graphs[key] = Graphed(hop, self.use_graphs)
        st.graphs[key]()
        st.tok_done = T
        st.T = 2 * T
        return st.lat[:2 * T]

    @torch.no_grad()
    def estimator_channels_first(self, x, mask, mu, t, spks, cond, streaming=False):
        B, _, T = x.shape
        tm = lambda a: self._to_time_major(a.to(self.dev, torch.float32).contiguous(), B, T)
        m = mask.to(self.dev, torch.float32).reshape(B, T).contiguous()
        d = self.estimator(tm(x), T * 80, tm(mu), spks.to(self.dev, torch.float32).contiguous(), tm(cond),
                           t.to(self.dev, torch.float32).contiguous(), B, T, m, streaming)
        out = torch.empty(B, 80, T, dtype=torch.float32, device=self.dev)
        ops.copy2d(d, F32, T * 80, 80, 1, out, F32, 80 * T, 1, T, rows=T, cols=80, batch=B)
        return out

    def _to_time_major(self, a, B, T):
        o = torch.empty(B, T, 80, dtype=torch.float32, device=self.dev)
        ops.copy2d(a, F32, 80 * T, 1, T, o, F32, T * 80, 80, 1, rows=T, cols=80, batch=B)
        return o

    def t_schedule(self):
        n = self.n_timesteps
        ts = torch.linspace(0, 1, n + 1, dtype=torch.float32)
        ts = 1 - torch.cos(ts * 0.5 * torch.pi)
        t, dt = ts[0:1].clone(), ts[1] - ts[0]
        tt, dd = [], []
        for step in range(1, n + 1):
            tt.append(float(t))
            dd.append(float(dt))
            t = t + dt
            if step < n:
                dt = ts[step + 1] - t
        return tt, dd

    class _Plan:
        pass

    def _cfm_plan(self, n, T, streaming, masked):
        key = ("cfm", n, T, bool(streaming), bool(masked), bool(self.polite))
        if key in self._plans:
            self._plans.move_to_end(key)
            return self._plans[key]
        P = FlowEngine._Plan()
        P.nbytes = 2 * n * T * (16 << 10)
        while self._plans and self.plan_bytes + P.nbytes > self.plan_budget_bytes:
            _, old = self._plans.popitem(last=False)
            self._release_plan(old)
        self.plan_bytes += P.nbytes
        P.x = self._new(n, T, 80, f32=True)
        P.mu = torch.zeros(2 * n, T, 80, device=self.dev)
        P.spks = torch.zeros(2 * n, 80, device=self.dev)
        P.cond = torch.zeros(2 * n, T, 80, device=self.dev)
        P.mask = torch.ones(2 * n, T, device=self.dev) if masked else None
        P.klen = torch.full((2 * n,), T, dtype=torch.int32, device=self.dev) if masked else None
        P.d = self._new(2 * n, T, 80, f32=True)
        tt, dd = self.t_schedule()
        P.t_all = torch.tensor([[v] * (2 * n) for v in tt], dtype=torch.float32, device=self.dev)
        P.z = self.rand_noise[0, :, :T].t().contiguous().to(self.dev)

        def run():
            P.x.copy_(P.z.unsqueeze(0).expand(n, T, 80))
            for s in range(self.n_timesteps):
                self.estimator(P.x, T * 80, P.mu, P.spks, P.cond, P.t_all[s], 2 * n, T, P.mask, streaming, out=P.d, x_mod=n, klen=P.klen)
                ops.cfg_euler(P.x, P.d[:n], P.d[n:], self.cfg, dd[s], n * T * 80)

        P.run = Graphed(run, self.use_graphs)
        self._plans[key] = P
        return P

    def _release_plan(self, P):
        self.plan_bytes -= P.nbytes
        P.run.release()
        P.__dict__.clear()

    def close(self):
        while self._plans:
            _, old = self._plans.popitem(last=False)
            self._release_plan(old)
        pool = getattr(self, "_stream_pool", None) or {}
        for key in list(pool):
            pool.pop(key).release()

    def cfm_batch(self, mus, spks, conds, streaming=False, pad_to=1):
        n = len(mus)
        Ts = [m.shape[0] for m in mus]
        T = ops.round_up(max(Ts), pad_to)
        masked = any(t != T for t in Ts)
        if self.shape_log is not None:
            self.shape_log.append((n, T, sum(Ts), sum(t * t for t in Ts), bool(self.polite)))
        P = self._cfm_plan(n, T, streaming, masked)
        if masked:
            P.mu[:n].zero_()
            P.cond[:n].zero_()
            P.mask.zero_()
        for i in range(n):
            P.mu[i, :Ts[i]].copy_(mus[i])
            P.cond[i, :Ts[i]].copy_(conds[i])
            P.spks[i].copy_(spks[i].reshape(-1))
            if masked:
                P.mask[i, :Ts[i]] = 1.0
                P.mask[n + i, :Ts[i]] = 1.0
        if masked:
            P.klen.copy_(torch.tensor(list(Ts) * 2, dtype=torch.int32), non_blocking=False)
        P.run()
        return [P.x[i, :Ts[i]] for i in range(n)]

    def cfm(self, mu, spks, cond, streaming=False) -> torch.Tensor:
        return self.cfm_batch([mu], [spks], [cond], streaming, pad_to=(2 * self.est_chunk if streaming else 1))[0]

    @torch.no_grad()
    def inference_time_major(self, token, prompt_token, prompt_feat, embedding, streaming=False, finalize=True,
                             reference_mels=None, stream_state=None):
        Lt, Lp, Tp = token.numel(), prompt_token.numel(), prompt_feat.shape[1]
        La = Lp + Lt
        if (stream_state is not None and streaming and not finalize and Tp == 2 * Lp
                and reference_mels is None and (2 * (La - self.L)) % self.est_chunk == 0 and 2 * (La - self.L) <= stream_state.Tcap
                and stream_state.tok_done < La - self.L):
            ids = torch.cat([prompt_token.reshape(-1), token.reshape(-1)]).to(self.dev, torch.int64)
            return self.stream_hop(stream_state, ids, embedding, prompt_feat[0] if Tp else None)[Tp:]
        mu, spks, cond, mel_len1 = self.conditions(token, prompt_token, prompt_feat, embedding, streaming, finalize, reference_mels)
        x = self.cfm(mu, spks, cond, streaming)
        return x[mel_len1:]

    @torch.no_grad()
    def conditions(self, token, prompt_token, prompt_feat, embedding, streaming=False, finalize=True, reference_mels=None):
        dt = self.dtype
        if reference_mels is not None and self.spk_enc is not None:
            emb = self.spk_enc.reference_embedding(reference_mels)
        else:
            emb = embedding.to(self.dev, torch.float32).contiguous()
        en = self._new(1, self.spk_dim)
        ops.rownorm(emb, self.spk_gamma, None, 1e-30, rows=1, C_=self.spk_dim, rms=True, out_act=en, dtype=dt)
        spks = self._new(1, 80, f32=True)
        ops.linear(en, self.spk_w, self.spk_dim, dtype=dt, bias=self.spk_b, out_f32=spks)
        ids = torch.cat([prompt_token.reshape(-1), token.reshape(-1)]).to(self.dev, torch.int64)
        mu = self.encode(ids, finalize, streaming)
        T = mu.shape[0]
        mel_len1 = prompt_feat.shape[1]
        cond = torch.zeros(T, 80, device=self.dev)
        if mel_len1:
            cond[:mel_len1].copy_(prompt_feat[0].to(self.dev, torch.float32))
        return mu, spks, cond, mel_len1

    def conditions_batch(self, tokens, prompt_tokens, prompt_feats, embeddings):
        dt, n = self.dtype, len(tokens)
        emb = torch.cat([e.to(self.dev, torch.float32).reshape(1, -1) for e in embeddings], 0).contiguous()
        en = self._new(n, self.spk_dim)
        ops.rownorm(emb, self.spk_gamma, None, 1e-30, rows=n, C_=self.spk_dim, rms=True, out_act=en, dtype=dt)
        spks = self._new(n, 80, f32=True)
        ops.linear(en, self.spk_w, self.spk_dim, dtype=dt, bias=self.spk_b, out_f32=spks)
        ids = [torch.cat([p.reshape(-1), t.reshape(-1)]).to(self.dev, torch.int64) for p, t in zip(prompt_tokens, tokens)]
        mus = self.encode_batch(ids)
        out = []
        for b in range(n):
            T, L1 = mus[b].shape[0], prompt_feats[b].shape[1]
            cond = torch.zeros(T, 80, device=self.dev)
            if L1:
                cond[:L1].copy_(prompt_feats[b][0].to(self.dev, torch.float32))
            out.append((mus[b], spks[b:b + 1], cond, L1))
        return out

    @torch.no_grad()
    def inference(self, token, prompt_token, prompt_feat, embedding, streaming=False, finalize=True, reference_mels=None):
        x = self.inference_time_major(token, prompt_token, prompt_feat, embedding, streaming, finalize, reference_mels)
        T2 = x.shape[0]
        out = torch.empty(1, 80, T2, dtype=torch.float32, device=self.dev)
        ops.copy2d(x, F32, 0, 80, 1, out, F32, 0, 1, T2, rows=T2, cols=80)
        return out
```

### minimax-speech_amd/mmx/ops.py

```python
import ctypes as C
import math

import torch

from . import _lib as L
from ._lib import ACT, BF16, F32, check, i64, load, stream, _p


def round_up(x, m):
    return (x + m - 1) // m * m


class Planed(torch.Tensor):
    """A packed weight held as bf16 PLANES hi + [mid +] lo = w of an fp32 checkpoint's values (include/mmx_hip.h MMX_X2W / MMX_X3W).
    The type is the marker: gemm() / skinny2() switch to the weight-plane dtype code when they are handed one; views and row
    slices keep the type (torch's default __torch_function__)."""


def weight_planes(w: torch.Tensor, n: int):
    out, r = [], w.float()
    for _ in range(n):
        t = r.to(torch.bfloat16)
        out.append(t)
        r = r - t.float()
    return out


def resolve_wplanes(wplanes, weights) -> bool:
    if wplanes != "auto":
        return bool(wplanes)
    for w in weights:
        w = w.detach().float()
        if bool(((w - w.to(torch.bfloat16).float()).abs() > 2.0 ** -16 * w.abs()).any()):
            return True
    return False


def pack_linear(w: torch.Tensor, dtype) -> torch.Tensor:
    N, K = w.shape
    Kp = round_up(K, 32)
    planes = L.WPLANES.get(dtype, 1)
    out = torch.zeros(N, planes * Kp, dtype=L.WEIGHT_DT[dtype], device=w.device)
    if planes == 1:
        out[:, :K] = w
        return out
    for i, t in enumerate(weight_planes(w, planes)):
        out[:, i * Kp:i * Kp + K] = t
    return out.as_subclass(Planed)


def conv1d_matrix(w: torch.Tensor) -> torch.Tensor:
    Cout, Cin, k = w.shape
    return w.permute(0, 2, 1).reshape(Cout, k * Cin)


def pack_conv1d(w: torch.Tensor, dtype) -> torch.Tensor:
    return pack_linear(conv1d_matrix(w), dtype)


def pack_convtranspose1d(w: torch.Tensor, stride: int, dtype) -> torch.Tensor:
    Cin, Cout, k = w.shape
    s = stride
    assert k == 2 * s
    wk = w.permute(2, 1, 0)
    tap0 = wk[s:2 * s]
    tap1 = wk[0:s]
    g = torch.cat([tap0, tap1], dim=2)
    return pack_linear(g.reshape(s * Cout, 2 * Cin), dtype)


def fold_weight_norm(g, v):
    n = v.reshape(v.shape[0], -1).norm(dim=1).reshape(-1, *([1] * (v.dim() - 1)))
    return g * (v / n)


def gemm(A, W, M, N, *, dtype, lda=None, cin=None, ntaps=1, dil=1, row_off=0, row_lo=0, row_hi=None, batch=1,
         a_bstride=0, w_bstride=0, bias=None, bias_mod=None, bias_per_row=False, act="none", act2="none", slope=0.1,
         residual=None, ldr=0, r_bstride=0, rowmask=None, rm_bstride=0, alpha=None, alpha_mod=None,
         out_f32=None, ldo_f=0, of_bstride=0, out_act=None, ldo_a=0, oa_bstride=0, out_off=0, out_len=None, row_stride=1,
         tile=0):
    ldw = W.shape[-1] if hasattr(W, "shape") else None
    assert ldw is not None
    if isinstance(W, Planed):
        dtype = {L.X2: L.X2W, L.X3: L.X3W, L.X2W: L.X2W, L.X3W: L.X3W}[dtype]
    elif dtype in L.WPLANES:
        raise L.MmxError("a weight-plane dtype needs a Planed weight (ops.pack_linear with X2W / X3W)")
    p = L.gemm_params(A=A, W=W, bias=bias, residual=residual, rowmask=rowmask, alpha=alpha, out_f32=out_f32,
                      out_act=out_act, lda=lda, ldw=ldw, ldr=ldr, ldo_f=ldo_f, ldo_a=ldo_a,
                      a_bstride=a_bstride, w_bstride=w_bstride, r_bstride=r_bstride, rm_bstride=rm_bstride,
                      of_bstride=of_bstride, oa_bstride=oa_bstride, row_off=row_off, row_lo=row_lo,
                      row_hi=(row_hi if row_hi is not None else (1 << 40)), out_off=out_off,
                      out_len=(out_len if out_len is not None else (1 << 62)), M=M, N=N, batch=batch,
                      ntaps=ntaps, cin=cin, dil=dil, bias_mod=(bias_mod or N), alpha_mod=(alpha_mod or N),
                      bias_per_row=int(bias_per_row), act=ACT[act], act2=ACT[act2], slope=slope, row_stride=row_stride)
    L.gemm_win(p, dtype, tile)


def linear(x, Wp, K, *, dtype, bias=None, act="none", act2="none", residual=None, rowmask=None, out_f32=None,
           out_act=None):
    N = Wp.shape[0]
    M = x.numel() // x.shape[-1]
    gemm(x, Wp, M, N, dtype=dtype, lda=x.shape[-1], cin=K, bias=bias, act=act, act2=act2,
         residual=residual, ldr=N, rowmask=rowmask, out_f32=out_f32, ldo_f=N, out_act=out_act, ldo_a=N)


def conv1d(x, Wp, *, T, Cin, k, dtype, dil=1, pad_left=0, batch=1, bias=None, act="none", slope=0.1, residual=None,
           rowmask=None, alpha=None, out_f32=None, out_act=None, T_out=None, act2="none", stride=1):
    Cout = Wp.shape[0]
    T_out = T if T_out is None else T_out
    gemm(x, Wp, T_out, Cout, dtype=dtype, lda=Cin, cin=Cin, ntaps=k, dil=dil, row_off=-pad_left, row_lo=0, row_hi=T, row_stride=stride,
         batch=batch, a_bstride=T * Cin, bias=bias, act=act, act2=act2, slope=slope,
         residual=residual, ldr=Cout, r_bstride=T_out * Cout, rowmask=rowmask, rm_bstride=T_out,
         alpha=alpha, out_f32=out_f32, ldo_f=Cout, of_bstride=T_out * Cout,
         out_act=out_act, ldo_a=Cout, oa_bstride=T_out * Cout)


def convtranspose1d(x, Wp, *, T, Cin, Cout, stride, dtype, batch=1, bias=None, alpha=None, out_f32=None, out_act=None):
    s = stride
    pad = math.ceil(s / 2)
    gemm(x, Wp, T + 1, s * Cout, dtype=dtype, lda=Cin, cin=Cin, ntaps=2, dil=1, row_off=-1, row_lo=0, row_hi=T,
         batch=batch, a_bstride=T * Cin, bias=bias, bias_mod=Cout, alpha=alpha, alpha_mod=Cout,
         out_f32=out_f32, ldo_f=s * Cout, of_bstride=T * s * Cout, out_act=out_act, ldo_a=s * Cout,
         oa_bstride=T * s * Cout, out_off=-pad * Cout, out_len=T * s * Cout)


def rownorm(x, gamma, beta, eps, *, rows, C_, batch=1, x_bstride=None, rms=False, act="none", rowmask=None,
            addvec=None, av_bstride=None, out_f32=None, out_act=None, dtype=F32, ldx=None, o_bstride=None, rm_bstride=None):
    ldx = C_ if ldx is None else ldx
    xb = rows * ldx if x_bstride is None else x_bstride
    ob = rows * C_ if o_bstride is None else o_bstride
    check(load().mmx_rownorm(_p(x), i64(ldx), i64(xb), rows, C_, batch, _p(gamma), _p(beta), C.c_float(eps), int(rms),
                             ACT[act], _p(rowmask), i64(rows if rm_bstride is None else rm_bstride), _p(addvec),
                             i64(C_ if av_bstride is None else av_bstride), _p(out_f32), i64(C_), i64(ob), _p(out_act), i64(C_),
                             i64(ob), dtype, stream()), "mmx_rownorm")


def groupnorm(x, gamma, beta, out, *, B, T, C_, groups, dtype, eps=1e-5, act="none", rowmask=None):
    check(load().mmx_groupnorm(_p(x), B, T, C_, groups, _p(gamma), _p(beta), C.c_float(eps), ACT[act], _p(rowmask), _p(out),
                               dtype, stream()), "mmx_groupnorm")


def act_rows(x, *, rows, C_, act="none", rowmask=None, out_f32=None, out_act=None, dtype=F32):
    check(load().mmx_act_rows(_p(x), i64(rows), C_, ACT[act], _p(rowmask), _p(out_f32), _p(out_act), dtype, stream()),
          "mmx_act_rows")


def mask_rows(x, rowmask, *, rows, C_, dtype):
    check(load().mmx_mask_rows(_p(x), i64(rows), C_, _p(rowmask), dtype, stream()), "mmx_mask_rows")


def pool_rows(x, out, *, B, T, C_, dtype, mask=None):
    check(load().mmx_pool_rows(_p(x), i64(T * C_), T, C_, B, _p(mask), i64(T), _p(out), i64(C_), dtype, stream()), "mmx_pool_rows")


def gather_rows(ids, table, *, scale=1.0, rowmask=None, out_f32=None, out_act=None, dtype=F32, ldo_f=None, ldo_a=None):
    n, C_ = ids.numel(), table.shape[1]
    check(load().mmx_gather_rows(_p(ids), n, _p(table), C_, C.c_float(scale), _p(rowmask), _p(out_f32), i64(ldo_f or C_),
                                 _p(out_act), i64(ldo_a or C_), dtype, stream()), "mmx_gather_rows")


def copy2d(src, src_dt, ibs, irs, ics, dst, dst_dt, obs, ors, ocs, rows, cols, batch=1, rep=1):
    check(load().mmx_copy2d(_p(src), src_dt, i64(ibs), i64(irs), i64(ics), rep, _p(dst), dst_dt, i64(obs), i64(ors),
                            i64(ocs), rows, cols, batch, stream()), "mmx_copy2d")


def est_pack(x, mu, spks, cond, h, *, B, T, dtype, x_bstride=None, x_mod=None):
    check(load().mmx_est_pack(_p(x), i64(T * 80 if x_bstride is None else x_bstride), (B if x_mod is None else x_mod), _p(mu), _p(spks), _p(cond), B, T, 80, _p(h), i64(h.shape[-1]), dtype, stream()),
          "mmx_est_pack")


def sinusoidal_emb(t, out, *, dim, dtype, scale=1000.0):
    check(load().mmx_sinusoidal_emb(_p(t), t.numel(), dim, C.c_float(scale), _p(out), dtype, stream()),
          "mmx_sinusoidal_emb")


def cfg_euler(x, d_cond, d_uncond, cfg, dt, n):
    check(load().mmx_cfg_euler(_p(x), _p(d_cond), _p(d_uncond), C.c_float(cfg), C.c_float(dt), i64(n), stream()),
          "mmx_cfg_euler")


def conv_cin1(x, w, bias, *, T, C_, k, batch, dtype, slope=0.1, alpha=None, out_f32=None, out_act=None):
    check(load().mmx_conv_cin1(_p(x), i64(T), T, C_, k, _p(w), _p(bias), C.c_float(slope), _p(alpha), _p(out_f32), _p(out_act),
                               batch, dtype, stream()), "mmx_conv_cin1")


def vae_sample(ml, noise, z, m, logs, *, rows, D):
    check(load().mmx_vae_sample(_p(ml), _p(noise), i64(rows), D, _p(z), _p(m), _p(logs), stream()), "mmx_vae_sample")


def prefetch4(tensors, sink, workgroups=128):
    t = list(tensors) + [None] * (4 - len(tensors))
    nb = lambda x: 0 if x is None else (x.numel() * x.element_size()) // 16 * 16
    check(load().mmx_prefetch4(_p(t[0]), i64(nb(t[0])), _p(t[1]), i64(nb(t[1])), _p(t[2]), i64(nb(t[2])), _p(t[3]), i64(nb(t[3])),
                               _p(sink), workgroups, stream()), "mmx_prefetch4")


def resample_linear(x, T2):
    x = x.contiguous()
    T = x.shape[-1]
    out = torch.empty(*x.shape[:-1], T2, dtype=torch.float32, device=x.device)
    check(load().mmx_resample_linear(_p(x), i64(x.numel() // T), T, T2, _p(out), stream()), "mmx_resample_linear")
    return out


def conv_cout1_tanh(act, w, bias, out, *, T, C_, k, batch, dtype, slope=0.1, use_tanh=True):
    check(load().mmx_conv_cout1_tanh(_p(act), i64(T * C_), T, C_, k, _p(w), _p(bias), C.c_float(slope), int(use_tanh),
                                     _p(out), i64(T), batch, dtype, stream()), "mmx_conv_cout1_tanh")


def est_next(wqkv=None, n1g=None, n1b=None, q_out=None, ldq=0, q_bs=0, vt_out=None, ldvt=0, vt_bs=0):
    return L.fill_struct(L.EstNext(), wqkv=wqkv, n1g=n1g, n1b=n1b, q_out=q_out, vt_out=vt_out, q_bs=q_bs, vt_bs=vt_bs,
                         ldq=ldq, ldvt=ldvt)


def est_tail(ao, x, w, *, B, T, dtype, bm, rowmask=None, act_out=None, act_ld=0, nxt=None, eps=1e-5, pf=0, t_begin=0,
             Tcap=None, waves=0, narrow=False, ldao=512):
    Tc = T if Tcap is None else Tcap
    p = L.fill_struct(L.EstTailParams(), ao=ao, x=x, wo=w["wo_p"], w1=w["w1_p"], w2=w["w2_p"], bo=w["bo"], b1=w["b1"],
                      b2=w["b2"], n3g=w["n3g"], n3b=w["n3b"], rowmask=rowmask, act_out=act_out, ao_bs=Tc * ldao,
                      x_bs=Tc * 256, rm_bs=Tc, act_bs=Tc * act_ld, ldao=ldao, act_ld=act_ld, B=B, T=T, t_begin=t_begin, eps=eps)
    if nxt is not None:
        p.next = nxt
    if isinstance(w["wo_p"], Planed):
        dtype = L.X2W
    check(load().mmx_est_tail(C.byref(p), C.c_int(dtype), C.c_int(bm), C.c_int(pf + 16 * waves + (512 if narrow else 0)), stream()),
          "mmx_est_tail")


def est_resnet(a_in, lda, cin, x, r, tv, tv_bs, *, B, T, dtype, bm, rowmask=None, nxt=None, eps=1e-5, pf=0, t_begin=0,
               Tcap=None, waves=0):
    Tc = T if Tcap is None else Tcap
    p = L.fill_struct(L.EstResnetParams(), a_in=a_in, x=x, w1=r["w1_p"], w2=r["w2_p"], wr=r["wr_p"], b1=r["b1"], g1=r["g1"],
                      be1=r["be1"], b2=r["b2"], g2=r["g2"], be2=r["be2"], br=r["br"], tv=tv, rowmask=rowmask,
                      a_bs=Tc * lda, x_bs=Tc * 256, tv_bs=tv_bs, rm_bs=Tc, lda=lda, cin=cin, B=B, T=T, t_begin=t_begin, eps=eps)
    if nxt is not None:
        p.next = nxt
    if isinstance(r["w1_p"], Planed):
        dtype = L.X2W
    check(load().mmx_est_resnet(C.byref(p), C.c_int(dtype), C.c_int(bm), C.c_int(pf + 16 * waves), stream()), "mmx_est_resnet")


def pack_dac_ru(w7: torch.Tensor, w1: torch.Tensor, dtype):
    C_ = w7.shape[0]
    CP = (C_ + 31) // 32 * 32
    wd = torch.float32 if dtype in L.WPLANES else L.WEIGHT_DT[dtype]
    a = torch.zeros(C_, 7, CP, dtype=torch.float32, device=w7.device)
    a[:, :, :C_] = w7.permute(0, 2, 1)
    b = torch.zeros(C_, CP, dtype=torch.float32, device=w7.device)
    b[:, :C_] = w1[:, :, 0]
    return (pack_skinny(a.reshape(C_, 7 * CP).to(wd).contiguous(), dtype=dtype), pack_skinny(b.to(wd).contiguous(), dtype=dtype))


def dac_ru(x, x_out, ru, *, B, T, C_, dil, dtype, act_out=None, alpha_next=None, lens=None, bm=0, slope=0.1, x_bs=None):
    p = L.fill_struct(L.DacRuParams(), x=x, x_out=x_out, act_out=act_out, w7=ru["w7_p"], w1=ru["w1_p"], b7=ru["b7"], b1=ru["b1"],
                      a0=ru["a0"], a2=ru["a2"], alpha_next=alpha_next, lens=lens, x_bs=(T * C_ if x_bs is None else x_bs),
                      B=B, T=T, C=C_, dil=dil, slope=slope)
    if isinstance(ru["w7_p"], Planed):
        dtype = L.X2W
    check(load().mmx_dac_ru(C.byref(p), C.c_int(dtype), C.c_int(bm), stream()), "mmx_dac_ru")


def attn_dense(q, k, v, out, *, B, H, Tq, Tk, ldq, ldk, ldv, ldo, q_bs, k_bs, v_bs, o_bs, scale, dtype,
               keymask=None, chunk=0, pos=None, ldp=0, pos_u=None, pos_v=None, head_stride=0, q_begin=0, km_bs=None):
    check(load().mmx_attn_dense(_p(q), i64(ldq), i64(q_bs), _p(k), i64(ldk), i64(k_bs), _p(v), i64(ldv), i64(v_bs),
                                _p(out), i64(ldo), i64(o_bs), B, H, 64, Tq, Tk, C.c_float(scale), _p(keymask),
                                i64(Tk if km_bs is None else km_bs), chunk, _p(pos), i64(ldp), _p(pos_u), _p(pos_v), head_stride,
                                q_begin, dtype, stream()),
          "mmx_attn_dense")


def attn_relpos_bf16(q, k, vt, pos, pos_u, pos_v, out, *, B, H, T, ldq, ldk, ldvt, ldp, ldo, q_bs, k_bs, vt_bs, o_bs, scale, chunk=0,
                     klen=None):
    if klen is not None:
        assert klen.dtype == torch.int32 and klen.numel() >= B
    check(load().mmx_attn_relpos_bf16(_p(q), i64(ldq), i64(q_bs), _p(k), i64(ldk), i64(k_bs), _p(vt), i64(ldvt), i64(vt_bs),
                                      _p(pos), i64(ldp), _p(pos_u), _p(pos_v), _p(out), i64(ldo), i64(o_bs), B, H, T,
                                      C.c_float(scale), chunk, _p(klen), stream()), "mmx_attn_relpos_bf16")


def attn_relpos_x(q, k, v, pos, pos_u, pos_v, out, *, B, H, T, ldq, ldk, ldv, ldp, ldo, q_bs, k_bs, v_bs, o_bs, scale, chunk=0, klen=None):
    if klen is not None:
        assert klen.dtype == torch.int32 and klen.numel() >= B
    check(load().mmx_attn_relpos_x(_p(q), i64(ldq), i64(q_bs), _p(k), i64(ldk), i64(k_bs), _p(v), i64(ldv), i64(v_bs), _p(pos), i64(ldp),
                                   _p(pos_u), _p(pos_v), _p(out), i64(ldo), i64(o_bs), B, H, T, C.c_float(scale), chunk, _p(klen), stream()),
          "mmx_attn_relpos_x")


def attn_flash_bf16(q, k, vt, out, *, B, H, T, ldq, ldk, ldvt, ldo, q_bs, k_bs, vt_bs, o_bs, scale, keymask=None,
                    chunk=0, q_begin=0, km_bs=None, fp8=False, klen=None):
    if klen is not None:
        assert klen.dtype == torch.int32 and klen.numel() >= B
    if fp8:
        check(load().mmx_attn_flash_fp8(_p(q), i64(ldq), i64(q_bs), _p(k), i64(ldk), i64(k_bs), _p(vt), i64(ldvt),
                                        i64(vt_bs), _p(out), i64(ldo), i64(o_bs), B, H, T, C.c_float(scale),
                                        _p(keymask), i64(T if km_bs is None else km_bs), chunk, q_begin, _p(klen), stream()), "mmx_attn_flash_fp8")
        return
    check(load().mmx_attn_flash_bf16(_p(q), i64(ldq), i64(q_bs), _p(k), i64(ldk), i64(k_bs), _p(vt), i64(ldvt),
                                     i64(vt_bs), _p(out), i64(ldo), i64(o_bs), B, H, T, C.c_float(scale),
                                     _p(keymask), i64(T if km_bs is None else km_bs), chunk, q_begin, _p(klen), stream()), "mmx_attn_flash_bf16")


def attn_flash_x(q, k, v, out, *, B, H, T, ldq, ldk, ldv, ldo, q_bs, k_bs, v_bs, o_bs, scale, keymask=None, chunk=0, q_begin=0,
                 km_bs=None, klen=None):
    if klen is not None:
        assert klen.dtype == torch.int32 and klen.numel() >= B
    check(load().mmx_attn_flash_x(_p(q), i64(ldq), i64(q_bs), _p(k), i64(ldk), i64(k_bs), _p(v), i64(ldv), i64(v_bs),
                                  _p(out), i64(ldo), i64(o_bs), B, H, T, C.c_float(scale), _p(keymask),
                                  i64(T if km_bs is None else km_bs), chunk, q_begin, _p(klen), stream()), "mmx_attn_flash_x")


def attn_flash_xs(qk, vt, out, *, B, H, T, ldqk, ldvt, ldo, qk_bs, vt_bs, o_bs, scale, keymask=None, chunk=0, q_begin=0, km_bs=None,
                  klen=None, form=0):
    if klen is not None:
        assert klen.dtype == torch.int32 and klen.numel() >= B
    check(load().mmx_attn_flash_xs(_p(qk), i64(ldqk), i64(qk_bs), _p(vt), i64(ldvt), i64(vt_bs), _p(out), i64(ldo), i64(o_bs), B, H, T,
                                   C.c_float(scale), _p(keymask), i64(T if km_bs is None else km_bs), chunk, q_begin, _p(klen), int(form),
                                   stream()), "mmx_attn_flash_xs")


def pack_skinny(w, *, dtype, kscale=None, interleave_half=0):
    N, K = w.shape
    if dtype in L.WPLANES:
        assert w.dtype == torch.float32 and kscale is None
        base = {L.X2W: L.X2, L.X3W: L.X3}[dtype]
        return torch.cat([pack_skinny(t.contiguous(), dtype=base, interleave_half=interleave_half)
                          for t in weight_planes(w, L.WPLANES[dtype])]).as_subclass(Planed)
    assert w.dtype == L.WEIGHT_DT[dtype]
    KB = 32 if L.WEIGHT_DT[dtype] == torch.bfloat16 else 16
    tiles = (N + 15) // 16
    wp = torch.empty(tiles * (K // KB) * 64 * (KB // 4), dtype=L.WEIGHT_DT[dtype], device=w.device)
    check(load().mmx_pack_skinny(_p(w), i64(w.stride(0)), N, K, _p(kscale), interleave_half, _p(wp), dtype, stream()),
          "mmx_pack_skinny")
    return wp


X_PACKED, OUT_PACKED = 1, 2


def packed_rows(B):
    return (B + 15) // 16 * 16


def pack_act(x, dtype):
    E = 8 if dtype == BF16 else 4
    B, K = x.shape
    R = packed_rows(B)
    xp = torch.zeros(R, K, dtype=x.dtype, device=x.device)
    xp[:B] = x
    return xp.reshape(R // 16, 16, K // (4 * E), 4, E).permute(0, 2, 3, 1, 4).contiguous().reshape(-1)


def unpack_act(xp, B, K, dtype):
    E = 8 if dtype == BF16 else 4
    R = packed_rows(B)
    return xp.reshape(R // 16, K // (4 * E), 4, 16, E).permute(0, 3, 1, 2, 4).reshape(R, K)[:B]


def skinny_gemm(x, wp, *, B, K, N, dtype, bias=None, rs=False, eps=1e-6, epi=0, out_f32=None, out_act=None,
                ldx=None, ldo_f=None, ldo_a=None, x_packed=False, out_packed=False, kgamma=None):
    xdt = L.dt_of(x)
    flags = (X_PACKED if x_packed else 0) | (OUT_PACKED if out_packed else 0)
    check(load().mmx_skinny_gemm(_p(x), xdt, i64(ldx if ldx is not None else K), B, K, N, _p(wp), _p(bias), int(rs),
                                 C.c_float(eps), epi, _p(out_f32), i64(ldo_f if ldo_f is not None else N),
                                 _p(out_act), i64(ldo_a if ldo_a is not None else N), dtype, flags, _p(kgamma), stream()),
          "mmx_skinny_gemm")


SSQ_SLOTS = 64


def plane_elems(B, K):
    return packed_rows(B) * K


def split_planes(x, f16=False):
    B, K = x.shape
    out, r = [], x.float()
    for _ in range(2 if f16 else 3):
        t = r.to(torch.float16 if f16 else torch.bfloat16)
        out.append(pack_act(t.view(torch.bfloat16) if f16 else t, BF16))
        r = r - t.float()
    return torch.stack(out)


def merge_planes(xs, B, K, f16=False):
    if f16:
        return sum(unpack_act(xs[s], B, K, BF16).contiguous().view(torch.float16).float() for s in range(2))
    return sum(unpack_act(xs[s], B, K, BF16).float() for s in range(3))


H2_WSCALE = 256.0


def pack_skinny_h2(w, *, planes=1, interleave_half=0):
    ws = w.float() * H2_WSCALE
    assert float(ws.abs().max()) < 65504.0, "weight out of the fp16 range of MMX_H2"
    out, r = [], ws
    for _ in range(planes):
        t = r.to(torch.float16)
        out.append(pack_skinny(t.view(torch.bfloat16).contiguous(), dtype=L.X3, interleave_half=interleave_half))
        r = r - t.float()
    return out[0] if planes == 1 else torch.cat(out).as_subclass(Planed)


def decode_prep(x, xs, ssq, *, B, K, gamma=None, h=None, dtype=L.X3):
    check(load().mmx_decode_prep(_p(x), i64(x.shape[-1]), B, K, _p(gamma), _p(h), i64(h.shape[-1] if h is not None else 0), _p(xs),
                                 _p(ssq), dtype, stream()), "mmx_decode_prep")


def skinny2(xs, wp, *, B, K, N, dtype, bias=None, ssq_in=None, eps=1e-6, epi=0, out=None, ldo=None, xs_out=None, gamma_next=None,
            ssq_out=None, tiles_per_wg=1, ksplit=1, part=None, tickets=None):
    if isinstance(wp, Planed):
        dtype = L.H2W if dtype in (L.H2, L.H2W) else L.X3W
    check(load().mmx_skinny2(_p(xs), B, K, N, _p(wp), _p(bias), _p(ssq_in), C.c_float(eps), epi, _p(out),
                             i64(ldo if ldo is not None else N), _p(xs_out), _p(gamma_next), _p(ssq_out), tiles_per_wg, ksplit,
                             _p(part), i64(part.numel() if part is not None else 0), _p(tickets), dtype, stream()), "mmx_skinny2")


def rope_kv_store(qkv, inv_freq, pos, q_out, kc, vc, block_table, *, B, rows, Hq, Hkv, page, dtype, ldqkv=None, qkv_bs=None,
                  ldq=None, q_bs=None):
    ldqkv = (Hq + 2 * Hkv) * 64 if ldqkv is None else ldqkv
    ldq = Hq * 64 if ldq is None else ldq
    check(load().mmx_rope_kv_store(_p(qkv), i64(ldqkv), i64(rows * ldqkv if qkv_bs is None else qkv_bs), B, rows, Hq, Hkv, 64,
                                   _p(inv_freq), _p(pos), _p(q_out), i64(ldq), i64(rows * ldq if q_bs is None else q_bs), _p(kc), _p(vc),
                                   _p(block_table), block_table.shape[1], page, dtype, stream()), "mmx_rope_kv_store")


def paged_attn(q, pos, kc, vc, block_table, out, *, B, rows, Hq, Hkv, page, dtype, ldq=None, q_bs=None, ldo=None, o_bs=None):
    ldq = Hq * 64 if ldq is None else ldq
    ldo = Hq * 64 if ldo is None else ldo
    check(load().mmx_paged_attn(_p(q), i64(ldq), i64(rows * ldq if q_bs is None else q_bs), B, rows, Hq, Hkv, 64, C.c_float(0.125),
                                _p(pos), _p(kc), _p(vc), _p(block_table), block_table.shape[1], page, _p(out),
                                i64(ldo), i64(rows * ldo if o_bs is None else o_bs), dtype, stream()), "mmx_paged_attn")


def decode_attn_bits(out_packed=False, per_head=False, out_split=False, one_head=False):
    return ((L.DA_PACKED if out_packed else 0) | (L.DA_PER_HEAD if per_head else 0) | (L.DA_ONE_HEAD if one_head else 0) |
            (L.DA_H2 if out_split == "f16" else L.DA_SPLIT if out_split else 0))


def decode_attn(qkv, inv_freq, pos, kc, vc, block_table, out, *, B, Hq, Hkv, page, dtype, rope_tab=None, out_packed=False,
                per_head=False, out_split=False, one_head=False, ldqkv=None, ldo=None, finished=None):
    assert finished is None or (finished.dtype == torch.int32 and finished.numel() >= B and finished.stride(-1) == 1)
    check(load().mmx_decode_attn_fin(_p(qkv), i64((Hq + 2 * Hkv) * 64 if ldqkv is None else ldqkv), B, Hq, Hkv, 64, _p(inv_freq), _p(rope_tab),
                                     _p(pos), _p(finished), _p(kc), _p(vc), _p(block_table), block_table.shape[1], page, C.c_float(0.125), _p(out),
                                     i64(Hq * 64 if ldo is None else ldo), dtype, decode_attn_bits(out_packed, per_head, out_split, one_head), stream()), "mmx_decode_attn_fin")


def swiglu(gu, out, *, rows, I, dtype, ldgu=None, ldo=None):
    check(load().mmx_swiglu(_p(gu), i64(ldgu or 2 * I), rows, I, _p(out), i64(ldo or I), dtype, stream()), "mmx_swiglu")


def sample_step(logits, state, out_tokens, speech_emb, next_x, *, V, B, eos_id, seed, top_k=25, top_p=0.8,
                win_size=10, tau_r=0.1, sampled=None, forced=None, logp_out=None):
    check(load().mmx_sample_step(_p(logits), i64(logits.shape[-1]), V, B, eos_id, top_k, C.c_float(top_p), win_size,
                                 C.c_float(tau_r), C.c_uint64(seed), _p(state), _p(out_tokens), out_tokens.shape[1],
                                 _p(sampled), _p(forced), _p(speech_emb), speech_emb.shape[1], _p(next_x),
                                 i64(next_x.shape[-1]), _p(logp_out), stream()), "mmx_sample_step")


SAMP_MODE, SAMP_TOP_K, SAMP_WIN, SAMP_TOP_P, SAMP_TAU_R, SAMP_SEED_LO, SAMP_SEED_HI = range(7)
SAMPLER_MODES = {"ras": 0, "nucleus": 1, "random": 2}


def sampler_column(mode=0, top_p=0.8, top_k=25, win_size=10, tau_r=0.1, seed=0):
    import struct
    mode = SAMPLER_MODES.get(mode, mode)
    if mode not in (0, 1, 2) or not 1 <= int(top_k) <= 64 or not 0 <= int(win_size) <= 64:
        raise ValueError(f"sampler out of range: mode {mode!r} (0..2), top_k {top_k} (1..64), win_size {win_size} (0..64)")
    bits = lambda v: struct.unpack("<i", struct.pack("<f", float(v)))[0]
    i32 = lambda u: u - (1 << 32) if u >= (1 << 31) else u
    seed = int(seed) & ((1 << 64) - 1)
    return [int(mode), int(top_k), int(win_size), bits(top_p), bits(tau_r), i32(seed & 0xffffffff), i32(seed >> 32), 0]


def sample_step_tab(logits, state, out_tokens, speech_emb, next_x, samp, *, V, B, eos_id, sampled=None, forced=None, logp_out=None):
    assert samp.dtype == torch.int32 and samp.is_contiguous() and samp.shape == (8, B)
    check(load().mmx_sample_step_tab(_p(logits), i64(logits.shape[-1]), V, B, eos_id, _p(samp), _p(state), _p(out_tokens),
                                     out_tokens.shape[1], _p(sampled), _p(forced), _p(speech_emb), speech_emb.shape[1],
                                     _p(next_x), i64(next_x.shape[-1]), _p(logp_out), stream()), "mmx_sample_step_tab")
```

Baseline: 569.5.

## Skip padded row tiles in flow estimator resnet and tail kernels

Passes per-batch valid lengths to the estimator's fused resnet and transformer-tail kernels, which return early when a whole 64-row-aligned tile lies past the sequence length. A third kernel also zero-fills outputs for tiles past the length. Persistent zeroed buffers are reused across timesteps, so skipped regions keep well-defined contents. The aim is to remove wasted compute on padding when batched non-streaming requests have uneven lengths. The cost is extra zero-initialised buffers and a dependence on the padding rows never being read with non-zero meaning.

```diff
diff --git a/include/mmx_hip.h b/include/mmx_hip.h
--- a/include/mmx_hip.h
+++ b/include/mmx_hip.h
@@ -219,6 +219,8 @@
 } MmxEstResnetParams;
 int mmx_est_tail(const MmxEstTailParams* p, int dtype, int bm, int cfg, hipStream_t stream);
 int mmx_est_resnet(const MmxEstResnetParams* p, int dtype, int bm, int cfg, hipStream_t stream);
+int mmx_est_tail_len(const MmxEstTailParams* p, const int32_t* lens, int dtype, int bm, int cfg, hipStream_t stream);
+int mmx_est_resnet_len(const MmxEstResnetParams* p, const int32_t* lens, int dtype, int bm, int cfg, hipStream_t stream);
 typedef struct {
     const float* x;
     float* x_out;
diff --git a/minimax-speech_amd/csrc/fused.hip b/minimax-speech_amd/csrc/fused.hip
--- a/minimax-speech_amd/csrc/fused.hip
+++ b/minimax-speech_amd/csrc/fused.hip
@@ -405,6 +405,11 @@
             *reinterpret_cast<uint2*>(tile0 + plane + off[u]) = lo;
         }
     }
+}
+
+__device__ __forceinline__ bool tile_is_padding(int len, int t0, int Tn) {
+    const int n = len < Tn ? (len > 0 ? len : 0) : Tn;
+    return t0 >= ((n + 63) & ~63);
 }
 
 template <typename T, int NW, int PW = 4>
@@ -511,7 +516,7 @@
 }
 
 template <typename T, int BM, int PF, int NW, int NS, int PW, bool WP = false>
-__device__ __forceinline__ void est_tail_tile(const MmxEstTailParams& p, const int tile) {
+__device__ __forceinline__ void est_tail_tile(const MmxEstTailParams& p, const int tile, const int32_t* __restrict__ lens) {
     constexpr bool HK = NS == 2 && BM == 64 && sizeof(T) == 2;
     static_assert(!HK || (NW == 8 && PW == 2), "64-row split tile: 8 waves, 32-column passes");
     constexpr int MF = BM / 16, E = FT<T>::E, KB = FT<T>::KB, C = 256, CI = 512, CF = 1024, CH = HK ? 256 : 512, NCH = CF / CH;
@@ -533,6 +538,7 @@
     const int g = lane >> 4, l16 = lane & 15, rl = lane >> 2;
     float* patch = patch_all + wave * PATCHF;
     const int b = blockIdx.y, t0 = p.t_begin + tile * BM, Tn = p.T;
+    const int len = lens ? lens[b] : Tn;
     const int col0 = wave * WC + (lane & 3) * CW;
     unsigned long long* st = nullptr;
     if constexpr (LAB) {
@@ -582,6 +588,7 @@
             }
         }
         ring.prime(wo_w, ns0, NK0, NFN);
+        if (tile_is_padding(len, t0, Tn)) return;
         if constexpr (HK) {
             static_assert(P0 == P1 && PL0 == PL1, "both halves of the attention tile have the shape of a1");
             load_tile_split_halves(reinterpret_cast<const float*>(p.ao) + (long)b * p.ao_bs, p.ldao, t0, Tn, BM, buf0, a1, P0, PL0, tid, 64 * NW);
@@ -748,12 +755,12 @@
 }
 
 template <typename T, int BM, int PF, int NW, int NS = 1, int OCC = 1, int PW = 4, bool WP = false>
-__global__ __launch_bounds__(64 * NW, OCC) void est_tail_kernel(MmxEstTailParams p) {
-    est_tail_tile<T, BM, PF, NW, NS, PW, WP>(p, blockIdx.x);
+__global__ __launch_bounds__(64 * NW, OCC) void est_tail_kernel(MmxEstTailParams p, const int32_t* __restrict__ lens) {
+    est_tail_tile<T, BM, PF, NW, NS, PW, WP>(p, blockIdx.x, lens);
 }
 
 template <typename T, int BM, int PF, int NW, int NS = 1, bool WP = false>
-__global__ __launch_bounds__(64 * NW) void est_resnet_kernel(MmxEstResnetParams p) {
+__global__ __launch_bounds__(64 * NW) void est_resnet_kernel(MmxEstResnetParams p, const int32_t* __restrict__ lens) {
     constexpr int MF = BM / 16, MH = MF + 1, E = FT<T>::E, KB = FT<T>::KB, C = 256;
     constexpr int WC = C / NW, CW = WC / 4, NFN = WC / 16;
     constexpr int P1 = tile_pitch(C, sizeof(T));
@@ -771,6 +778,7 @@
     const int g = lane >> 4, l16 = lane & 15, rl = lane >> 2;
     float* patch = patch_all + wave * PATCH_FLOATS;
     const int b = blockIdx.y, t0 = p.t_begin + blockIdx.x * BM, Tn = p.T;
+    const int len = lens ? lens[b] : Tn;
     const int col0 = wave * WC + (lane & 3) * CW;
     const int cs = cin / KB;
     const T* w1 = reinterpret_cast<const T*>(p.w1) + (long)lane * E;
@@ -794,6 +802,7 @@
         const int t = t0 - 16 + i * 16 + rl;
         rm1[i] = (t >= 0 && t < Tn) ? (rmk ? rmk[t] : 1.f) : 0.f;
     }
+    if (tile_is_padding(len, t0, Tn)) return;
     if constexpr (NS == 1) load_tile<T>(reinterpret_cast<const T*>(p.a_in) + (long)b * p.a_bs, p.lda, t0 - 18, Tn, BM + 18, cin, ain, PA, tid, 64 * NW);
     else load_tile_split(reinterpret_cast<const float*>(p.a_in) + (long)b * p.a_bs, p.lda, t0 - 18, Tn, BM + 18, cin, ain, PA, PLA, tid, 64 * NW);
     __syncthreads();
@@ -916,6 +925,19 @@
         prm[id] = v < 5 ? val : 1.0f / (val + 1e-9f);
     }
     __syncthreads();
+    if (t0 >= len) {
+        const int rows = p.T - t0 < BM ? p.T - t0 : BM;
+        float* xo = p.x_out ? p.x_out + (long)b * p.x_bs + (long)t0 * C : nullptr;
+        for (int id = tid * 4; id < rows * C; id += 256 * 4) {
+            if (xo) *reinterpret_cast<float4*>(xo + id) = make_float4(0.f, 0.f, 0.f, 0.f);
+            if (p.act_out) {
+                TA* ao = reinterpret_cast<TA*>(p.act_out) + (long)b * p.x_bs + (long)t0 * C + id;
+                if constexpr (NS == 1) *reinterpret_cast<uint2*>(ao) = make_uint2(0, 0);
+                else *reinterpret_cast<float4*>(ao) = make_float4(0.f, 0.f, 0.f, 0.f);
+            }
+        }
+        return;
+    }
     {
         constexpr int CPR = CP / 4, U = 16;
         const int total = rows_in * CPR;
@@ -1062,19 +1084,19 @@
            (size_t)(bm + 16) * nw * 4;
 }
 
-template <typename P>
+template <typename P, typename... X>
 struct Form {
     int dtype;
     bool wp;
     int bm, nw, pf;
     int pw, C;
-    int (*launch)(const P&, hipStream_t);
+    int (*launch)(const P&, X..., hipStream_t);
 };
 template <typename T, int NS>
 constexpr int form_dtype = sizeof(T) == 4 ? MMX_F32 : NS == 2 ? MMX_X2 : MMX_BF16;
-template <typename P, size_t N>
-constexpr const Form<P>* find_form(const Form<P> (&forms)[N], int dtype, bool wp, int bm, int nw, int pf, int pw, int C) {
-    for (const Form<P>& f : forms)
+template <typename F, size_t N>
+constexpr const F* find_form(const F (&forms)[N], int dtype, bool wp, int bm, int nw, int pf, int pw, int C) {
+    for (const F& f : forms)
         if (f.dtype == dtype && f.wp == wp && f.bm == bm && f.nw == nw && f.pf == pf && f.pw == pw && f.C == C) return &f;
     return nullptr;
 }
@@ -1104,15 +1126,15 @@
 }
 
 template <typename T, int BM, int PF, int NW, int NS, int PW, bool WP>
-int launch_tail(const MmxEstTailParams& p, hipStream_t stream) {
+int launch_tail(const MmxEstTailParams& p, const int32_t* lens, hipStream_t stream) {
     constexpr size_t lds = tail_lds(sizeof(T), BM, NW, NS);
     MMX_CHECK_ARG(lds <= LDS_MAX);
     MMX_LDS_OPT_IN((est_tail_kernel<T, BM, PF, NW, NS, 1, PW, WP>), lds);
-    hipLaunchKernelGGL((est_tail_kernel<T, BM, PF, NW, NS, 1, PW, WP>), dim3((p.T - p.t_begin + BM - 1) / BM, p.B), dim3(64 * NW), lds, stream, p);
+    hipLaunchKernelGGL((est_tail_kernel<T, BM, PF, NW, NS, 1, PW, WP>), dim3((p.T - p.t_begin + BM - 1) / BM, p.B), dim3(64 * NW), lds, stream, p, lens);
     MMX_LAUNCH_CHECK();
     return MMX_OK;
 }
-using TailForm = Form<MmxEstTailParams>;
+using TailForm = Form<MmxEstTailParams, const int32_t*>;
 template <typename T, int BM, int PF, int NW, int NS = 1, int PW = 4, bool WP = false>
 constexpr TailForm tail_form() { return {form_dtype<T, NS>, WP, BM, NW, PF, PW, 0, launch_tail<T, BM, PF, NW, NS, PW, WP>}; }
 constexpr TailForm TAIL_FORMS[] = {
@@ -1146,15 +1168,15 @@
 static_assert(tail_select(MMX_F32, false, 32, 0)->launch == launch_tail<float, 32, 4, 4, 1, 4, false> && tail_select(MMX_F32, false, 16, 0)->launch == launch_tail<float, 16, 8, 4, 1, 4, false>);
 
 template <typename T, int BM, int PF, int NW, int NS, bool WP>
-int launch_resnet(const MmxEstResnetParams& p, hipStream_t stream) {
+int launch_resnet(const MmxEstResnetParams& p, const int32_t* lens, hipStream_t stream) {
     const size_t lds = resnet_lds(sizeof(T), BM, NW, NS, p.cin);
     MMX_CHECK_ARG(lds <= LDS_MAX);
     MMX_LDS_OPT_IN((est_resnet_kernel<T, BM, PF, NW, NS, WP>), lds);
-    hipLaunchKernelGGL((est_resnet_kernel<T, BM, PF, NW, NS, WP>), dim3((p.T - p.t_begin + BM - 1) / BM, p.B), dim3(64 * NW), lds, stream, p);
+    hipLaunchKernelGGL((est_resnet_kernel<T, BM, PF, NW, NS, WP>), dim3((p.T - p.t_begin + BM - 1) / BM, p.B), dim3(64 * NW), lds, stream, p, lens);
     MMX_LAUNCH_CHECK();
     return MMX_OK;
 }
-using ResnetForm = Form<MmxEstResnetParams>;
+using ResnetForm = Form<MmxEstResnetParams, const int32_t*>;
 template <typename T, int BM, int PF, int NW, int NS = 1, bool WP = false>
 constexpr ResnetForm resnet_form() { return {form_dtype<T, NS>, WP, BM, NW, PF, 0, 0, launch_resnet<T, BM, PF, NW, NS, WP>}; }
 constexpr ResnetForm RESNET_FORMS[] = {
@@ -1241,34 +1263,40 @@
 }
 #endif
 
-extern "C" int mmx_est_tail(const MmxEstTailParams* pp, int dtype, int bm, int cfg, hipStream_t stream) {
+extern "C" int mmx_est_tail_len(const MmxEstTailParams* pp, const int32_t* lens, int dtype, int bm, int cfg, hipStream_t stream) {
     MMX_CHECK_ARG(pp != nullptr);
     const MmxEstTailParams& p = *pp;
     const bool wplanes = dtype == MMX_X2W;
     if (wplanes) dtype = MMX_X2;
     MMX_CHECK_ARG(p.ao && p.x && p.wo && p.w1 && p.w2 && p.bo && p.b1 && p.b2 && p.n3g && p.n3b && p.B > 0 && p.T > 0);
-    MMX_CHECK_ARG(p.t_begin >= 0 && p.t_begin < p.T && p.t_begin % 16 == 0);
+    MMX_CHECK_ARG(p.t_begin >= 0 && p.t_begin < p.T && p.t_begin % 16 == 0 && (!lens || p.t_begin == 0));
     MMX_CHECK_ARG(p.ldao >= 512 && p.ldao % (dtype == MMX_X2 ? 4 : 8) == 0 && p.ao_bs % (dtype == MMX_X2 ? 4 : 8) == 0 && p.x_bs % 4 == 0);
     MMX_CHECK_ARG(((uintptr_t)p.ao % 16) == 0 && ((uintptr_t)p.x % 16) == 0);
     MMX_CHECK_ARG(!p.act_out || (p.act_ld % (dtype == MMX_X2 ? 4 : 8) == 0 && p.act_bs % (dtype == MMX_X2 ? 4 : 8) == 0 && ((uintptr_t)p.act_out % 16) == 0));
     if (int rc = check_next(p.next, dtype, p.T)) return rc;
     const TailForm* form = tail_select(dtype, wplanes, bm, cfg);
-    return form ? form->launch(p, stream) : MMX_EARG;
-}
-
-extern "C" int mmx_est_resnet(const MmxEstResnetParams* pp, int dtype, int bm, int cfg, hipStream_t stream) {
+    return form ? form->launch(p, lens, stream) : MMX_EARG;
+}
+extern "C" int mmx_est_tail(const MmxEstTailParams* pp, int dtype, int bm, int cfg, hipStream_t stream) {
+    return mmx_est_tail_len(pp, nullptr, dtype, bm, cfg, stream);
+}
+
+extern "C" int mmx_est_resnet_len(const MmxEstResnetParams* pp, const int32_t* lens, int dtype, int bm, int cfg, hipStream_t stream) {
     MMX_CHECK_ARG(pp != nullptr);
     const MmxEstResnetParams& p = *pp;
     const bool wplanes = dtype == MMX_X2W;
     if (wplanes) dtype = MMX_X2;
     MMX_CHECK_ARG(p.a_in && p.x && p.w1 && p.w2 && p.wr && p.b1 && p.b2 && p.br && p.g1 && p.be1 && p.g2 && p.be2 && p.tv);
-    MMX_CHECK_ARG(p.t_begin >= 0 && p.t_begin < p.T && p.t_begin % 16 == 0);
+    MMX_CHECK_ARG(p.t_begin >= 0 && p.t_begin < p.T && p.t_begin % 16 == 0 && (!lens || p.t_begin == 0));
     MMX_CHECK_ARG(p.B > 0 && p.T > 0 && p.cin >= 64 && p.cin % 32 == 0 && p.cin <= 512 && p.lda >= p.cin);
     MMX_CHECK_ARG(p.lda % (dtype == MMX_X2 ? 4 : 8) == 0 && p.a_bs % (dtype == MMX_X2 ? 4 : 8) == 0);
     MMX_CHECK_ARG(((uintptr_t)p.a_in % 16) == 0 && ((uintptr_t)p.x % 16) == 0 && p.x_bs % 4 == 0 && p.tv_bs % 4 == 0 && ((uintptr_t)p.tv % 16) == 0);
     if (int rc = check_next(p.next, dtype, p.T)) return rc;
     const ResnetForm* form = resnet_select(dtype, wplanes, bm, cfg, p.cin);
-    return form ? form->launch(p, stream) : MMX_EARG;
+    return form ? form->launch(p, lens, stream) : MMX_EARG;
+}
+extern "C" int mmx_est_resnet(const MmxEstResnetParams* pp, int dtype, int bm, int cfg, hipStream_t stream) {
+    return mmx_est_resnet_len(pp, nullptr, dtype, bm, cfg, stream);
 }
 
 extern "C" int mmx_dac_ru(const MmxDacRuParams* pp, int dtype, int bm, hipStream_t stream) {
diff --git a/minimax-speech_amd/mmx/_lib.py b/minimax-speech_amd/mmx/_lib.py
--- a/minimax-speech_amd/mmx/_lib.py
+++ b/minimax-speech_amd/mmx/_lib.py
@@ -25,7 +25,7 @@
 SYMBOLS = [
     "mmx_abi_version", "mmx_gemm_win", "mmx_gemm_win_tile", "mmx_rownorm", "mmx_groupnorm", "mmx_act_rows", "mmx_gather_rows", "mmx_copy2d", "mmx_est_pack",
     "mmx_sinusoidal_emb", "mmx_cfg_euler", "mmx_attn_dense", "mmx_attn_flash_bf16", "mmx_attn_flash_fp8", "mmx_attn_relpos_bf16", "mmx_attn_relpos_x", "mmx_attn_flash_x", "mmx_attn_flash_xs", "mmx_conv_cout1_tanh", "mmx_conv_cin1", "mmx_vae_sample", "mmx_resample_linear", "mmx_prefetch4", "mmx_mask_rows",
-    "mmx_est_tail", "mmx_est_resnet", "mmx_dac_ru", "mmx_pack_skinny", "mmx_skinny_gemm", "mmx_skinny2", "mmx_decode_prep", "mmx_rope_kv_store", "mmx_paged_attn", "mmx_decode_attn", "mmx_decode_attn_fin", "mmx_swiglu", "mmx_sample_step",
+    "mmx_est_tail", "mmx_est_resnet", "mmx_est_tail_len", "mmx_est_resnet_len", "mmx_dac_ru", "mmx_pack_skinny", "mmx_skinny_gemm", "mmx_skinny2", "mmx_decode_prep", "mmx_rope_kv_store", "mmx_paged_attn", "mmx_decode_attn", "mmx_decode_attn_fin", "mmx_swiglu", "mmx_sample_step",
     "mmx_sample_step_tab", "mmx_logmel", "mmx_pool_rows", "mmx_logmel_w", "mmx_s3_rope_fsmn", "mmx_fsq_encode", "mmx_resample_sinc", "mmx_kweight_blocks", "mmx_loudness_gate", "mmx_scale_rows",
     "mmx_spec_dist", "mmx_wave_sums",
 ]
diff --git a/minimax-speech_amd/mmx/flow.py b/minimax-speech_amd/mmx/flow.py
--- a/minimax-speech_amd/mmx/flow.py
+++ b/minimax-speech_amd/mmx/flow.py
@@ -86,6 +86,8 @@
 
 
 class FlowEngine:
+    skip_padding = True
+
     def __init__(self, sd: Dict[str, torch.Tensor], dtype=BF16, device="cuda", n_timesteps=10, cfg_rate=0.7,
                  enc_chunk=25, est_chunk=50, pre_lookahead_len=3, use_graphs=True, parts=("encoder", "estimator"),
                  fused=None, attn="bf16", wplanes=False):
@@ -486,18 +488,29 @@
         ops.linear(t2, self.mlp_w, 1024, dtype=dt, bias=self.mlp_b, out_f32=tv)
         return tv
 
-    def estimator(self, x, x_bstride, mu, spks, cond, t, B, T, mask=None, streaming=False, out=None, x_mod=None, klen=None):
+    def _on_rows(self, B, T):
+        return bool(self.fused or (self.fused is None and (self.dtype == BF16 or self.split or B * ((T + 15) // 16) >= 256)))
+
+    def _skip_bufs(self, B, T):
+        C = self.C
+        z = lambda *sh, f32=False: torch.zeros(*sh, dtype=torch.float32 if f32 else self.tdt, device=self.dev)
+        qk, vt = self._attn_bufs(B, T, presplit=True)
+        return dict(a=z(B, T, C), cat=z(B, T, 2 * C), xs=z(B, T, C, f32=True), attn=(qk.zero_(), vt))
+
+    def estimator(self, x, x_bstride, mu, spks, cond, t, B, T, mask=None, streaming=False, out=None, x_mod=None, klen=None, skip=None):
         C, chunk = self.C, (self.est_chunk if streaming else 0)
         tv = self._time_mlp(t, B)
-        a = self._new(B, T, C)
-        S = dict(h0=self._new(B, T, 320), cat=self._new(B, T, 2 * C), amid=[a] * len(self.mid), aup=a, a2=self._new(B, T, C),
-                 c1=self._new(B, T, C, f32=True), afin=a, d=(self._new(B, T, 80, f32=True) if out is None else out),
-                 xs=self._new(B, T, C, f32=True))
+        skip = skip or {}
+        a = skip["a"] if skip else self._new(B, T, C)
+        S = dict(h0=self._new(B, T, 320), cat=(skip["cat"] if skip else self._new(B, T, 2 * C)), amid=[a] * len(self.mid), aup=a,
+                 a2=self._new(B, T, C), c1=self._new(B, T, C, f32=True), afin=a, d=(self._new(B, T, 80, f32=True) if out is None else out),
+                 xs=(skip["xs"] if skip else self._new(B, T, C, f32=True)))
         ops.est_pack(x, mu, spks, cond, S["h0"], B=B, T=T, dtype=self.dtype, x_bstride=x_bstride, x_mod=(x_mod or B))
-        if self.fused or (self.fused is None and (self.dtype == BF16 or self.split or B * ((T + 15) // 16) >= 256)):
+        if self._on_rows(B, T):
             S["ao"] = self._new(B, T, 512)
-            self._estimator_rows(S, tv, B, T, chunk, itertools.repeat(self._attn_bufs(B, T, presplit=True)), mask=mask,
-                                 klen=klen, fp8=self.attn_fp8, form=(self.polite_flash_form if self.polite else 0))
+            bufs = skip["attn"] if skip else self._attn_bufs(B, T, presplit=True)
+            self._estimator_rows(S, tv, B, T, chunk, itertools.repeat(bufs), mask=mask, klen=klen, fp8=self.attn_fp8,
+                                 form=(self.polite_flash_form if self.polite else 0), lens=(klen if skip else None))
             return S["d"]
 
         def stage(sw, a_in, lda, act_out, act_ld):
@@ -559,7 +572,7 @@
             return bm, br
         return (32 if tiles(32) >= 128 else 16), 16
 
-    def _estimator_rows(self, S, tv, B, T, chunk, attn_bufs, mask=None, klen=None, r0=0, Tc=None, fp8=False, form=0):
+    def _estimator_rows(self, S, tv, B, T, chunk, attn_bufs, mask=None, klen=None, r0=0, Tc=None, fp8=False, form=0, lens=None):
         dt, C, Tc = self.dtype, self.C, Tc or T
         bm_t, bm_r = self._tile_rows(B, T - r0)
         ntv = tv.shape[1]
@@ -573,13 +586,13 @@
             bufs = [next(attn_bufs) for _ in blocks]
             ops.est_resnet(a_in, lda, lda, S["xs"], r, tv[:, r["idx"] * C:], ntv, B=B, T=T, dtype=dt,
                            bm=(16 if (self.split and lda > 320) else bm_r), rowmask=mask, nxt=nxt(blocks[0], *bufs[0]),
-                           t_begin=r0, Tcap=Tc)
+                           t_begin=r0, Tcap=Tc, lens=lens)
             for j, w in enumerate(blocks):
                 last = j == len(blocks) - 1
                 self._attention(*bufs[j], S["ao"], B=B, T=T, chunk=chunk, mask=mask, klen=klen, q_begin=r0, fp8=fp8, form=form)
                 ops.est_tail(S["ao"], S["xs"], w, B=B, T=T, dtype=dt, bm=bm_t, rowmask=(mask if last else None),
                              act_out=(act_out if last else None), act_ld=act_ld,
-                             nxt=(None if last else nxt(blocks[j + 1], *bufs[j + 1])), t_begin=r0, Tcap=Tc)
+                             nxt=(None if last else nxt(blocks[j + 1], *bufs[j + 1])), t_begin=r0, Tcap=Tc, lens=lens)
 
         self._walk(stage, S, B, T, mask, r0, Tc)
 
@@ -764,6 +777,7 @@
         P.mask = torch.ones(2 * n, T, device=self.dev) if masked else None
         P.klen = torch.full((2 * n,), T, dtype=torch.int32, device=self.dev) if masked else None
         P.d = self._new(2 * n, T, 80, f32=True)
+        P.skip = self._skip_bufs(2 * n, T) if masked and n > 1 and not streaming and self.skip_padding and self._on_rows(2 * n, T) else None
         tt, dd = self.t_schedule()
         P.t_all = torch.tensor([[v] * (2 * n) for v in tt], dtype=torch.float32, device=self.dev)
         P.z = self.rand_noise[0, :, :T].t().contiguous().to(self.dev)
@@ -771,7 +785,7 @@
         def run():
             P.x.copy_(P.z.unsqueeze(0).expand(n, T, 80))
             for s in range(self.n_timesteps):
-                self.estimator(P.x, T * 80, P.mu, P.spks, P.cond, P.t_all[s], 2 * n, T, P.mask, streaming, out=P.d, x_mod=n, klen=P.klen)
+                self.estimator(P.x, T * 80, P.mu, P.spks, P.cond, P.t_all[s], 2 * n, T, P.mask, streaming, out=P.d, x_mod=n, klen=P.klen, skip=P.skip)
                 ops.cfg_euler(P.x, P.d[:n], P.d[n:], self.cfg, dd[s], n * T * 80)
 
         P.run = Graphed(run, self.use_graphs)
diff --git a/minimax-speech_amd/mmx/ops.py b/minimax-speech_amd/mmx/ops.py
--- a/minimax-speech_amd/mmx/ops.py
+++ b/minimax-speech_amd/mmx/ops.py
@@ -213,8 +213,13 @@
                          ldq=ldq, ldvt=ldvt)
 
 
+def _lens_ptr(lens, B):
+    assert lens.is_cuda and lens.dtype == torch.int32 and lens.is_contiguous() and lens.numel() >= B, "lens: int32 [B] on the device"
+    return _p(lens)
+
+
 def est_tail(ao, x, w, *, B, T, dtype, bm, rowmask=None, act_out=None, act_ld=0, nxt=None, eps=1e-5, pf=0, t_begin=0,
-             Tcap=None, waves=0, narrow=False, ldao=512):
+             Tcap=None, waves=0, narrow=False, ldao=512, lens=None):
     Tc = T if Tcap is None else Tcap
     p = L.fill_struct(L.EstTailParams(), ao=ao, x=x, wo=w["wo_p"], w1=w["w1_p"], w2=w["w2_p"], bo=w["bo"], b1=w["b1"],
                       b2=w["b2"], n3g=w["n3g"], n3b=w["n3b"], rowmask=rowmask, act_out=act_out, ao_bs=Tc * ldao,
@@ -223,12 +228,15 @@
         p.next = nxt
     if isinstance(w["wo_p"], Planed):
         dtype = L.X2W
-    check(load().mmx_est_tail(C.byref(p), C.c_int(dtype), C.c_int(bm), C.c_int(pf + 16 * waves + (512 if narrow else 0)), stream()),
-          "mmx_est_tail")
+    cfg = C.c_int(pf + 16 * waves + (512 if narrow else 0))
+    if lens is None:
+        check(load().mmx_est_tail(C.byref(p), C.c_int(dtype), C.c_int(bm), cfg, stream()), "mmx_est_tail")
+    else:
+        check(load().mmx_est_tail_len(C.byref(p), _lens_ptr(lens, B), C.c_int(dtype), C.c_int(bm), cfg, stream()), "mmx_est_tail_len")
 
 
 def est_resnet(a_in, lda, cin, x, r, tv, tv_bs, *, B, T, dtype, bm, rowmask=None, nxt=None, eps=1e-5, pf=0, t_begin=0,
-               Tcap=None, waves=0):
+               Tcap=None, waves=0, lens=None):
     Tc = T if Tcap is None else Tcap
     p = L.fill_struct(L.EstResnetParams(), a_in=a_in, x=x, w1=r["w1_p"], w2=r["w2_p"], wr=r["wr_p"], b1=r["b1"], g1=r["g1"],
                       be1=r["be1"], b2=r["b2"], g2=r["g2"], be2=r["be2"], br=r["br"], tv=tv, rowmask=rowmask,
@@ -237,7 +245,11 @@
         p.next = nxt
     if isinstance(r["w1_p"], Planed):
         dtype = L.X2W
-    check(load().mmx_est_resnet(C.byref(p), C.c_int(dtype), C.c_int(bm), C.c_int(pf + 16 * waves), stream()), "mmx_est_resnet")
+    if lens is None:
+        check(load().mmx_est_resnet(C.byref(p), C.c_int(dtype), C.c_int(bm), C.c_int(pf + 16 * waves), stream()), "mmx_est_resnet")
+    else:
+        check(load().mmx_est_resnet_len(C.byref(p), _lens_ptr(lens, B), C.c_int(dtype), C.c_int(bm), C.c_int(pf + 16 * waves), stream()),
+              "mmx_est_resnet_len")
 
 
 def pack_dac_ru(w7: torch.Tensor, w1: torch.Tensor, dtype):
```

Result: no change. 572.9 (median of 6 runs) (+0.6%).
